# jeya-maria-jose/Medical-Transformer

Hardware: AMD Instinct MI355X
Metric: training images/sec (MedT, 3x128x128) (higher is better)
Workload: dtype f32; 1 GPU; MedT imgsize=128 bs=4/GPU train step (fwd+CE+bwd+Adam), BASELINE.json configs[2] (per GPU: also configs[3]'s shard); global_batch=4, parallelism=dp1

## Files before the change

include/medt_abi.h:

```cpp
#ifndef MEDT_ABI_H
#define MEDT_ABI_H

#include <stddef.h>
#include <stdint.h>

#ifdef __cplusplus
extern "C" {
#endif

#define MEDT_ABI_VERSION 11

#define MEDT_OK            0
#define MEDT_EINVAL       -1
#define MEDT_EUNSUPPORTED -2
#define MEDT_ELAUNCH      -3
#define MEDT_EWORKSPACE   -4

int         medt_abi_version(void);
const char* medt_last_error(void);

void*  medt_queue_create(void);
int    medt_queue_destroy(void* queue);
int    medt_queue_bind(void* queue, void* stream);
size_t medt_queue_pending(const void* queue);
int    medt_queue_flush(void* queue, void* stream);
int    medt_queue_flush2(void* queue, void* stream, void* aux_stream);
int    medt_queue_discard(void* queue);

typedef struct medt_axial_desc {
    int32_t N, C, H, W;
    int32_t G;
    int32_t axis;
    int32_t has_pos;
    int32_t stride;
    int32_t training;
    int32_t bn_groups;
    float   eps;
    float   momentum;
    int32_t out_relu;
    int32_t gate_mode;
    int32_t act_dtype;
} medt_axial_desc;

typedef struct medt_bn_ptrs {
    const float* weight;
    const float* bias;
    float*       running_mean;
    float*       running_var;
    int64_t*     num_batches_tracked;
} medt_bn_ptrs;

typedef struct medt_axial_params {
    const float* w_qkv;
    medt_bn_ptrs bn_qkv;
    medt_bn_ptrs bn_similarity;
    medt_bn_ptrs bn_output;
    const float* relative;
    const float* f_qr;
    const float* f_kr;
    const float* f_sve;
    const float* f_sv;
} medt_axial_params;

typedef struct medt_axial_saved {
    void*  qkv_raw;
    void*  stacked;
    float* lse;
    float* stats;
} medt_axial_saved;

typedef struct medt_axial_grads {
    float* w_qkv;
    float* bn_qkv_weight;  float* bn_qkv_bias;
    float* bn_sim_weight;  float* bn_sim_bias;
    float* bn_out_weight;  float* bn_out_bias;
    float* relative;
    float* gates;
} medt_axial_grads;

size_t medt_axial_stats_floats(const medt_axial_desc*);
size_t medt_axial_workspace_bytes(const medt_axial_desc*);

int medt_axial_layer_fwd(const medt_axial_desc*, const medt_axial_params*, const float* x, float* y,
                         const medt_axial_saved*, void* workspace, size_t workspace_bytes, void* stream);

int medt_axial_layer_bwd(const medt_axial_desc*, const medt_axial_params*, const float* x, const float* y,
                         const float* dy, const medt_axial_saved*, float* dx, const medt_axial_grads*,
                         void* workspace, size_t workspace_bytes, void* stream);

int medt_axial_core_stats(const medt_axial_desc*, const medt_axial_params*, const medt_axial_saved*,
                          void* workspace, size_t workspace_bytes, void* stream);
int medt_axial_core_fwd(const medt_axial_desc*, const medt_axial_params*, const medt_axial_saved*,
                        void* workspace, size_t workspace_bytes, void* stream);
int medt_axial_core_bwd(const medt_axial_desc*, const medt_axial_params*, const medt_axial_saved*, const float* dy,
                        void* workspace, size_t workspace_bytes, void* stream);

typedef struct medt_block_desc {
    int32_t N, C, width, H, W;
    int32_t G;
    int32_t training, bn_groups;
    float   eps, momentum;
} medt_block_desc;

typedef struct medt_block_params {
    const float*      w_down;
    medt_bn_ptrs      bn1;
    medt_axial_params height;
    medt_axial_params width;
    const float*      w_up;
    medt_bn_ptrs      bn2;
} medt_block_params;

typedef struct medt_block_saved {
    float* z1;
    float* y1;
    float* stats1;
    medt_axial_saved height;
    float* y_h;
    medt_axial_saved width;
    float* y_w;
    float* z2;
    float* stats2;
} medt_block_saved;

size_t medt_wopos_block_workspace_bytes(const medt_block_desc*);
int medt_wopos_block_fwd(const medt_block_desc*, const medt_block_params*, const float* x, float* y,
                         const medt_block_saved*, void* workspace, size_t workspace_bytes, void* stream);

typedef struct medt_block_s2_params {
    medt_block_params blk;
    const float*      w_ds;
    medt_bn_ptrs      bn_ds;
} medt_block_s2_params;
typedef struct medt_block_s2_saved {
    medt_block_saved blk;
    float *zd, *yd, *statsd;
} medt_block_s2_saved;
size_t medt_wopos_block_s2_workspace_bytes(const medt_block_desc*);
int medt_wopos_block_s2_fwd(const medt_block_desc*, const medt_block_s2_params*, const float* x, float* y,
                            const medt_block_s2_saved*, void* workspace, size_t workspace_bytes, void* stream);

typedef struct medt_block_grads {
    float *w_down, *bn1_weight, *bn1_bias;
    medt_axial_grads height, width;
    float *w_up, *bn2_weight, *bn2_bias;
} medt_block_grads;
size_t medt_wopos_block_bwd_workspace_bytes(const medt_block_desc*);
int medt_wopos_block_bwd(const medt_block_desc*, const medt_block_params*, const float* x, const float* y, const float* dy,
                         const medt_block_saved*, float* dx, const float* dx_add, const medt_block_grads*,
                         void* workspace, size_t workspace_bytes, void* stream);

typedef struct medt_conv_desc {
    int32_t N, Cin, H, W, Cout;
    int32_t K, stride, pad;
    int32_t has_bias;
    int32_t has_bn;
    int32_t has_res;
    int32_t relu;
    int32_t training, bn_groups;
    float   eps, momentum;
    int32_t lean;
} medt_conv_desc;

size_t medt_conv_stats_floats(const medt_conv_desc*);
size_t medt_conv_workspace_bytes(const medt_conv_desc*);

int medt_conv_block_fwd(const medt_conv_desc*, const float* x, const float* w, const float* bias,
                        const medt_bn_ptrs* bn, const float* res, float* z, float* y, float* stats,
                        void* workspace, size_t workspace_bytes, void* stream);
int medt_conv_block_bwd(const medt_conv_desc*, const float* x, const float* w, const medt_bn_ptrs* bn,
                        const float* z, const float* y, const float* stats, const float* dy,
                        float* dx, float* dw, float* dbias, float* dbn_weight, float* dbn_bias, float* dres,
                        const float* dx_add, void* workspace, size_t workspace_bytes, void* stream);

int medt_gate_mlp_fwd(const float* x, const float* w1, const float* b1, const float* w2, const float* b2, float* xn, float* h,
                      float* o, float* gates, int N, int C, int H, int W, int axis, void* stream);
int medt_gate_mlp_bwd(const float* dgates, const float* gates, const float* o, const float* h, const float* xn,
                      const float* w1, const float* w2, float* scratch, float* dw1, float* db1, float* dw2, float* db2,
                      float* dx, int N, int C, int H, int W, int axis, void* stream);

int medt_up2x_relu_add_fwd(const float* x, const float* skip, float* y, int NC, int H, int W, void* stream);
int medt_up2x_relu_bwd(const float* x, const float* dy, float* dx, int NC, int H, int W, void* stream);

int medt_patch_gather(const float* x, float* xp, int N, int C, int S, int P, int G, void* stream);
int medt_logo_merge_fwd(const float* x, const float* yp, float* y, int N, int C, int S, int P, int G, void* stream);
int medt_logo_merge_bwd(const float* dy, float* dx, float* dyp, int N, int C, int S, int P, int G, void* stream);

size_t medt_ce_partials(int N, int HW);
int medt_ce_fwd(const float* logits, const int64_t* target, float* partials, float* loss_out, int N, int K, int HW,
                int ignore_index, void* stream);
int medt_ce_bwd(const float* logits, const int64_t* target, const float* loss_out, const float* dloss, float* dlogits,
                int N, int K, int HW, int ignore_index, void* stream);

size_t medt_seg_loss_workspace(int N, int K, int HW);
size_t medt_seg_loss_out_floats(int N, int K);
int medt_seg_loss_fwd(const float* logits, const int64_t* target, const float* class_weight, float* partials, float* out,
                      int N, int K, int HW, int ignore_index, float ce_scale, float dice_scale, float eps, void* stream);
int medt_seg_loss_bwd(const float* logits, const int64_t* target, const float* class_weight, const float* out,
                      const float* dloss, float* dlogits, int N, int K, int HW, int ignore_index, float ce_scale,
                      float dice_scale, float eps, void* stream);

int medt_adam_step(float* p, const float* g, float* m, float* v, float* state, size_t n, float lr, float beta1,
                   float beta2, float eps, float weight_decay, float gscale, void* stream);

int medt_relu_mask(const float* a, const float* y, float* out, size_t n, void* stream);

int medt_seg_counts(const float* logits, const int64_t* target, int32_t* counts, int N, int K, int HW, float threshold,
                    void* stream);

int medt_window_gather(const float* image, float* windows, const int32_t* oy, const int32_t* ox, int C, int H, int W, int S,
                       int ny, int nx, void* stream);
int medt_window_blend(const float* win_logits, float* blended, uint8_t* mask, const int32_t* oy, const int32_t* ox, int K,
                      int H, int W, int S, int ny, int nx, float threshold, void* stream);

size_t medt_augment_param_floats(void);
size_t medt_augment_workspace(int N, int th, int tw);
int medt_augment_stats(const uint8_t* image, const float* params, float* workspace, int N, int H, int W, int C, int th,
                       int tw, void* stream);
int medt_augment_apply(const uint8_t* image, const uint8_t* mask, const float* params, float* workspace, float* out_image,
                       int64_t* out_mask, int N, int H, int W, int C, int th, int tw, int use_stats, void* stream);

#define MEDT_EDT_NONE    2147483647
#define MEDT_EDT_MAX_DIM 4096
int medt_edt_cols(const uint8_t* mask, int32_t* g2, int N, int H, int W, int border_mode, void* stream);
int medt_edt_rows(const int32_t* g2, const uint8_t* select, int32_t* d2, int N, int H, int W, void* stream);

#define MEDT_LABEL_TILE_H  16
#define MEDT_LABEL_TILE_W  64
#define MEDT_LABEL_MAX_DIM 4096
size_t medt_label_workspace_bytes(int N, int H, int W);
int medt_label_components(const uint8_t* mask, int32_t* labels, int32_t* count, void* workspace, size_t workspace_bytes, int N,
                          int H, int W, int connectivity, int background, void* stream);
int medt_label_tables(const int32_t* labels, int32_t* area, uint8_t* frame, int N, int H, int W, int stride, int max_count,
                      void* stream);
int medt_label_select(const int32_t* labels, const uint8_t* keep, const uint8_t* mask, uint8_t* out, int N, int H, int W,
                      int stride, void* stream);

#ifdef __cplusplus
}
#endif
#endif
```

medical-transformer_amd/csrc/conv.hip:

```cpp
#include "defer.h"
#include <type_traits>

namespace medt {

template <int K, int OT>
__global__ __launch_bounds__(MEDT_THREADS) void conv2d_fwd_kernel(
    const float* __restrict__ x, const float* __restrict__ w, const float* __restrict__ bias, float* __restrict__ y,
    float* __restrict__ partials, int Cin, int H, int W, int Cout, int Ho, int Wo, int stride, int pad, int relu,
    int npg, int y_bf16) {
    constexpr int KK = K * K;
    MEDT_STATIC_SHARED float red[MEDT_WAVES * OT * 2 * 2];
    const int HoWo = Ho * Wo, per_group = npg * HoWo, ppg = (per_group + MEDT_THREADS - 1) / MEDT_THREADS;
    const int grp = blockIdx.x / ppg, part = blockIdx.x - grp * ppg, o0 = blockIdx.y * OT;
    const int q = part * MEDT_THREADS + threadIdx.x;
    const bool ok = q < per_group;
    const int ni = ok ? q / HoWo : 0, p = ok ? q - ni * HoWo : 0;
    const int n = grp * npg + ni;
    const int ho = p / Wo, wo = p - ho * Wo;
    const int h0 = ho * stride - pad, w0 = wo * stride - pad;
    float acc[OT];
#pragma unroll
    for (int o = 0; o < OT; ++o) acc[o] = bias ? bias[o0 + o] : 0.f;
    const float* xn = x + (size_t)n * Cin * H * W;
    int off[KK];
// ... 304 lines not shown
    for (; o + U <= Cout; o += U) taps(std::integral_constant<int, U>{}, o);
    for (; o < Cout; ++o) taps(std::integral_constant<int, 1>{}, o);
    if (ok) {
        const size_t o0 = ((size_t)n * Cin + c0) * HW + p;
#pragma unroll
        for (int c = 0; c < CT; ++c) dx[o0 + (size_t)c * HW] = add ? acc[c] + add[o0 + (size_t)c * HW] : acc[c];
    }
}

template <int K, int CT, int TM = (1 << (K * K)) - 1>
__global__ __launch_bounds__(MEDT_THREADS) void conv2d_bwd_data_ws_kernel(
    const float* __restrict__ dy, const float* __restrict__ w, float* __restrict__ dx, int N, int Cin, int H, int W,
    int Cout, int Ho, int Wo, int stride, int pad, const float* __restrict__ add, int stage_dy) {
    constexpr int KK = K * K;
    MEDT_STATIC_SHARED float red[3][CT][64];
    extern __shared__ __attribute__((aligned(16))) float wl[];
    const int lane = threadIdx.x & 63, wv = threadIdx.x >> 6;
    const int HW = H * W;
    const long q = (long)blockIdx.x * 64 + lane;
    const int c0 = blockIdx.y * CT;
    if constexpr (TM == (1 << KK) - 1) {
        const int nw = Cout * CT * KK;
        for (int e0 = threadIdx.x; e0 < nw; e0 += 8 * MEDT_THREADS) {
            float v[8];
#pragma unroll
            for (int u = 0; u < 8; ++u) {
                const int e = min(e0 + u * MEDT_THREADS, nw - 1), o = e / (CT * KK), r = e - o * (CT * KK);
                v[u] = w[((size_t)o * Cin + c0) * KK + r];
            }
            MEDT_SCHED_FENCE();
#pragma unroll
            for (int u = 0; u < 8; ++u)
                if (e0 + u * MEDT_THREADS < nw) wl[e0 + u * MEDT_THREADS] = v[u];
        }
    } else {
        constexpr int NL = __builtin_popcount((unsigned)TM);
        const int nw = Cout * CT * NL;
        for (int e0 = threadIdx.x; e0 < nw; e0 += 8 * MEDT_THREADS) {
            float v[8];
            int dst[8];
#pragma unroll
            for (int u = 0; u < 8; ++u) {
                const int e = min(e0 + u * MEDT_THREADS, nw - 1), oc = e / NL, tl = e - oc * NL;
                int t = 0, seen = 0;
#pragma unroll
                for (int b = 0; b < KK; ++b)
                    if ((TM >> b) & 1) { if (seen == tl) t = b; ++seen; }
                const int o = oc / CT, c = oc - o * CT;
                dst[u] = oc * KK + t;
                v[u] = w[((size_t)o * Cin + c0 + c) * KK + t];
            }
            MEDT_SCHED_FENCE();
#pragma unroll
            for (int u = 0; u < 8; ++u)
                if (e0 + u * MEDT_THREADS < nw) wl[dst[u]] = v[u];
        }
    }
    float* dl = wl + Cout * CT * KK;
    const int HoWo_ = Ho * Wo;
    const int nb0 = (int)(((long)blockIdx.x * 64) / HW);
    const int img_stride = Cout * HoWo_ + 1;
    if (stage_dy) {
        const int nb1 = min(N - 1, (int)(((long)blockIdx.x * 64 + 63) / HW));
        const int per = Cout * HoWo_, cnt = (nb1 - nb0 + 1) * per;
        const float* src = dy + (size_t)nb0 * per;
        for (int e0 = threadIdx.x; e0 < cnt; e0 += 8 * MEDT_THREADS) {
            float v[8];
#pragma unroll
            for (int u = 0; u < 8; ++u) v[u] = src[min(e0 + u * MEDT_THREADS, cnt - 1)];
            MEDT_SCHED_FENCE();
#pragma unroll
            for (int u = 0; u < 8; ++u) {
                const int e = e0 + u * MEDT_THREADS;
                if (e < cnt) { const int im = e / per; dl[im * img_stride + (e - im * per)] = v[u]; }
            }
        }
    }
    const bool ok = q < (long)N * HW;
    const int n = ok ? (int)(q / HW) : 0, p = ok ? (int)(q - (long)n * HW) : 0;
    const int h = p / W, ww = p - h * W;
    int off[KK];
#pragma unroll
    for (int kh = 0; kh < K; ++kh)
#pragma unroll
        for (int kw = 0; kw < K; ++kw) {
            const int hh = h + pad - kh, wq = ww + pad - kw;
            int o = -1;
            if (ok && hh >= 0 && wq >= 0 && hh % stride == 0 && wq % stride == 0) {
                const int ho = hh / stride, wo = wq / stride;
                if (ho < Ho && wo < Wo) o = ho * Wo + wo;
            }
            off[kh * K + kw] = o;
        }
    float acc[CT];
#pragma unroll
    for (int c = 0; c < CT; ++c) acc[c] = 0.f;
    const float* dyn = dy + (size_t)n * Cout * Ho * Wo;
    const int ob = (Cout * wv) / 4, oe = (Cout * (wv + 1)) / 4;
    __syncthreads();
    constexpr int U = K == 1 ? 16 : 4;
    const int HoWo = Ho * Wo;
    const float* dln = dl + (n - nb0) * img_stride;
    auto taps = [&](auto u_tag, int o) {
        constexpr int UU = decltype(u_tag)::value;
        float dr[UU][KK];
        if (stage_dy) {
#pragma unroll
            for (int u = 0; u < UU; ++u)
#pragma unroll
                for (int t = 0; t < KK; ++t) dr[u][t] = ((TM >> t) & 1) ? dln[(o + u) * HoWo + max(off[t], 0)] : 0.f;
        } else {
#pragma unroll
            for (int u = 0; u < UU; ++u)
#pragma unroll
                for (int t = 0; t < KK; ++t) dr[u][t] = ((TM >> t) & 1) ? dyn[(size_t)(o + u) * HoWo + max(off[t], 0)] : 0.f;
            MEDT_SCHED_FENCE();
        }
#pragma unroll
        for (int u = 0; u < UU; ++u) {
            float dv[KK];
#pragma unroll
            for (int t = 0; t < KK; ++t) dv[t] = off[t] >= 0 ? dr[u][t] : 0.f;
#pragma unroll
            for (int c = 0; c < CT; ++c) {
                const float* wp = wl + ((o + u) * CT + c) * KK;
#pragma unroll
                for (int t = 0; t < KK; ++t)
                    if ((TM >> t) & 1) acc[c] = fmaf(wp[t], dv[t], acc[c]);
            }
        }
        MEDT_SCHED_FENCE();
    };
    int o = ob;
    for (; o + U <= oe; o += U) taps(std::integral_constant<int, U>{}, o);
    for (; o < oe; ++o) taps(std::integral_constant<int, 1>{}, o);
    if (wv > 0) {
#pragma unroll
        for (int c = 0; c < CT; ++c) red[wv - 1][c][lane] = acc[c];
    }
    __syncthreads();
    if (wv == 0 && ok) {
        const size_t o0 = ((size_t)n * Cin + c0) * HW + p;
#pragma unroll
        for (int c = 0; c < CT; ++c) {
            const float v = acc[c] + (red[0][c][lane] + red[1][c][lane]) + red[2][c][lane];
            dx[o0 + (size_t)c * HW] = add ? v + add[o0 + (size_t)c * HW] : v;
        }
    }
}

static bool conv_bwd_data_ws_enabled() {
    static const bool on = true;
    return on;
}

template <int K>
static int conv2d_bwd_data_k(const float* dy, const float* w, float* dx, int N, int Cin, int H, int W, int Cout, int Ho,
                             int Wo, int stride, int pad, hipStream_t s, const float* add) {
    if constexpr (K != 7) {
        static const long ws_pos3 = 16384L;
        const long npos = (long)N * H * W;
        if ((npos <= 4096 || (K == 3 && Cout * K * K >= 512 && npos <= ws_pos3)) && Cout >= 64 && conv_bwd_data_ws_enabled()) {
            const unsigned g64 = (unsigned)(((long)N * H * W + 63) / 64);
            const int imgs = H * W >= 64 ? 2 : 64 / (H * W) + 1;
            const size_t dy_floats = (size_t)imgs * (Cout * Ho * Wo + 1);
            int tmask = 0;
            if (K == 3)
                for (int h = 0; h < H && h < 8; ++h)
                    for (int ww = 0; ww < W && ww < 8; ++ww)
                        for (int t = 0; t < 9; ++t) {
                            const int hh = h + pad - t / 3, wq = ww + pad - t % 3;
                            if (hh >= 0 && wq >= 0 && hh % stride == 0 && wq % stride == 0 && hh / stride < Ho && wq / stride < Wo) tmask |= 1 << t;
                        }
#ifdef MEDT_AB_DGRAD_ALLTAPS
            tmask = 0x1ff;
#endif
            const bool four = K == 3 && H <= 8 && W <= 8 && tmask == 0x1b0;
#define MEDT_LAUNCH_WS(CT)                                                                                           \
    do {                                                                                                             \
        if constexpr (K == 3) {                                                                                      \
            if (four) {                                                                                              \
                hipLaunchKernelGGL((conv2d_bwd_data_ws_kernel<K, CT, 0x1b0>), dim3(g64, Cin / CT), dim3(MEDT_THREADS), \
                                   ((size_t)Cout * CT * K * K + (stage ? dy_floats : 0)) * sizeof(float), s, dy, w, dx, N, Cin, H, W, \
                                   Cout, Ho, Wo, stride, pad, add, stage);                                          \
                break;                                                                                               \
            }                                                                                                        \
        }                                                                                                            \
        hipLaunchKernelGGL((conv2d_bwd_data_ws_kernel<K, CT>), dim3(g64, Cin / CT), dim3(MEDT_THREADS),               \
                           ((size_t)Cout * CT * K * K + (stage ? dy_floats : 0)) * sizeof(float), s, dy, w, dx, N, Cin, H, W, \
                           Cout, Ho, Wo, stride, pad, add, stage);                                                  \
    } while (0)
            int ct = pick_tile(Cin, K == 1 ? 8 : 4, g64);
            while (ct > 1 && (size_t)Cout * ct * K * K * sizeof(float) > 48 * 1024) ct >>= 1;
            if ((size_t)Cout * ct * K * K * sizeof(float) > 48 * 1024) ct = 0;
            const int stage = (K == 3 && ct && ((size_t)Cout * ct * K * K + dy_floats) * sizeof(float) <= 60 * 1024) ? 1 : 0;
            switch (ct) {
                case 0: break;
                case 8: if constexpr (K == 1) { MEDT_LAUNCH_WS(8); } break;
                case 4: MEDT_LAUNCH_WS(4); break;
                case 2: MEDT_LAUNCH_WS(2); break;
                default: MEDT_LAUNCH_WS(1); break;
            }
#undef MEDT_LAUNCH_WS
            if (ct) return launch_status("conv2d_bwd_data_ws");
        }
    }
    const unsigned gx = (unsigned)(((long)N * H * W + MEDT_THREADS - 1) / MEDT_THREADS);
#define MEDT_LAUNCH_BWD(CT)                                                                                       \
    hipLaunchKernelGGL((conv2d_bwd_data_kernel<K, CT>), dim3(gx, Cin / CT), dim3(MEDT_THREADS), 0, s, dy, w, dx, N, Cin, \
                       H, W, Cout, Ho, Wo, stride, pad, add)
    switch (pick_tile(Cin, K == 7 ? 4 : 16, gx)) {
        case 16: if constexpr (K != 7) { MEDT_LAUNCH_BWD(16); } break;
        case 8: if constexpr (K != 7) { MEDT_LAUNCH_BWD(8); } break;
        case 4: MEDT_LAUNCH_BWD(4); break;
        case 2: MEDT_LAUNCH_BWD(2); break;
        default: MEDT_LAUNCH_BWD(1); break;
    }
#undef MEDT_LAUNCH_BWD
    return launch_status("conv2d_bwd_data");
}

static bool conv2d_bwd_data_thin(int N, int Cin, int H, int W, int Cout, int K, int stride, int pad) {
    return (conv_thin_mode() & 2) && stride == 1 && K == 3 && pad == 1 && !conv_use_mfma(Cout, Cin, K, 1, (long)N * H * W) &&
           conv_thin_ok(N, 1, Cout, H, W, Cin, K, 1, 1);
}
bool conv2d_bwd_data_flips(int N, int Cin, int H, int W, int Cout, int K, int stride, int pad) {
    return stride == 1 && K - 1 - pad >= 0 &&
           (conv_use_mfma(Cout, Cin, K, 1, (long)N * H * W) || conv2d_bwd_data_thin(N, Cin, H, W, Cout, K, stride, pad));
}

int conv2d_bwd_data(const float* dy, const float* w, float* dx, float* wt_scratch, float* ksplit_scratch, int N, int Cin,
                    int H, int W, int Cout, int K, int stride, int pad, hipStream_t s, const float* add, bool wt_ready) {
    const int Ho = (H + 2 * pad - K) / stride + 1, Wo = (W + 2 * pad - K) / stride + 1;
    if (abl_skip(N >= 16 ? (K == 3 ? "conv3_dgrad_l" : "conv1_dgrad_l") : (K == 3 ? "conv3_dgrad_g" : "conv1_dgrad_g"))) return MEDT_OK;
    if (wt_scratch && conv2d_bwd_data_thin(N, Cin, H, W, Cout, K, stride, pad)) {
        if (!wt_ready) {
            int rc = conv_flip_weights(w, wt_scratch, Cout, Cin, K, s);
            if (rc) return rc;
        }
        return conv_thin_fwd(dy, wt_scratch, nullptr, add, dx, nullptr, N, 1, Cout, H, W, Cin, 0, s);
    }
    if (!add && wt_scratch && conv_use_mfma(Cout, Cin, K, 1, (long)N * H * W) && conv2d_bwd_data_flips(N, Cin, H, W, Cout, K, stride, pad) &&
        (ksplit_scratch || conv_mfma_scratch_floats(N, 1, H * W, Cout, Cin, K, conv_rows16_ok(Cout, H, W, K, 1, K - 1 - pad)) == 0))
        return conv_mfma_bwd_data_s1(dy, w, wt_scratch, ksplit_scratch, dx, N, Cin, H, W, Cout, K, pad, s, wt_ready);
    switch (K) {
        case 1: return conv2d_bwd_data_k<1>(dy, w, dx, N, Cin, H, W, Cout, Ho, Wo, stride, pad, s, add);
        case 3: return conv2d_bwd_data_k<3>(dy, w, dx, N, Cin, H, W, Cout, Ho, Wo, stride, pad, s, add);
        case 7: return conv2d_bwd_data_k<7>(dy, w, dx, N, Cin, H, W, Cout, Ho, Wo, stride, pad, s, add);
    }
    set_error("conv2d: kernel size %d unsupported (1, 3, 7)", K);
    return MEDT_EUNSUPPORTED;
}

template <int K, int TO, int TC>
__device__ __forceinline__ void conv_wgrad_body(
    const float* __restrict__ dy, const float* __restrict__ raw, const float* __restrict__ coef,
    const float* __restrict__ x, float* __restrict__ scratch, int N, int Cin, int H, int W, int Cout, int Ho, int Wo,
    int stride, int pad, int QS, int npg, int bx, int by, int bz) {
    constexpr int KK = K * K, RO = TO / 16, RC = TC / 16;
    MEDT_STATIC_SHARED __attribute__((aligned(16))) float A[TO][68];
    MEDT_STATIC_SHARED __attribute__((aligned(16))) float B[TC][68];
    const int Ktot = Cin * KK, HoWo = Ho * Wo;
    const int o0 = bx * TO, k0 = by * TC;
    const long NP = (long)N * HoWo;
    const long q_begin = (long)bz * QS;
    const long q_end = q_begin + QS < NP ? q_begin + QS : NP;
    const int to = threadIdx.x >> 4, tc = threadIdx.x & 15;
    const int j = threadIdx.x & 63, r0 = threadIdx.x >> 6;
    float acc[RO][RC];
#pragma unroll
    for (int a = 0; a < RO; ++a)
#pragma unroll
        for (int b = 0; b < RC; ++b) acc[a][b] = 0.f;
    constexpr int NA = TO / 4, NB = TC / 4;
    float ra[NA], rb[NB];
    auto fetch = [&](long q0) {
        const long q = q0 + j;
        const bool qok = q < q_end;
        const int n = qok ? (int)(q / HoWo) : 0, p = qok ? (int)(q - (long)n * HoWo) : 0;
        const int ho = p / Wo, wo = p - ho * Wo;
        const int hb = ho * stride - pad, wb = wo * stride - pad;
        const float* dyp = dy + (size_t)n * Cout * HoWo + p;
        const float* rawp = raw ? raw + (size_t)n * Cout * HoWo + p : nullptr;
        const float* cf = coef ? coef + (size_t)(n / npg) * Cout * 3 : nullptr;
        const float* xp = x + (size_t)n * Cin * H * W;
#pragma unroll
        for (int i = 0; i < NA; ++i) {
            float a = 0.f;
            const int o = o0 + r0 + 4 * i;
            if (qok && o < Cout) {
                a = dyp[(size_t)o * HoWo];
                if (cf) a = fmaf(cf[o * 3], a, fmaf(cf[o * 3 + 1], rawp[(size_t)o * HoWo], cf[o * 3 + 2]));
            }
            ra[i] = a;
        }
#pragma unroll
        for (int i = 0; i < NB; ++i) {
            float b = 0.f;
            const int k = k0 + r0 + 4 * i;
            if (qok && k < Ktot) {
                const int c = k / KK, t = k - c * KK;
                const int kh = t / K, kw = t - kh * K;
                const int h = hb + kh, w = wb + kw;
                if (h >= 0 && h < H && w >= 0 && w < W) b = xp[((size_t)c * H + h) * W + w];
            }
            rb[i] = b;
// ... 223 lines not shown
```

medical-transformer_amd/csrc/medt_api.hip:

```cpp
#include "defer.h"
#include "fin_inline.h"
#include <string.h>

namespace medt {

static thread_local char g_err[512] = "";

void set_error(const char* fmt, ...) {
    va_list ap;
    va_start(ap, fmt);
    vsnprintf(g_err, sizeof(g_err), fmt, ap);
    va_end(ap);
}

bool abl_skip(const char* family) {
#ifndef MEDT_ABLATE
    (void)family;
    return false;
#else
    static const char* env = [] {
        const char* e = getenv("MEDT_SKIP");
        if (e && *e)
            fprintf(stderr, "libmedt_hip: MEDT_SKIP=%s -- TIMING EXPERIMENT: these kernel families are NOT launched, every result of "
                            "this process is garbage\n", e);
// ... 19 lines not shown
    if (e != hipSuccess) {
        (void)hipGetLastError();
        set_error("%s: opt-in for more than 64 KB of dynamic LDS refused on device %d: %s", what, dev, hipGetErrorString(e));
        return MEDT_ELAUNCH;
    }
    if (dev < 64) done[dev] = 1;
    return MEDT_OK;
}

int launch_status(const char* what) {
    hipError_t e = hipGetLastError();
    if (e != hipSuccess) {
        set_error("%s: %s", what, hipGetErrorString(e));
        return MEDT_ELAUNCH;
    }
    return MEDT_OK;
}

struct LayerStats {
    BnStats qkv, sim, out;
    LayerStats(float* p, const AxialGeom& g) {
        const int nq = g.groups * 2 * g.C, ns = g.groups * g.SC, no = g.groups * g.OC;
        qkv = BnStats(p, nq);
        sim = BnStats(p + 4 * (size_t)nq, ns);
        out = BnStats(p + 4 * (size_t)(nq + ns), no);
    }
};

struct FwdWs {
    float *part_qkv, *part_sim, *part_out, *qkv_ksplit, *tables, *gate_eff;
    unsigned* flag;
    FwdWs(Carver& c, const AxialGeom& g) {
        flag = c.take<unsigned>(4);
        gate_eff = c.take<float>(4);
        const size_t kq = conv2d_fwd_scratch_floats(g.N, g.groups, g.C, g.H, g.W, 2 * g.C, 1, 1, 0);
        qkv_ksplit = c.take<float>(kq);
        if (!kq) qkv_ksplit = nullptr;
        part_qkv = c.take<float>((size_t)g.groups * conv_parts_per_group(g.N, g.groups, g.HW, g.C, 2 * g.C, 1, 1) * 2 * g.C * 2 * 2);
        part_sim = c.take<float>((size_t)g.groups * sim_stats_parts(g) * g.SC * 2 * 2);
        tables = c.take<float>(sim_tables_floats(g));
        part_out = c.take<float>((size_t)g.groups * g.tpg * g.OC * 2 * 2);
    }
};

struct BwdWs {
    float *part_ob, *coef_out, *part_sb, *coef_sim, *dqkv, *part_qb, *coef_qkv, *rel_part, *gate_part, *dw_scratch,
        *dy_masked, *gate_eff, *gate_tmp;
    float *tables, *gram, *pg_part, *gate_raw, *gate_rows;
    float* raw32;
    size_t nblocks;
    bool sweep;
    SweepPlan plan;
    size_t sweep_blocks;
    int qb_rpg;
    BwdWs(Carver& c, const AxialGeom& g, int stride, int out_relu, int gate_mode) {
        gate_eff = c.take<float>(4);
        gate_tmp = c.take<float>(4);
        const int ppg = conv2d_parts_per_group(g.N, g.groups, g.HW), TL = 2 * g.L - 1;
        sweep = axial_bwd_sweep_plan(g, gate_mode == 2 ? 4 : 0, &plan);
        sweep_blocks = sweep ? (size_t)g.groups * plan.nparts * g.G : 0;
        qb_rpg = sweep ? plan.nparts + plan.fparts : g.tpg;
        nblocks = (size_t)g.groups * g.tpg * g.G;
        const size_t rel_rows = sweep ? sweep_blocks + (size_t)g.groups * g.G : nblocks;
        part_ob = c.take<float>((size_t)g.groups * ppg * g.OC * 2);
        coef_out = c.take<float>((size_t)g.groups * g.OC * 3);
        part_sb = c.take<float>((size_t)g.groups * (sweep && plan.nparts > g.tpg ? plan.nparts : g.tpg) * g.G * 4);
        coef_sim = c.take<float>((size_t)g.groups * g.SC * 3);
        dqkv = c.take<float>((size_t)g.N * 2 * g.C * g.HW);
        part_qb = c.take<float>((size_t)g.groups * (qb_rpg > g.tpg ? qb_rpg : g.tpg) * 2 * g.C * 2);
        coef_qkv = c.take<float>((size_t)g.groups * 2 * g.C * 3);
        rel_part = c.take<float>(g.pos ? (rel_rows > nblocks ? rel_rows : nblocks) * 2 * g.gp * TL : 0);
        const size_t nseqh = (size_t)g.groups * g.spg * g.G;
        gate_part = c.take<float>(g.pos ? (nblocks > nseqh ? nblocks : nseqh) * 4 : 0);
        dw_scratch = c.take<float>((size_t)conv2d_bwd_weight_splits(g.N, g.C, 2 * g.C, 1, g.H, g.W) * 2 * g.C * g.C);
        dy_masked = c.take<float>(out_relu ? (size_t)g.N * g.C * (g.H / stride) * (g.W / stride) : 0);
        tables = c.take<float>(sweep ? sim_tables_floats(g) : 0);
        gram = c.take<float>(sweep ? (size_t)g.groups * g.spg * g.G * plan.npg_floats : 0);
        pg_part = c.take<float>(sweep ? sweep_blocks * g.L * plan.npg_floats : 0);
        gate_raw = c.take<float>(sweep ? sweep_blocks * 4 : 0);
        gate_rows = c.take<float>(sweep ? (size_t)g.groups * g.G * 4 : 0);
        static const bool raw32_on = true;
        raw32 = c.take<float>(sweep && g.bf16 && raw32_on ? (size_t)g.N * 2 * g.C * g.HW : 0);
        if (!(sweep && g.bf16 && raw32_on)) raw32 = nullptr;
    }
};

static int attention_core_bwd(const AxialGeom& g, const medt_axial_desc* d, const medt_axial_params* p, const BwdWs& w,
                              const float* qkv_raw, const float* stacked, const float* lse, const float* dy, const LayerStats& st,
                              GatePtrs gates, bool want_gates, float* d_sim_w, float* d_sim_b, hipStream_t s,
                              const BfinSrc* ob = nullptr, bool sim_inline = false, const BfinSrc* qb = nullptr,
                              const float* ymask = nullptr) {
    const int tr = d->training ? 1 : 0;
    int rc;
    if (w.sweep) {
        if ((rc = axial_attn_bwd_sweep(g, w.plan, qkv_raw, st.qkv, st.sim, p->relative, gates, stacked, lse, dy, w.coef_out,
                                       d->stride, w.dqkv, w.part_qb, w.qb_rpg, w.part_sb, w.rel_part, w.pg_part, w.gram,
                                       want_gates ? w.gate_raw : nullptr, s, w.raw32, ob, ymask))) return rc;
        AxialGeom gs = g;
        gs.tpg = w.plan.nparts;
        SimBSrc sb = no_simb_src();
        if (sim_inline) {
            sb.partials = w.part_sb; sb.rows = w.plan.nparts; sb.G = g.G; sb.SC = g.SC; sb.training = tr; sb.on = 1;
            sb.count = g.sim_count; sb.ss = st.sim; sb.weight = p->bn_similarity.weight;
            sb.coef = w.coef_sim; sb.dweight = d_sim_w; sb.dbias = d_sim_b;
        } else {
            const TablesJob tj{p->relative, w.tables, g.hq, g.L, tr ? sim_tables_blocks(g) : 0};
            if ((rc = axial_sim_bwd_finalize(gs, w.part_sb, st.sim, p->bn_similarity.weight, tr, w.coef_sim, d_sim_w, d_sim_b, s, &tj)))
                return rc;
        }
        if ((rc = axial_attn_bwd_fix(g, w.plan, qkv_raw, st.qkv, w.coef_sim, w.tables, w.gram, gates, tr, w.dqkv, w.part_qb,
                                     w.qb_rpg, s, sim_inline ? &sb : nullptr))) return rc;
        return axial_attn_bwd_relfix(g, w.plan, p->relative, w.coef_sim, st.sim, gates, w.pg_part,
                                     want_gates ? w.gate_raw : nullptr, tr, d->eps,
                                     w.rel_part + w.sweep_blocks * 2 * g.gp * (2 * g.L - 1), w.gate_rows, s, qb);
    }
    if ((rc = axial_attn_bwd_stats(g, qkv_raw, st.qkv, st.sim, p->relative, gates, stacked, lse, dy, w.coef_out, d->stride,
                                   w.part_sb, s))) return rc;
    if ((rc = axial_sim_bwd_finalize(g, w.part_sb, st.sim, p->bn_similarity.weight, tr, w.coef_sim, d_sim_w, d_sim_b, s)))
        return rc;
    return axial_attn_bwd(g, qkv_raw, st.qkv, st.sim, w.coef_sim, p->relative, gates, stacked, lse, dy, w.coef_out, d->stride,
                          w.dqkv, w.part_qb, w.rel_part, want_gates ? w.gate_part : nullptr, s);
}

static int effective_gates(const medt_axial_desc* d, const medt_axial_params* p, float* eff, hipStream_t s, GatePtrs* out) {
    *out = GatePtrs{p->f_qr, p->f_kr, p->f_sve, p->f_sv, 0};
    if (d->gate_mode == 0 || !p->f_qr) return MEDT_OK;
    if (d->gate_mode == 2) {
        *out = GatePtrs{p->f_qr, p->f_qr + 1, p->f_qr + 3, p->f_qr + 2, 4};
        return MEDT_OK;
    }
    if (d->gate_mode != 1) { set_error("axial: gate_mode %d unsupported (0: raw, 1: sigmoid, 2: per sequence)", d->gate_mode); return MEDT_EUNSUPPORTED; }
    if (!p->f_kr || !p->f_sve || !p->f_sv) { set_error("axial: gate_mode 1 needs all four gates"); return MEDT_EINVAL; }
    int rc = gate_sigmoid_fwd(p->f_qr, p->f_kr, p->f_sve, p->f_sv, eff, s);
    if (rc) return rc;
    *out = GatePtrs{eff, eff + 1, eff + 2, eff + 3, 0};
    return MEDT_OK;
}

static int check_common(const medt_axial_desc* d, const medt_axial_params* p, const medt_axial_saved* sv, AxialGeom* g) {
    if (!d || !p || !sv) { set_error("null descriptor / params / saved"); return MEDT_EINVAL; }
    int rc = axial_geom(*d, g);
    if (rc) return rc;
    if (!p->w_qkv || !p->bn_qkv.weight || !p->bn_qkv.bias || !p->bn_similarity.weight || !p->bn_similarity.bias ||
        !p->bn_output.weight || !p->bn_output.bias) { set_error("null parameter pointer"); return MEDT_EINVAL; }
    if (!d->training && (!p->bn_qkv.running_mean || !p->bn_qkv.running_var || !p->bn_similarity.running_mean ||
                         !p->bn_similarity.running_var || !p->bn_output.running_mean || !p->bn_output.running_var)) {
        set_error("eval mode needs running statistics"); return MEDT_EINVAL;
    }
    if (g->pos && !p->relative) { set_error("has_pos without relative table"); return MEDT_EINVAL; }
    if (!sv->qkv_raw || !sv->stacked || !sv->stats) { set_error("null saved buffer"); return MEDT_EINVAL; }
    return MEDT_OK;
}

}

using namespace medt;

extern "C" {

int medt_abi_version(void) { return MEDT_ABI_VERSION; }
const char* medt_last_error(void) { return g_err; }

size_t medt_axial_stats_floats(const medt_axial_desc* d) {
    AxialGeom g;
    if (!d || axial_geom(*d, &g)) return 0;
    return (size_t)4 * g.groups * (2 * g.C + g.SC + g.OC);
}

size_t medt_axial_workspace_bytes(const medt_axial_desc* d) {
    AxialGeom g;
    if (!d || axial_geom(*d, &g)) return 0;
    Carver cf(nullptr, 0), cb(nullptr, 0);
    FwdWs f(cf, g);
    BwdWs b(cb, g, d->stride, d->out_relu, d->gate_mode);
    return align_up(cf.off > cb.off ? cf.off : cb.off, 256) + 256;
}

int medt_axial_core_stats(const medt_axial_desc* d, const medt_axial_params* p, const medt_axial_saved* sv, void* ws,
                          size_t ws_bytes, void* stream) {
    AxialGeom g;
    int rc = check_common(d, p, sv, &g);
    if (rc) return rc;
    float* qkv_raw = (float*)sv->qkv_raw;
    float* stacked = (float*)sv->stacked;
    Carver c(ws, ws_bytes);
    FwdWs w(c, g);
    if (!ws || !c.ok()) { set_error("workspace too small: need %zu", c.off); return MEDT_EWORKSPACE; }
    LayerStats st(sv->stats, g);
    GatePtrs gates;
    if ((rc = effective_gates(d, p, w.gate_eff, (hipStream_t)stream, &gates))) return rc;
    return axial_logit_stats(g, qkv_raw, st.qkv, p->relative, gates, w.tables, w.part_sim, (hipStream_t)stream);
}

int medt_axial_core_fwd(const medt_axial_desc* d, const medt_axial_params* p, const medt_axial_saved* sv, void* ws,
                        size_t ws_bytes, void* stream) {
    AxialGeom g;
    int rc = check_common(d, p, sv, &g);
    if (rc) return rc;
    float* qkv_raw = (float*)sv->qkv_raw;
    float* stacked = (float*)sv->stacked;
    Carver c(ws, ws_bytes);
    FwdWs w(c, g);
    if (!ws || !c.ok()) { set_error("workspace too small: need %zu", c.off); return MEDT_EWORKSPACE; }
    LayerStats st(sv->stats, g);
    GatePtrs gates;
    if ((rc = effective_gates(d, p, w.gate_eff, (hipStream_t)stream, &gates))) return rc;
    return axial_attn_fwd(g, qkv_raw, st.qkv, st.sim, p->relative, gates, stacked, sv->lse,
                          d->training ? w.part_out : nullptr, w.flag, (hipStream_t)stream);
}

int medt_axial_core_bwd(const medt_axial_desc* d, const medt_axial_params* p, const medt_axial_saved* sv, const float* dy,
                        void* ws, size_t ws_bytes, void* stream) {
    AxialGeom g;
    int rc = check_common(d, p, sv, &g);
    if (rc) return rc;
    float* qkv_raw = (float*)sv->qkv_raw;
    float* stacked = (float*)sv->stacked;
    if (!dy || !sv->lse) { set_error("core_bwd: null dy / lse"); return MEDT_EINVAL; }
    if (d->out_relu) { set_error("core_bwd: out_relu layers are not supported by the benchmark entry"); return MEDT_EUNSUPPORTED; }
    Carver c(ws, ws_bytes);
    BwdWs w(c, g, d->stride, d->out_relu, d->gate_mode);
    if (!ws || !c.ok()) { set_error("workspace too small: need %zu", c.off); return MEDT_EWORKSPACE; }
    hipStream_t s = (hipStream_t)stream;
    LayerStats st(sv->stats, g);
    GatePtrs gates;
    if ((rc = effective_gates(d, p, w.gate_eff, s, &gates))) return rc;
    return attention_core_bwd(g, d, p, w, qkv_raw, stacked, sv->lse, dy, st, gates, p->f_qr != nullptr, w.part_ob,
                              w.part_ob + g.SC, s);
}

int medt_axial_layer_fwd(const medt_axial_desc* d, const medt_axial_params* p, const float* x, float* y,
                         const medt_axial_saved* sv, void* ws, size_t ws_bytes, void* stream) {
    AxialGeom g;
    int rc = check_common(d, p, sv, &g);
    if (rc) return rc;
    float* qkv_raw = (float*)sv->qkv_raw;
    float* stacked = (float*)sv->stacked;
    if (!x || !y) { set_error("null x / y"); return MEDT_EINVAL; }
    if (d->training && g.row_count <= 1.0) {
        set_error("axial: training-mode BatchNorm needs more than 1 value per channel (got %g)", g.row_count);
        return MEDT_EINVAL;
    }
    Carver c(ws, ws_bytes);
    FwdWs w(c, g);
    if (!ws || !c.ok()) { set_error("workspace too small: need %zu", c.off); return MEDT_EWORKSPACE; }
    hipStream_t s = (hipStream_t)stream;
    LayerStats st(sv->stats, g);
    GatePtrs gates;
    if ((rc = effective_gates(d, p, w.gate_eff, s, &gates))) return rc;
    const int tr = d->training ? 1 : 0, ppg = conv_parts_per_group(g.N, g.groups, g.HW, g.C, 2 * g.C, 1, 1);
    if (wopos_small_ok(g, *d)) {
        if ((rc = wopos_small_fwd(g, *d, *p, x, y, qkv_raw, stacked, sv->lse, w.part_qkv, w.part_sim, w.part_out,
                                  s))) return rc;
        if (Queue* q = queue_for(s)) {
            q->fin.push_back(FinJob{make_fin(w.part_qkv, 1, 2 * g.C, g.row_count, p->bn_qkv, st.qkv), g.groups, tr, d->momentum, d->eps});
            q->fin.push_back(FinJob{make_fin(w.part_sim, 1, g.SC, g.sim_count, p->bn_similarity, st.sim), g.groups, tr, d->momentum, d->eps});
            q->fin.push_back(FinJob{make_fin(w.part_out, 1, g.OC, g.row_count, p->bn_output, st.out), g.groups, tr, d->momentum, d->eps});
            return MEDT_OK;
        }
        return bn_finalize3(w.part_qkv, 2 * g.C, g.row_count, p->bn_qkv, st.qkv, w.part_sim, g.SC, g.sim_count,
                            p->bn_similarity, st.sim, w.part_out, g.OC, g.row_count, p->bn_output, st.out, 1, g.groups,
                            d->momentum, d->eps, tr, s);
    }
    if ((rc = conv2d_fwd(x, p->w_qkv, nullptr, qkv_raw, tr ? w.part_qkv : nullptr, w.qkv_ksplit, g.N, g.C, g.H, g.W,
                         2 * g.C, 1, 1, 0, 0, g.groups, s, g.bf16))) return rc;
    const TablesJob tj{p->relative, w.tables, g.hq, g.L, tr ? sim_tables_blocks(g) : 0};
    if ((rc = bn_finalize(w.part_qkv, ppg, g.groups, 2 * g.C, g.row_count, p->bn_qkv, d->momentum, d->eps, tr,
                          st.qkv, s, &tj))) return rc;
    if (tr && (rc = axial_logit_stats(g, qkv_raw, st.qkv, p->relative, gates, w.tables, w.part_sim, s))) return rc;
    auto fin_src_of = [&](const float* partials, int parts, int CH, double count, const medt_bn_ptrs& bn, BnStats out) {
        FinSrc fs = no_fin_src();
        fs.f = make_fin(partials, parts, CH, count, bn, out);
        fs.momentum = d->momentum; fs.eps = d->eps; fs.on = 1;
        return fs;
    };
    const bool sim_inl = inline_fin_ok(tr, g.groups, sim_stats_parts(g)) && axial_attn_fwd_inlines(g, gates, w.flag);
    const FinSrc sim_src = fin_src_of(w.part_sim, sim_stats_parts(g), g.SC, g.sim_count, p->bn_similarity, st.sim);
    if (!sim_inl && (rc = bn_finalize(w.part_sim, sim_stats_parts(g), g.groups, g.SC, g.sim_count, p->bn_similarity, d->momentum,
                                      d->eps, tr, st.sim, s))) return rc;
    if ((rc = axial_attn_fwd(g, qkv_raw, st.qkv, st.sim, p->relative, gates, stacked, sv->lse,
                             tr ? w.part_out : nullptr, w.flag, s, sim_inl ? &sim_src : nullptr))) return rc;
    const bool out_inl = inline_fin_ok(tr, g.groups, g.oparts) && axial_out_fwd_inlines(*d);
    const FinSrc out_src = fin_src_of(w.part_out, g.oparts, g.OC, g.row_count, p->bn_output, st.out);
    if (!out_inl && (rc = bn_finalize(w.part_out, g.oparts, g.groups, g.OC, g.row_count, p->bn_output, d->momentum, d->eps, tr,
                                      st.out, s))) return rc;
    return axial_out_fwd(*d, stacked, st.out, y, s, out_inl ? &out_src : nullptr);
}

int medt_axial_layer_bwd(const medt_axial_desc* d, const medt_axial_params* p, const float* x, const float* y,
                         const float* dy, const medt_axial_saved* sv, float* dx, const medt_axial_grads* gr, void* ws,
                         size_t ws_bytes, void* stream) {
    AxialGeom g;
    int rc = check_common(d, p, sv, &g);
    if (rc) return rc;
    float* qkv_raw = (float*)sv->qkv_raw;
    float* stacked = (float*)sv->stacked;
    if (!x || !dy || !dx || !gr || !sv->lse) { set_error("null x / dy / dx / grads / lse"); return MEDT_EINVAL; }
    if (!gr->w_qkv || !gr->bn_qkv_weight || !gr->bn_qkv_bias || !gr->bn_sim_weight || !gr->bn_sim_bias ||
        !gr->bn_out_weight || !gr->bn_out_bias || (g.pos && !gr->relative)) {
        set_error("null gradient pointer"); return MEDT_EINVAL;
    }
    if (d->out_relu && !y) { set_error("out_relu backward needs the forward output y"); return MEDT_EINVAL; }
    Carver c(ws, ws_bytes);
    BwdWs w(c, g, d->stride, d->out_relu, d->gate_mode);
    if (!ws || !c.ok()) { set_error("workspace too small: need %zu", c.off); return MEDT_EWORKSPACE; }
    hipStream_t s = (hipStream_t)stream;
    LayerStats st(sv->stats, g);
    GatePtrs gates;
    if ((rc = effective_gates(d, p, w.gate_eff, s, &gates))) return rc;
    const int tr = d->training ? 1 : 0, ppg = conv2d_parts_per_group(g.N, g.groups, g.HW), TL = 2 * g.L - 1;
    if (wopos_small_bwd_ok(g, *d)) {
        if ((rc = wopos_small_bwd(g, *d, *p, y, dy, qkv_raw, stacked, sv->lse, st.qkv, st.sim, st.out, w.dqkv,
                                  w.part_ob, w.part_sb, w.part_qb, w.coef_qkv, s))) return rc;
        if ((rc = wopos_small_bwd_finalize(g, *d, *p, w.part_ob, w.part_sb, w.part_qb, st.qkv, st.sim, st.out, *gr, s,
                                           queue_for(s)))) return rc;
        if ((rc = conv1x1_bwd_data(w.dqkv, qkv_raw, w.coef_qkv, p->w_qkv, dx, g.N, g.C, 2 * g.C, g.HW, g.groups, s)))
            return rc;
        return conv2d_bwd_weight(w.dqkv, qkv_raw, w.coef_qkv, x, gr->w_qkv, w.dw_scratch, g.N, g.C, g.H, g.W, 2 * g.C,
                                 1, 1, 0, g.groups, s, queue_for(s));
    }
    const float* ymask = nullptr;
    if (d->out_relu) {
#ifndef MEDT_AB_NO_MASK_FUSE
        if (w.sweep) ymask = y;
#endif
        if (!ymask) {
            if ((rc = relu_mask(dy, y, w.dy_masked, (size_t)g.N * g.C * (g.H / d->stride) * (g.W / d->stride), s))) return rc;
            dy = w.dy_masked;
        }
    }
    const float out_dscale = 1.f / (float)(d->stride * d->stride);
    const bool sim_inl = w.sweep && g.pos && inline_fin_ok(tr, g.groups, w.plan.nparts) &&
                         axial_out_bwd_stats_tables_ok(*d, sim_tables_blocks(g), g.L);
    const TablesJob btj{p->relative, w.tables, g.hq, g.L, sim_tables_blocks(g)};
    if ((rc = axial_out_bwd_stats(*d, stacked, dy, st.out, w.part_ob, s, sim_inl ? &btj : nullptr, ymask))) return rc;
    BfinSrc ob = no_bfin_src();
    if (w.sweep && inline_fin_ok(tr, g.groups, ppg)) {
        ob.j = BfinJob{w.part_ob, ppg, g.groups, g.OC, tr, g.row_count, out_dscale, st.out, p->bn_output.weight, w.coef_out,
                       gr->bn_out_weight, gr->bn_out_bias};
        ob.on = 1;
    } else if ((rc = bn_bwd_finalize(w.part_ob, ppg, g.groups, g.OC, g.row_count, out_dscale, st.out, p->bn_output.weight, tr,
                                     w.coef_out, gr->bn_out_weight, gr->bn_out_bias, s))) return rc;
    BfinSrc qb = no_bfin_src();
    if (w.sweep && (!g.bf16 || w.raw32) && inline_fin_ok(tr, g.groups, w.qb_rpg)) {
        qb.j = BfinJob{w.part_qb, w.qb_rpg, g.groups, 2 * g.C, tr, g.row_count, 1.f, st.qkv, p->bn_qkv.weight, w.coef_qkv,
                       gr->bn_qkv_weight, gr->bn_qkv_bias};
        qb.on = 1;
    }
    if ((rc = attention_core_bwd(g, d, p, w, qkv_raw, stacked, sv->lse, dy, st, gates, gr->gates != nullptr,
                                 gr->bn_sim_weight, gr->bn_sim_bias, s, ob.on ? &ob : nullptr, sim_inl, qb.on ? &qb : nullptr, ymask))) return rc;
    const float *bq_raw = qkv_raw, *bq_coef = w.coef_qkv;
    static const bool bf16_fused = true;
    if (g.bf16 && w.raw32) {
        if (!qb.on && (rc = bn_bwd_finalize(w.part_qb, w.qb_rpg, g.groups, 2 * g.C, g.row_count, 1.f, st.qkv, p->bn_qkv.weight, tr,
                                         w.coef_qkv, gr->bn_qkv_weight, gr->bn_qkv_bias, s))) return rc;
        bq_raw = w.raw32;
    } else if (g.bf16 && bf16_fused && (long)g.N * 2 * g.C <= 65535) {
        if ((rc = bn_bwd_fin_apply_bf16(w.part_qb, w.qb_rpg, g.groups, 2 * g.C, g.row_count, 1.f, st.qkv, p->bn_qkv.weight, tr,
                                        w.coef_qkv, gr->bn_qkv_weight, gr->bn_qkv_bias, w.dqkv, qkv_raw, g.N, g.HW, s))) return rc;
        bq_raw = nullptr;
        bq_coef = nullptr;
    } else {
        if (!qb.on && (rc = bn_bwd_finalize(w.part_qb, w.qb_rpg, g.groups, 2 * g.C, g.row_count, 1.f, st.qkv, p->bn_qkv.weight, tr,
                                            w.coef_qkv, gr->bn_qkv_weight, gr->bn_qkv_bias, s))) return rc;
        if (g.bf16) {
            if ((rc = bn_bwd_apply_raw_bf16(w.dqkv, qkv_raw, w.coef_qkv, g.N, 2 * g.C, g.HW, g.groups, s))) return rc;
            bq_raw = nullptr;
            bq_coef = nullptr;
        }
    }
    if ((rc = conv1x1_bwd_data(w.dqkv, bq_raw, bq_coef, p->w_qkv, dx, g.N, g.C, 2 * g.C, g.HW, g.groups, s)))
        return rc;
    Queue* q = queue_for(s);
    if ((rc = conv2d_bwd_weight(w.dqkv, bq_raw, bq_coef, x, gr->w_qkv, w.dw_scratch, g.N, g.C, g.H, g.W, 2 * g.C, 1,
                                1, 0, g.groups, s, q))) return rc;
    if (g.pos) {
        const int rel_rows = w.sweep ? (int)w.sweep_blocks + g.groups * g.G : (int)w.nblocks;
        const float* gate_src = w.sweep ? w.gate_rows : w.gate_part;
        const int gate_rows = w.sweep ? g.groups * g.G : (int)w.nblocks;
        if (q) q->reduce.push_back(RJob{w.rel_part, gr->relative, rel_rows, 2 * g.gp * TL});
        else if ((rc = reduce_rows(w.rel_part, rel_rows, 2 * g.gp * TL, gr->relative, s))) return rc;
        if (gr->gates && d->gate_mode == 2) {
            if ((rc = gate_seq_reduce(w.gate_part, gr->gates, g.groups * g.spg, g.G, s))) return rc;
        } else if (gr->gates) {
            const bool sig = d->gate_mode == 1 && p->f_qr;
            if (q && !sig) q->reduce.push_back(RJob{gate_src, gr->gates, gate_rows, 4});
            else {
                if ((rc = reduce_rows(gate_src, gate_rows, 4, sig ? w.gate_tmp : gr->gates, s))) return rc;
                if (sig && (rc = gate_sigmoid_bwd(w.gate_tmp, w.gate_eff, gr->gates, s))) return rc;
            }
        }
    }
    return MEDT_OK;
}


}

namespace medt {
struct ConvGeom { int Ho, Wo, HoWo, ppg, ppg_bwd, splits; size_t out_elems; };
static int conv_geom(const medt_conv_desc* d, ConvGeom* g) {
    if (!d || d->N <= 0 || d->Cin <= 0 || d->Cout <= 0 || d->H <= 0 || d->W <= 0 || d->stride < 1 || d->pad < 0) {
        set_error("conv: bad descriptor"); return MEDT_EINVAL;
    }
    if (d->K != 1 && d->K != 3 && d->K != 7) { set_error("conv: kernel size %d unsupported (1, 3, 7)", d->K); return MEDT_EUNSUPPORTED; }
    if (d->has_bn && (d->bn_groups < 1 || d->N % d->bn_groups)) { set_error("conv: bad bn_groups"); return MEDT_EINVAL; }
    if (d->has_bn && d->has_bias) { set_error("conv: bias followed by BatchNorm is not on the reference's path"); return MEDT_EUNSUPPORTED; }
    if (!d->has_bn && d->has_res) { set_error("conv: residual without BatchNorm is not on the reference's path"); return MEDT_EUNSUPPORTED; }
    g->Ho = (d->H + 2 * d->pad - d->K) / d->stride + 1;
    g->Wo = (d->W + 2 * d->pad - d->K) / d->stride + 1;
    if (g->Ho <= 0 || g->Wo <= 0) { set_error("conv: empty output"); return MEDT_EINVAL; }
    if ((double)d->N * d->Cin * d->H * d->W >= 2147483648.0 || (double)d->N * d->Cout * g->Ho * g->Wo >= 2147483648.0 ||
        (double)d->Cout * d->Cin * d->K * d->K >= 2147483648.0) {
        set_error("conv: tensors of 2^31 elements and more are unsupported"); return MEDT_EUNSUPPORTED;
    }
    g->HoWo = g->Ho * g->Wo;
    g->ppg = conv_stem7_ok(d->Cin, d->H, d->W, d->Cout, d->K, d->stride, d->pad)
                 ? conv_stem7_parts_per_group(d->N, d->has_bn ? d->bn_groups : 1, g->HoWo)
                 : conv_parts_per_group(d->N, d->has_bn ? d->bn_groups : 1, g->HoWo, d->Cin, d->Cout, d->K, d->stride, d->H, d->W, d->pad);
    g->ppg_bwd = conv2d_parts_per_group(d->N, d->has_bn ? d->bn_groups : 1, g->HoWo);
    g->splits = conv2d_bwd_weight_splits(d->N, d->Cin, d->Cout, d->K, g->Ho, g->Wo);
    g->out_elems = (size_t)d->N * d->Cout * g->HoWo;
    return MEDT_OK;
}
struct ConvWs {
    float *partials, *coef, *bias_scratch, *gbuf, *dz, *dw_scratch, *wt, *ksplit, *ksplit_fwd, *ksplit_bwd;
    ConvWs(Carver& c, const medt_conv_desc* d, const ConvGeom& g) {
        wt = c.take<float>((size_t)d->Cout * d->Cin * d->K * d->K);
        const size_t kf = conv2d_fwd_scratch_floats(d->N, d->has_bn ? d->bn_groups : 1, d->Cin, d->H, d->W, d->Cout, d->K,
                                                    d->stride, d->pad);
        const size_t kb = conv2d_bwd_data_scratch_floats(d->N, d->Cin, d->H, d->W, d->Cout, d->K, d->stride, d->pad);
        ksplit = c.take<float>(kf > kb ? kf : kb);
        if (!(kf > 0 || kb > 0)) ksplit = nullptr;
        ksplit_fwd = kf > 0 ? ksplit : nullptr;
        ksplit_bwd = kb > 0 ? ksplit : nullptr;
        partials = c.take<float>(d->has_bn ? (size_t)d->bn_groups * (2 * g.ppg > g.ppg_bwd ? 2 * g.ppg : g.ppg_bwd) * d->Cout * 2 : 0);
        coef = c.take<float>(d->has_bn ? (size_t)d->bn_groups * d->Cout * 3 : 0);
        bias_scratch = c.take<float>((size_t)16 * d->Cout);
        gbuf = c.take<float>(g.out_elems);
        dz = c.take<float>(d->has_bn ? g.out_elems : 0);
        dw_scratch = c.take<float>((size_t)g.splits * d->Cout * d->Cin * d->K * d->K);
    }
};
}

extern "C" {

static bool conv_preflip(const medt_conv_desc* d) {
    static const bool on = true;
    return on && d->training && d->K == 3 && conv2d_bwd_data_flips(d->N, d->Cin, d->H, d->W, d->Cout, d->K, d->stride, d->pad);
}
static size_t conv_bn_stats_floats(const medt_conv_desc* d) { return d->has_bn ? (size_t)4 * d->bn_groups * d->Cout : 0; }
static float* conv_preflip_ptr(const medt_conv_desc* d, float* stats) { return stats + align_up(conv_bn_stats_floats(d), 64); }

size_t medt_conv_stats_floats(const medt_conv_desc* d) {
    if (!d) return 0;
    const size_t bn = (d->has_bn && d->bn_groups > 0 && d->Cout > 0) ? (size_t)4 * d->bn_groups * d->Cout : 0;
    ConvGeom g;
    if (conv_geom(d, &g)) return bn;
    return conv_preflip(d) ? align_up(bn, 64) + (size_t)d->Cout * d->Cin * d->K * d->K : bn;
}

size_t medt_conv_workspace_bytes(const medt_conv_desc* d) {
    ConvGeom g;
    if (conv_geom(d, &g)) return 0;
    Carver c(nullptr, 0);
    ConvWs w(c, d, g);
    return align_up(c.off, 256) + 256;
}

int medt_conv_block_fwd(const medt_conv_desc* d, const float* x, const float* w, const float* bias,
                        const medt_bn_ptrs* bn, const float* res, float* z, float* y, float* stats, void* ws,
                        size_t ws_bytes, void* stream) {
    ConvGeom g;
    int rc = conv_geom(d, &g);
    if (rc) return rc;
    if (!x || !w || !y || (d->has_bias && !bias) || (d->has_bn && (!bn || !z || !stats)) || (d->has_res && !res)) {
        set_error("conv fwd: null pointer"); return MEDT_EINVAL;
    }
    hipStream_t s = (hipStream_t)stream;
    Carver c(ws, ws_bytes);
    ConvWs cw(c, d, g);
    if (!ws || !c.ok()) { set_error("conv workspace too small: need %zu", c.off); return MEDT_EWORKSPACE; }
    if (stats && conv_preflip(d)) {
        float* wt = conv_preflip_ptr(d, stats);
        if (Queue* q = queue_for(s)) q->flip.push_back(FlipJob{w, wt, d->Cout, d->Cin, d->K});
        else if ((rc = conv_flip_weights(w, wt, d->Cout, d->Cin, d->K, s))) return rc;
    }
    if (!d->has_bn)
        return conv2d_fwd(x, w, d->has_bias ? bias : nullptr, y, nullptr, cw.ksplit_fwd, d->N, d->Cin, d->H, d->W, d->Cout,
                          d->K, d->stride, d->pad, d->relu, 1, s);
    const int tr = d->training ? 1 : 0;
    if (!tr && (!bn->running_mean || !bn->running_var)) { set_error("conv fwd: eval mode needs running statistics"); return MEDT_EINVAL; }
    if (tr && (double)(d->N / d->bn_groups) * g.HoWo <= 1.0) {
        set_error("conv fwd: training-mode BatchNorm needs more than 1 value per channel"); return MEDT_EINVAL;
    }
    BnStats st(stats, d->bn_groups * d->Cout);
    if (conv_small_ok(*d)) {
        if ((rc = conv_small_fwd(*d, x, w, *bn, res, z, y, cw.partials, s))) return rc;
        if (Queue* q = queue_for(s)) {
            q->fin.push_back(FinJob{make_fin(cw.partials, 1, d->Cout, (double)(d->N / d->bn_groups) * g.HoWo, *bn, st),
                                    d->bn_groups, tr, d->momentum, d->eps});
            return MEDT_OK;
        }
        return bn_finalize(cw.partials, 1, d->bn_groups, d->Cout, (double)(d->N / d->bn_groups) * g.HoWo, *bn, d->momentum,
                           d->eps, tr, st, s);
    }
    if ((rc = conv2d_fwd(x, w, nullptr, z, tr ? cw.partials : nullptr, cw.ksplit_fwd, d->N, d->Cin, d->H, d->W, d->Cout, d->K,
                         d->stride, d->pad, 0, d->bn_groups, s))) return rc;
    static const bool fused_fin = true;
    const double count = (double)(d->N / d->bn_groups) * g.HoWo;
    if (!fused_fin) {
        if ((rc = bn_finalize(cw.partials, g.ppg, d->bn_groups, d->Cout, count, *bn, d->momentum, d->eps, tr, st, s))) return rc;
        return bn_apply_act(z, st, d->has_res ? res : nullptr, y, d->N, d->Cout, g.HoWo, d->bn_groups, d->relu, s);
    }
    if ((rc = bn_fin_apply(z, cw.partials, g.ppg, count, *bn, d->eps, tr, st, d->has_res ? res : nullptr, y, d->N, d->Cout,
                           g.HoWo, d->bn_groups, d->relu, s))) return rc;
    if (!tr) return MEDT_OK;
    if (Queue* q = queue_for(s)) {
        q->fin.push_back(FinJob{make_fin(cw.partials, g.ppg, d->Cout, count, *bn, st), d->bn_groups, 2, d->momentum, d->eps});
        return MEDT_OK;
    }
    return bn_finalize(cw.partials, g.ppg, d->bn_groups, d->Cout, count, *bn, d->momentum, d->eps, 2, st, s);
}

int medt_conv_block_bwd(const medt_conv_desc* d, const float* x, const float* w, const medt_bn_ptrs* bn, const float* z,
                        const float* y, const float* stats, const float* dy, float* dx, float* dw, float* dbias,
                        float* dbn_weight, float* dbn_bias, float* dres, const float* dx_add, void* ws, size_t ws_bytes,
                        void* stream) {
    ConvGeom g;
    int rc = conv_geom(d, &g);
    if (rc) return rc;
    if (!x || !w || !dy || !dw || (d->relu && !y) || (d->has_bn && (!bn || !z || !stats || !dbn_weight || !dbn_bias)) ||
        (d->has_bias && !dbias)) { set_error("conv bwd: null pointer"); return MEDT_EINVAL; }
    Carver c(ws, ws_bytes);
    ConvWs cw(c, d, g);
    if (!ws || !c.ok()) { set_error("conv workspace too small: need %zu", c.off); return MEDT_EWORKSPACE; }
    hipStream_t s = (hipStream_t)stream;
    const float* grad_out;
    bool dx_done = false;
    if (d->has_bn) {
        BnStats st(const_cast<float*>(stats), d->bn_groups * d->Cout);
        float* gb = (d->has_res && dres) ? dres : cw.gbuf;
        const bool small = conv_small_ok(*d);
        const bool aligned = ((((uintptr_t)dy | (uintptr_t)y | (uintptr_t)z | (uintptr_t)dres | (uintptr_t)cw.dz) & 15) == 0);
        if (small || (aligned && bn_chan_threads(*d, g.HoWo))) {
            if (small && dx && aligned && !d->lean && bn_dgrad1x1_small_ok(*d)) {
                rc = bn_dgrad1x1_small(*d, dy, y, z, st, bn->weight, w, dx_add, (d->has_res && dres) ? dres : nullptr,
                                       cw.dz, cw.partials, dx, s);
                dx_done = true;
            } else if (small)
                rc = bn_act_bwd_small(*d, dy, y, z, st, bn->weight, (d->has_res && dres) ? dres : nullptr, cw.dz,
                                      cw.partials, g.HoWo, s);
            else
                rc = bn_act_bwd_chan(*d, dy, y, z, st, bn->weight, (d->has_res && dres) ? dres : nullptr, cw.dz,
                                     cw.partials, g.HoWo, s);
            if (rc) return rc;
            if (Queue* q = queue_for(s))
                q->bfin.push_back(BfinJob{cw.partials, 1, d->bn_groups, d->Cout, d->training ? 1 : 0,
                                          (double)(d->N / d->bn_groups) * g.HoWo, 1.f, st, bn->weight, cw.coef, dbn_weight,
                                          dbn_bias});
            else if ((rc = bn_bwd_finalize(cw.partials, 1, d->bn_groups, d->Cout, (double)(d->N / d->bn_groups) * g.HoWo, 1.f,
                                           st, bn->weight, d->training ? 1 : 0, cw.coef, dbn_weight, dbn_bias, s))) return rc;
        } else {
        if ((rc = bn_act_bwd_stats(dy, y, z, st, gb, cw.partials, d->N, d->Cout, g.HoWo, d->bn_groups, d->relu, s))) return rc;
        if ((rc = bn_bwd_finalize(cw.partials, g.ppg_bwd, d->bn_groups, d->Cout,
                                  (double)(d->N / d->bn_groups) * g.HoWo, 1.f, st, bn->weight, d->training ? 1 : 0, cw.coef,
                                  dbn_weight, dbn_bias, s))) return rc;
        if ((rc = bn_bwd_apply(gb, z, cw.coef, cw.dz, d->N, d->Cout, g.HoWo, d->bn_groups, s))) return rc;
        }
        grad_out = cw.dz;
    } else if (d->relu) {
        if ((rc = relu_mask(dy, y, cw.gbuf, g.out_elems, s))) return rc;
        grad_out = cw.gbuf;
    } else {
        grad_out = dy;
    }
    const bool preflipped = stats && conv_preflip(d);
    if (dx && !dx_done && (rc = conv2d_bwd_data(grad_out, w, dx, preflipped ? conv_preflip_ptr(d, const_cast<float*>(stats)) : cw.wt, cw.ksplit_bwd,
                                                d->N, d->Cin, d->H, d->W, d->Cout, d->K, d->stride, d->pad, s, dx_add, preflipped))) return rc;
    Queue* q = queue_for(s);
    if (d->has_bias) {
        if (q) {
            const int splits = channel_sum_splits_for(d->N, g.HoWo);
            q->csum.push_back(CJob{grad_out, splits == 1 ? dbias : cw.bias_scratch, d->N, d->Cout, g.HoWo, splits});
            if (splits > 1) q->reduce.push_back(RJob{cw.bias_scratch, dbias, splits, d->Cout});
        } else if ((rc = channel_sum(grad_out, dbias, cw.bias_scratch, d->N, d->Cout, g.HoWo, s))) return rc;
    }
    return conv2d_bwd_weight(grad_out, nullptr, nullptr, x, dw, cw.dw_scratch, d->N, d->Cin, d->H, d->W, d->Cout, d->K, d->stride,
                             d->pad, 1, s, q);
}

size_t medt_wopos_block_workspace_bytes(const medt_block_desc* d) {
    if (!d || !wopos_block_ok(*d)) return 0;
    return align_up(wopos_block_part_doubles(*d) * sizeof(double), 256) + 256;
}

int medt_wopos_block_fwd(const medt_block_desc* d, const medt_block_params* p, const float* x, float* y,
                         const medt_block_saved* sv, void* ws, size_t ws_bytes, void* stream) {
    if (!d || !p || !x || !y || !sv) { set_error("block fwd: null argument"); return MEDT_EINVAL; }
    if (!wopos_block_ok(*d)) { set_error("block fwd: shape not supported by the fused kernel"); return MEDT_EUNSUPPORTED; }
    if (!p->w_down || !p->w_up || !p->height.w_qkv || !p->width.w_qkv || !sv->z1 || !sv->y1 || !sv->stats1 || !sv->y_h ||
        !sv->y_w || !sv->z2 || !sv->stats2 || !sv->height.qkv_raw || !sv->height.stacked || !sv->height.lse ||
        !sv->height.stats || !sv->width.qkv_raw || !sv->width.stacked || !sv->width.lse || !sv->width.stats) {
        set_error("block fwd: null pointer"); return MEDT_EINVAL;
    }
    const medt_bn_ptrs* bns[8] = {&p->bn1, &p->height.bn_qkv, &p->height.bn_similarity, &p->height.bn_output,
                                  &p->width.bn_qkv, &p->width.bn_similarity, &p->width.bn_output, &p->bn2};
    for (int b = 0; b < 8; ++b) {
        if (!bns[b]->weight || !bns[b]->bias) { set_error("block fwd: null BatchNorm parameter"); return MEDT_EINVAL; }
        if (!d->training && (!bns[b]->running_mean || !bns[b]->running_var)) {
            set_error("block fwd: eval mode needs running statistics"); return MEDT_EINVAL;
        }
    }
    Carver c(ws, ws_bytes);
    double* parts = c.take<double>(wopos_block_part_doubles(*d));
    if (!ws || !c.ok()) { set_error("block workspace too small: need %zu", c.off); return MEDT_EWORKSPACE; }
    hipStream_t s = (hipStream_t)stream;
    int rc = wopos_block_fwd(*d, *p, x, y, *sv, parts, s);
    if (rc) return rc;
    const int tr = d->training ? 1 : 0, gs = d->bn_groups, W = d->width, G = d->G;
    const double rows = (double)(d->N / gs) * d->H * d->W, sims = rows * d->H;
    AxialGeom gh;
    {
        medt_axial_desc ad{d->N, W, d->H, d->W, G, 0, 0, 1, d->training, gs, d->eps, d->momentum, 0, 0, 0};
        if ((rc = axial_geom(ad, &gh))) return rc;
    }
    LayerStats sh(sv->height.stats, gh), sw(sv->width.stats, gh);
    const int chs[8] = {W, 2 * W, G, W, 2 * W, G, W, d->C};
    const double cnt[8] = {rows, rows, sims, rows, rows, sims, rows, rows};
    BnStats outs[8] = {BnStats(sv->stats1, gs * W), sh.qkv, sh.sim, sh.out, sw.qkv, sw.sim, sw.out, BnStats(sv->stats2, gs * d->C)};
    const float* pp = reinterpret_cast<const float*>(parts);
    Queue* q = queue_for(s);
    for (int b = 0; b < 8; ++b) {
        if (q) q->fin.push_back(FinJob{make_fin(pp, 1, chs[b], cnt[b], *bns[b], outs[b]), gs, tr, d->momentum, d->eps});
        else if ((rc = bn_finalize(pp, 1, gs, chs[b], cnt[b], *bns[b], d->momentum, d->eps, tr, outs[b], s))) return rc;
        pp += (size_t)gs * chs[b] * 2 * 2;
    }
    return MEDT_OK;
}

size_t medt_wopos_block_s2_workspace_bytes(const medt_block_desc* d) {
    if (!d || !wopos_block_s2_ok(*d)) return 0;
    return align_up(wopos_block_s2_part_doubles(*d) * sizeof(double), 256) + 256;
}

int medt_wopos_block_s2_fwd(const medt_block_desc* d, const medt_block_s2_params* p, const float* x, float* y,
                            const medt_block_s2_saved* sv, void* ws, size_t ws_bytes, void* stream) {
    if (!d || !p || !x || !y || !sv) { set_error("block s2 fwd: null argument"); return MEDT_EINVAL; }
    if (!wopos_block_s2_ok(*d)) { set_error("block s2 fwd: shape not supported by the fused kernel"); return MEDT_EUNSUPPORTED; }
    const medt_block_params& bp = p->blk;
    const medt_block_saved& b0 = sv->blk;
    if (!bp.w_down || !bp.w_up || !bp.height.w_qkv || !bp.width.w_qkv || !p->w_ds || !b0.z1 || !b0.y1 || !b0.stats1 || !b0.y_h ||
        !b0.y_w || !b0.z2 || !b0.stats2 || !b0.height.qkv_raw || !b0.height.stacked || !b0.height.lse || !b0.height.stats ||
        !b0.width.qkv_raw || !b0.width.stacked || !b0.width.lse || !b0.width.stats || !sv->zd || !sv->yd || !sv->statsd) {
        set_error("block s2 fwd: null pointer"); return MEDT_EINVAL;
    }
    const medt_bn_ptrs* bns[9] = {&bp.bn1, &bp.height.bn_qkv, &bp.height.bn_similarity, &bp.height.bn_output,
                                  &bp.width.bn_qkv, &bp.width.bn_similarity, &bp.width.bn_output, &bp.bn2, &p->bn_ds};
    for (int b = 0; b < 9; ++b) {
        if (!bns[b]->weight || !bns[b]->bias) { set_error("block s2 fwd: null BatchNorm parameter"); return MEDT_EINVAL; }
        if (!d->training && (!bns[b]->running_mean || !bns[b]->running_var)) {
            set_error("block s2 fwd: eval mode needs running statistics"); return MEDT_EINVAL;
        }
    }
    Carver c(ws, ws_bytes);
    double* parts = c.take<double>(wopos_block_s2_part_doubles(*d));
    if (!ws || !c.ok()) { set_error("block s2 workspace too small: need %zu", c.off); return MEDT_EWORKSPACE; }
    hipStream_t s = (hipStream_t)stream;
    int rc = wopos_block_s2_fwd(*d, *p, x, y, *sv, parts, s);
    if (rc) return rc;
    const int tr = d->training ? 1 : 0, gs = d->bn_groups, W = d->width, G = d->G, CO = 2 * d->width;
    const double rows = (double)(d->N / gs) * d->H * d->W, sims = rows * d->H, rows2 = rows / 4;
    AxialGeom gh;
    {
        medt_axial_desc ad{d->N, W, d->H, d->W, G, 0, 0, 1, d->training, gs, d->eps, d->momentum, 0, 0, 0};
        if ((rc = axial_geom(ad, &gh))) return rc;
    }
    LayerStats sh(b0.height.stats, gh), sw(b0.width.stats, gh);
    const int chs[9] = {W, 2 * W, G, W, 2 * W, G, W, CO, CO};
    const double cnt[9] = {rows, rows, sims, rows, rows, sims, rows, rows2, rows2};
    BnStats outs[9] = {BnStats(b0.stats1, gs * W), sh.qkv, sh.sim, sh.out, sw.qkv, sw.sim, sw.out, BnStats(b0.stats2, gs * CO),
                       BnStats(sv->statsd, gs * CO)};
    const float* pp = reinterpret_cast<const float*>(parts);
    Queue* q = queue_for(s);
    for (int b = 0; b < 9; ++b) {
        if (q) q->fin.push_back(FinJob{make_fin(pp, 1, chs[b], cnt[b], *bns[b], outs[b]), gs, tr, d->momentum, d->eps});
        else if ((rc = bn_finalize(pp, 1, gs, chs[b], cnt[b], *bns[b], d->momentum, d->eps, tr, outs[b], s))) return rc;
        pp += (size_t)gs * chs[b] * 2 * 2;
    }
    return MEDT_OK;
}

size_t medt_wopos_block_bwd_workspace_bytes(const medt_block_desc* d) {
    if (!d || !wopos_block_bwd_ok(*d)) return 0;
    return wopos_block_bwd_ws_bytes(*d);
}

int medt_wopos_block_bwd(const medt_block_desc* d, const medt_block_params* p, const float* x, const float* y, const float* dy,
                         const medt_block_saved* sv, float* dx, const float* dx_add, const medt_block_grads* gr, void* ws,
                         size_t ws_bytes, void* stream) {
    if (!d || !p || !x || !y || !dy || !sv || !dx || !gr) { set_error("block bwd: null argument"); return MEDT_EINVAL; }
    if (!wopos_block_bwd_ok(*d)) { set_error("block bwd: shape not supported by the fused kernel, or MEDT_BLOCK_BWD != 1"); return MEDT_EUNSUPPORTED; }
    if (!p->w_down || !p->w_up || !p->height.w_qkv || !p->width.w_qkv || !sv->z1 || !sv->y1 || !sv->stats1 || !sv->y_h ||
        !sv->y_w || !sv->z2 || !sv->stats2 || !sv->height.qkv_raw || !sv->height.stacked || !sv->height.lse ||
        !sv->height.stats || !sv->width.qkv_raw || !sv->width.stacked || !sv->width.lse || !sv->width.stats) {
        set_error("block bwd: null pointer"); return MEDT_EINVAL;
    }
    const medt_bn_ptrs* bns[8] = {&p->bn1, &p->height.bn_qkv, &p->height.bn_similarity, &p->height.bn_output,
                                  &p->width.bn_qkv, &p->width.bn_similarity, &p->width.bn_output, &p->bn2};
    for (int b = 0; b < 8; ++b)
        if (!bns[b]->weight) { set_error("block bwd: null BatchNorm weight"); return MEDT_EINVAL; }
    const medt_axial_grads* ag[2] = {&gr->height, &gr->width};
    for (int l = 0; l < 2; ++l)
        if (!ag[l]->w_qkv || !ag[l]->bn_qkv_weight || !ag[l]->bn_qkv_bias || !ag[l]->bn_sim_weight || !ag[l]->bn_sim_bias ||
            !ag[l]->bn_out_weight || !ag[l]->bn_out_bias) { set_error("block bwd: null gradient pointer"); return MEDT_EINVAL; }
    if (!gr->w_down || !gr->bn1_weight || !gr->bn1_bias || !gr->w_up || !gr->bn2_weight || !gr->bn2_bias) {
        set_error("block bwd: null gradient pointer"); return MEDT_EINVAL;
    }
    return wopos_block_bwd(*d, *p, x, y, dy, dx_add, *sv, dx, *gr, ws, ws_bytes, (hipStream_t)stream);
}

int medt_gate_mlp_fwd(const float* x, const float* w1, const float* b1, const float* w2, const float* b2, float* xn, float* h,
                      float* o, float* gates, int N, int C, int H, int W, int axis, void* stream) {
    if (!x || !w1 || !b1 || !w2 || !b2 || !xn || !h || !o || !gates || N < 1 || C < 1 || C > 4096 || H < 1 || W < 1) {
        set_error("gate_mlp fwd: bad arguments"); return MEDT_EINVAL;
    }
    return gate_mlp_fwd(x, w1, b1, w2, b2, xn, h, o, gates, N, C, H, W, axis ? 1 : 0, (hipStream_t)stream);
}
int medt_gate_mlp_bwd(const float* dgates, const float* gates, const float* o, const float* h, const float* xn,
                      const float* w1, const float* w2, float* scratch, float* dw1, float* db1, float* dw2, float* db2,
                      float* dx, int N, int C, int H, int W, int axis, void* stream) {
    if (!dgates || !gates || !o || !h || !xn || !w1 || !w2 || !scratch || !dw1 || !db1 || !dw2 || !db2 || !dx) {
        set_error("gate_mlp bwd: null pointer"); return MEDT_EINVAL;
    }
    const size_t nseq = (size_t)N * (axis ? H : W);
    float *d_o = scratch, *dh = d_o + nseq * 4, *dxn = dh + nseq * C;
    return gate_mlp_bwd(dgates, gates, o, h, xn, w1, w2, d_o, dh, dxn, dw1, db1, dw2, db2, dx, N, C, H, W, axis ? 1 : 0,
                        (hipStream_t)stream);
}

int medt_up2x_relu_add_fwd(const float* x, const float* skip, float* y, int NC, int H, int W, void* stream) {
    if (!x || !y || NC <= 0 || H <= 0 || W <= 0) { set_error("up2x fwd: bad arguments"); return MEDT_EINVAL; }
// ... 228 lines not shown
```

medical-transformer_amd/csrc/medt_kernels.h:

```cpp
#pragma once
#include "medt_common.h"

namespace medt {

struct Queue;

int conv1x1_ptiles(int HW);
int conv1x1_fwd(const float* x, const float* w, float* y, float* partials,
                int N, int Cin, int Cout, int HW, hipStream_t s);
int conv1x1_bwd_data(const float* dy, const float* raw, const float* coef, const float* w, float* dx,
                     int N, int Cin, int Cout, int HW, int groups, hipStream_t s);
struct TablesJob { const float* relative; float* tables; int HQ, L, blocks; };
int bn_finalize(const float* partials, int parts_per_group, int groups, int CH, double count,
                const medt_bn_ptrs& bn, float momentum, float eps, int training, BnStats out, hipStream_t s,
                const TablesJob* tables = nullptr);
int bn_finalize3(const float* p0, int CH0, double n0, const medt_bn_ptrs& bn0, BnStats o0,
                 const float* p1, int CH1, double n1, const medt_bn_ptrs& bn1, BnStats o1,
                 const float* p2, int CH2, double n2, const medt_bn_ptrs& bn2, BnStats o2,
                 int ppg, int groups, float momentum, float eps, int training, hipStream_t s);
int bn_bwd_finalize(const float* partials, int parts_per_group, int groups, int CH, double count, float dscale,
                    BnStats st, const float* weight, int training, float* coef, float* dweight, float* dbias,
                    hipStream_t s);

struct FinSrc;
bool axial_out_fwd_inlines(const medt_axial_desc& d);
int axial_out_fwd(const medt_axial_desc& d, const float* stacked, BnStats st, float* y, hipStream_t s, const FinSrc* src = nullptr);
int bn_bwd_apply_raw_bf16(float* d, const float* raw_bf16, const float* coef, int N, int CH, int HW, int groups, hipStream_t s);
int bn_bwd_fin_apply_bf16(const float* partials, int ppg, int groups, int CH, double count, float dscale, BnStats st,
                          const float* weight, int training, float* coef, float* dweight, float* dbias, float* d,
                          const float* raw_bf16, int N, int HW, hipStream_t s);
bool axial_out_bwd_stats_tables_ok(const medt_axial_desc& d, int blocks, int L);
int axial_out_bwd_stats(const medt_axial_desc& d, const float* stacked, const float* dy, BnStats st,
                        float* partials, hipStream_t s, const TablesJob* tj = nullptr, const float* ymask = nullptr);

int reduce_rows(const float* in, int P, int K, float* out, hipStream_t s);

int conv2d_parts_per_group(int N, int groups, int HoWo);
int conv_parts_per_group(int N, int groups, int HoWo, int Cin, int Cout, int K, int stride, int H = 0, int W = 0, int pad = 0);
bool conv_thin_ok(int N, int groups, int Cin, int H, int W, int Cout, int K, int stride, int pad);
int conv_thin_parts_per_group(int N, int groups, int Cin, int H, int W, int Cout, int K, int stride, int pad);
int conv_thin_fwd(const float* x, const float* w, const float* bias, const float* add, float* y, float* partials, int N, int groups,
                  int Cin, int H, int W, int Cout, int relu, hipStream_t s);
bool conv_stem7_ok(int Cin, int H, int W, int Cout, int K, int stride, int pad);
int conv_stem7_parts_per_group(int N, int groups, int HoWo);
int conv_stem7_fwd(const float* x, const float* w, const float* bias, float* y, float* partials, int N, int H, int W, int Cout,
                   int relu, hipStream_t s);
int conv2d_fwd(const float* x, const float* w, const float* bias, float* y, float* partials, float* scratch, int N,
               int Cin, int H, int W, int Cout, int K, int stride, int pad, int relu, int groups, hipStream_t s,
               int y_bf16 = 0);
size_t conv2d_fwd_scratch_floats(int N, int groups, int Cin, int H, int W, int Cout, int K, int stride, int pad);
int conv2d_bwd_data(const float* dy, const float* w, float* dx, float* wt_scratch, float* ksplit_scratch, int N, int Cin,
                    int H, int W, int Cout, int K, int stride, int pad, hipStream_t s, const float* add = nullptr, bool wt_ready = false);
bool conv2d_bwd_data_flips(int N, int Cin, int H, int W, int Cout, int K, int stride, int pad);
int conv_flip_weights(const float* w, float* wt, int Cout, int Cin, int K, hipStream_t s);
size_t conv2d_bwd_data_scratch_floats(int N, int Cin, int H, int W, int Cout, int K, int stride, int pad);
int conv2d_bwd_weight_splits(int N, int Cin, int Cout, int K, int Ho, int Wo);
int conv2d_bwd_weight(const float* dy, const float* raw, const float* coef, const float* x, float* dw, float* scratch,
                      int N, int Cin, int H, int W, int Cout, int K, int stride, int pad, int groups, hipStream_t s,
                      Queue* q = nullptr);
int channel_sum_splits_for(int N, int HW);
int channel_sum(const float* x, float* out, float* scratch , int N, int C, int HW, hipStream_t s);

bool conv_use_mfma(int Cin, int Cout, int K, int stride, long positions);
int conv_mfma_parts_per_group(int N, int groups, int HoWo);
bool conv_rows16_ok(int Cin, int H, int W, int K, int stride, int pad);
size_t conv_mfma_scratch_floats(int N, int groups, int HoWo, int Cin, int Cout, int K, bool rows16 = false);
int conv_mfma_fwd(const float* x, const float* w, const float* bias, float* y, float* partials, float* scratch, int N,
                  int Cin, int H, int W, int Cout, int K, int stride, int pad, int relu, int groups, hipStream_t s);
int conv_mfma_bwd_data_s1(const float* dy, const float* w, float* wt_scratch, float* ksplit_scratch, float* dx, int N,
                          int Cin, int H, int W, int Cout, int K, int pad, hipStream_t s, bool wt_ready = false);
int conv_wgrad_mfma(const float* dy, const float* raw, const float* coef, const float* x, float* scratch, int N, int Cin,
                    int H, int W, int Cout, int Ho, int Wo, int K, int stride, int pad, int QS, int splits, int npg,
                    hipStream_t s);

int bn_apply_act(const float* z, BnStats st, const float* res, float* y, int N, int C, int HW, int groups, int relu,
                 hipStream_t s);
int bn_act_bwd_stats(const float* dy, const float* y, const float* z, BnStats st, float* g, float* partials, int N, int C,
                     int HW, int groups, int relu, hipStream_t s);
int bn_bwd_apply(const float* g, const float* z, const float* coef, float* dz, int N, int C, int HW, int groups,
                 hipStream_t s);
int relu_mask(const float* a, const float* y, float* out, size_t total, hipStream_t s);
int seg_counts(const float* logits, const int64_t* target, int* counts, int N, int K, int HW, float threshold, hipStream_t s);
int relu_fwd(const float* x, float* y, size_t total, hipStream_t s);
int up2x_relu_add_fwd(const float* x, const float* skip, float* y, int NC, int H, int W, hipStream_t s);
int up2x_relu_bwd(const float* x, const float* dy, float* dx, int NC, int H, int W, hipStream_t s);
int patch_gather(const float* x, float* xp, int N, int C, int S, int P, int G, hipStream_t s);
int window_gather(const float* image, float* windows, const int32_t* oy, const int32_t* ox, int C, int H, int W, int S,
                  int ny, int nx, hipStream_t s);
int window_blend(const float* win, float* blended, uint8_t* mask, const int32_t* oy, const int32_t* ox, int K, int H, int W,
                 int S, int ny, int nx, float threshold, hipStream_t s);
size_t augment_param_floats();
int augment_parts(int th, int tw);
int augment_stats(const uint8_t* image, const float* params, float* workspace, int N, int H, int W, int C, int th, int tw,
                  hipStream_t s);
int augment_apply(const uint8_t* image, const uint8_t* mask, const float* params, float* workspace, float* out_image,
                  int64_t* out_mask, int N, int H, int W, int C, int th, int tw, int use_stats, hipStream_t s);
int edt_cols(const uint8_t* mask, int32_t* g2, int N, int H, int W, int border_mode, hipStream_t s);
int edt_rows(const int32_t* g2, const uint8_t* select, int32_t* d2, int N, int H, int W, hipStream_t s);
size_t label_workspace_bytes(int N, int H, int W);
int label_components(const uint8_t* mask, int32_t* labels, int32_t* count, void* workspace, int N, int H, int W, int connectivity,
                     int background, hipStream_t s);
int label_tables(const int32_t* labels, int32_t* area, uint8_t* frame, int N, int H, int W, int stride, hipStream_t s);
int label_select(const int32_t* labels, const uint8_t* keep, const uint8_t* mask, uint8_t* out, int N, int H, int W, int stride,
                 hipStream_t s);
int logo_merge_fwd(const float* x, const float* yp, float* y, int N, int C, int S, int P, int G, hipStream_t s);
int logo_merge_bwd(const float* dy, float* dx, float* dyp, int N, int C, int S, int P, int G, hipStream_t s);
int ce_parts(size_t npix);
int ce_fwd(const float* logits, const int64_t* target, float* partials, float* loss_out, int N, int K, int HW, int ignore,
           hipStream_t s);
int ce_bwd(const float* logits, const int64_t* target, const float* loss_out, const float* dloss, float* dlogits, int N,
           int K, int HW, int ignore, hipStream_t s);
int seg_loss_bpi(int HW);
size_t seg_loss_partials(int N, int K, int HW);
size_t seg_loss_out_floats(int N, int K);
int seg_loss_fwd(const float* logits, const int64_t* target, const float* weight, float* partials, float* out, int N, int K,
                 int HW, int ignore, float ce_scale, float dice_scale, float eps, hipStream_t s);
int seg_loss_bwd(const float* logits, const int64_t* target, const float* weight, const float* out, const float* dloss,
                 float* dlogits, int N, int K, int HW, int ignore, float ce_scale, float dice_scale, hipStream_t s);
int gate_sigmoid_fwd(const float* f_qr, const float* f_kr, const float* f_sve, const float* f_sv, float* eff, hipStream_t s);
int gate_sigmoid_bwd(const float* d_eff, const float* eff, float* dgate, hipStream_t s);
int gate_seq_reduce(const float* partials, float* dgates, int nseq, int G, hipStream_t s);
int gate_mlp_fwd(const float* x, const float* w1, const float* b1, const float* w2, const float* b2, float* xn, float* h,
                 float* o, float* gates, int N, int C, int H, int W, int axis, hipStream_t s);
int gate_mlp_bwd(const float* dgates, const float* gates, const float* o, const float* h, const float* xn, const float* w1,
                 const float* w2, float* d_o, float* dh, float* dxn, float* dw1, float* db1, float* dw2, float* db2,
                 float* dx, int N, int C, int H, int W, int axis, hipStream_t s);
int adam_step(float* p, const float* g, float* m, float* v, float* state, size_t n, float lr, float b1, float b2,
              float eps, float wd, float gscale, hipStream_t s);

struct AxialGeom {
    int N, C, H, W, G, gp, hq, L, Bo, axis, pos, OC, OCg, SC;
    int bf16;
    int groups, npg;
    int spg;
    int S_T;
    int tpg;
    int HW;
    int fast3;
    int fparts;
    int nt;
    int rows4, nt4, oparts;
    int bound_path;
    float bound_shift;
    double sim_count;
    double row_count;
};
int  axial_geom(const medt_axial_desc& d, AxialGeom* g);
size_t axial_core_lds_bytes(const AxialGeom& g, bool backward);

struct GatePtrs { const float *f_qr, *f_kr, *f_sve, *f_sv; int stride; };

struct FinSrc;
struct BfinSrc;
int axial_attn_fwd_fast(const AxialGeom& g, const float* qkv_raw, BnStats qkv, BnStats sim, const float* relative,
                        GatePtrs gates, float* stacked, float* lse, float* out_partials, unsigned* flag, hipStream_t s,
                        const FinSrc* simsrc = nullptr);
int axial_attn_fwd_fast_bf16(const AxialGeom& g, const float* qkv_raw, BnStats qkv, BnStats sim, const float* relative,
                             GatePtrs gates, float* stacked, float* lse, float* out_partials, unsigned* flag,
                             hipStream_t s, const FinSrc* simsrc = nullptr);
int fast3_max_subtiles(int gp, int L, int axis);
int fast4_subtile_sequences(int L);
int fast4_max_subtiles(int axis);
bool wopos_block_ok(const medt_block_desc& d);
size_t wopos_block_part_doubles(const medt_block_desc& d);
int wopos_block_fwd(const medt_block_desc& d, const medt_block_params& p, const float* x, float* y,
                    const medt_block_saved& sv, double* parts, hipStream_t s);
bool wopos_block_s2_ok(const medt_block_desc& d);
size_t wopos_block_s2_part_doubles(const medt_block_desc& d);
int wopos_block_s2_fwd(const medt_block_desc& d, const medt_block_s2_params& p, const float* x, float* y,
                       const medt_block_s2_saved& sv, double* parts, hipStream_t s);
bool wopos_block_bwd_ok(const medt_block_desc& d);
size_t wopos_block_bwd_ws_bytes(const medt_block_desc& d);
int wopos_block_bwd(const medt_block_desc& d, const medt_block_params& p, const float* x, const float* y, const float* dy,
                    const float* dx_add, const medt_block_saved& sv, float* dx, const medt_block_grads& gr, void* ws,
                    size_t ws_bytes, hipStream_t s);

bool conv_small_ok(const medt_conv_desc& d);
int conv_small_fwd(const medt_conv_desc& d, const float* x, const float* w, const medt_bn_ptrs& bn, const float* res,
                   float* z, float* y, float* partials, hipStream_t s);
bool bn_dgrad1x1_small_ok(const medt_conv_desc& d);
int bn_dgrad1x1_small(const medt_conv_desc& d, const float* dy, const float* y, const float* z, BnStats st,
                      const float* gamma, const float* w, const float* dx_add, float* g, float* dz, float* partials,
                      float* dx, hipStream_t s);
int bn_act_bwd_small(const medt_conv_desc& d, const float* dy, const float* y, const float* z, BnStats st,
                     const float* weight, float* g, float* dz, float* partials, int HoWo, hipStream_t s);
int bn_fin_apply(const float* z, const float* partials, int ppg, double count, const medt_bn_ptrs& bn, float eps, int training,
                 BnStats st, const float* res, float* y, int N, int C, int HW, int groups, int relu, hipStream_t s);
bool conv_fwd_ws_ok(int Cin, int Cout, int K, int stride, long positions);
int bn_chan_threads(const medt_conv_desc& d, int HoWo);
int bn_act_bwd_chan(const medt_conv_desc& d, const float* dy, const float* y, const float* z, BnStats st,
                    const float* weight, float* g, float* dz, float* partials, int HoWo, hipStream_t s);
bool wopos_small_ok(const AxialGeom& g, const medt_axial_desc& d);
int wopos_small_fwd(const AxialGeom& g, const medt_axial_desc& d, const medt_axial_params& p, const float* x, float* y,
                    float* qkv_raw, float* stacked, float* lse, float* part_q, float* part_s, float* part_o,
                    hipStream_t s);
bool wopos_small_bwd_ok(const AxialGeom& g, const medt_axial_desc& d);
int wopos_small_bwd(const AxialGeom& g, const medt_axial_desc& d, const medt_axial_params& p, const float* y,
                    const float* dy, const float* qkv_raw, const float* stacked, const float* lse, BnStats sq, BnStats ss,
                    BnStats so, float* dqkv, float* part_ob, float* part_sb, float* part_qb, float* coef_qkv,
                    hipStream_t s);
int wopos_small_bwd_finalize(const AxialGeom& g, const medt_axial_desc& d, const medt_axial_params& p,
                             const float* part_ob, const float* part_sb, const float* part_qb, BnStats sq, BnStats ss,
                             BnStats so, const medt_axial_grads& gr, hipStream_t s, Queue* q);
bool fast_path_enabled();

// ... 45 lines not shown
```

medical-transformer_amd/csrc/pointwise.hip:

```cpp
#include "defer.h"
#include "fin_inline.h"
#include "sim_tables.h"
#include <type_traits>

namespace medt {

template <int OT>
__global__ __launch_bounds__(MEDT_THREADS) void conv1x1_fwd_kernel(
    const float* __restrict__ x, const float* __restrict__ w, float* __restrict__ y, float* __restrict__ partials,
    int Cin, int Cout, int HW) {
    MEDT_STATIC_SHARED float red[MEDT_WAVES * OT * 2 * 2];
    const int  p  = blockIdx.x * MEDT_THREADS + threadIdx.x;
    const int  n  = blockIdx.y;
    const int  o0 = blockIdx.z * OT;
    const bool ok = p < HW;
    const float* xp = x + (size_t)n * Cin * HW + (ok ? p : 0);
    float acc[OT];
#pragma unroll
    for (int o = 0; o < OT; ++o) acc[o] = 0.f;
    {
        int c = 0;
        for (; c + 8 <= Cin; c += 8) {
            float xr[8];
#pragma unroll
            for (int u = 0; u < 8; ++u) xr[u] = xp[(size_t)(c + u) * HW];
            MEDT_SCHED_FENCE();
#pragma unroll
            for (int u = 0; u < 8; ++u)
#pragma unroll
                for (int o = 0; o < OT; ++o) acc[o] = fmaf(w[(o0 + o) * Cin + c + u], xr[u], acc[o]);
            MEDT_SCHED_FENCE();
        }
        for (; c < Cin; ++c) {
            const float xv = xp[(size_t)c * HW];
#pragma unroll
            for (int o = 0; o < OT; ++o) acc[o] = fmaf(w[(o0 + o) * Cin + c], xv, acc[o]);
        }
    }
    if (ok) {
        float* yp = y + ((size_t)n * Cout + o0) * HW + p;
#pragma unroll
        for (int o = 0; o < OT; ++o) yp[(size_t)o * HW] = acc[o];
    }
    if (partials) {
        float v[2 * OT];
#pragma unroll
        for (int o = 0; o < OT; ++o) { v[2 * o] = acc[o]; v[2 * o + 1] = acc[o] * acc[o]; }
        block_sum_d<2 * OT>(v, red, reinterpret_cast<double*>(partials) + ((size_t)(n * gridDim.x + blockIdx.x) * Cout + o0) * 2);
    }
}

int conv1x1_ptiles(int HW) { return cdiv(HW, MEDT_THREADS); }

int conv1x1_fwd(const float* x, const float* w, float* y, float* partials, int N, int Cin, int Cout, int HW,
                hipStream_t s) {
    const int pt = conv1x1_ptiles(HW);
    if (Cout % 16 == 0) {
        hipLaunchKernelGGL(conv1x1_fwd_kernel<16>, dim3(pt, N, Cout / 16), dim3(MEDT_THREADS), 0, s, x, w, y, partials,
                           Cin, Cout, HW);
    } else if (Cout % 8 == 0) {
        hipLaunchKernelGGL(conv1x1_fwd_kernel<8>, dim3(pt, N, Cout / 8), dim3(MEDT_THREADS), 0, s, x, w, y, partials,
                           Cin, Cout, HW);
    } else if (Cout % 2 == 0) {
        hipLaunchKernelGGL(conv1x1_fwd_kernel<2>, dim3(pt, N, Cout / 2), dim3(MEDT_THREADS), 0, s, x, w, y, partials,
                           Cin, Cout, HW);
    } else {
        hipLaunchKernelGGL(conv1x1_fwd_kernel<1>, dim3(pt, N, Cout), dim3(MEDT_THREADS), 0, s, x, w, y, partials, Cin,
                           Cout, HW);
    }
    return launch_status("conv1x1_fwd");
}

template <int CT>
__global__ __launch_bounds__(MEDT_THREADS) void conv1x1_bwd_data_kernel(
    const float* __restrict__ dy, const float* __restrict__ raw, const float* __restrict__ coef,
    const float* __restrict__ w, float* __restrict__ dx, int N, int Cin, int Cout, int HW, int npg) {
    const long q = (long)blockIdx.x * MEDT_THREADS + threadIdx.x;
    const int  c0 = blockIdx.y * CT;
    const bool ok = q < (long)N * HW;
    const int  n = ok ? (int)(q / HW) : 0, p = ok ? (int)(q - (long)n * HW) : 0;
    const size_t base = (size_t)n * Cout * HW + p;
    const float* cf = coef ? coef + (size_t)(n / npg) * Cout * 3 : nullptr;
    float acc[CT];
#pragma unroll
    for (int c = 0; c < CT; ++c) acc[c] = 0.f;
    auto batch = [&](auto u_tag, auto cf_tag, int o) {
        constexpr int UU = decltype(u_tag)::value;
        constexpr bool CF = decltype(cf_tag)::value;
        float dv[UU], rv[UU], k0[UU], k1[UU], k2[UU];
#pragma unroll
        for (int u = 0; u < UU; ++u) {
            dv[u] = dy[base + (size_t)(o + u) * HW];
            if constexpr (CF) {
                rv[u] = raw[base + (size_t)(o + u) * HW];
                k0[u] = cf[(o + u) * 3 + 0];
                k1[u] = cf[(o + u) * 3 + 1];
                k2[u] = cf[(o + u) * 3 + 2];
            }
        }
        MEDT_SCHED_FENCE();
#pragma unroll
        for (int u = 0; u < UU; ++u) {
            float v = dv[u];
            if constexpr (CF) v = fmaf(k0[u], v, fmaf(k1[u], rv[u], k2[u]));
#pragma unroll
            for (int c = 0; c < CT; ++c) acc[c] = fmaf(w[(o + u) * Cin + c0 + c], v, acc[c]);
        }
        MEDT_SCHED_FENCE();
    };
    {
        int o = 0;
        if (cf) {
            for (; o + 8 <= Cout; o += 8) batch(std::integral_constant<int, 8>{}, std::true_type{}, o);
            for (; o < Cout; ++o) batch(std::integral_constant<int, 1>{}, std::true_type{}, o);
        } else {
            for (; o + 8 <= Cout; o += 8) batch(std::integral_constant<int, 8>{}, std::false_type{}, o);
            for (; o < Cout; ++o) batch(std::integral_constant<int, 1>{}, std::false_type{}, o);
        }
    }
    if (ok) {
        float* dp = dx + ((size_t)n * Cin + c0) * HW + p;
#pragma unroll
        for (int c = 0; c < CT; ++c) dp[(size_t)c * HW] = acc[c];
    }
}

template <int CT>
__global__ __launch_bounds__(MEDT_THREADS) void conv1x1_bwd_data_ws_kernel(
    const float* __restrict__ dy, const float* __restrict__ raw, const float* __restrict__ coef,
    const float* __restrict__ w, float* __restrict__ dx, int N, int Cin, int Cout, int HW, int npg) {
    MEDT_STATIC_SHARED float red[3][CT][64];
    extern __shared__ __attribute__((aligned(16))) float wl[];
    const int lane = threadIdx.x & 63, wv = threadIdx.x >> 6;
    const long q = (long)blockIdx.x * 64 + lane;
    const int  c0 = blockIdx.y * CT;
    for (int e0 = threadIdx.x; e0 < Cout * CT; e0 += 8 * MEDT_THREADS) {
        float v[8];
#pragma unroll
        for (int u = 0; u < 8; ++u) {
            const int e = min(e0 + u * MEDT_THREADS, Cout * CT - 1);
            v[u] = w[(e / CT) * Cin + c0 + (e % CT)];
        }
        MEDT_SCHED_FENCE();
#pragma unroll
        for (int u = 0; u < 8; ++u)
            if (e0 + u * MEDT_THREADS < Cout * CT) wl[e0 + u * MEDT_THREADS] = v[u];
    }
    const bool ok = q < (long)N * HW;
    const int  n = ok ? (int)(q / HW) : 0, p = ok ? (int)(q - (long)n * HW) : 0;
    const size_t base = (size_t)n * Cout * HW + p;
    const float* cf = coef ? coef + (size_t)(n / npg) * Cout * 3 : nullptr;
    const int ob = (Cout * wv) / 4, oe = (Cout * (wv + 1)) / 4;
    float acc[CT];
#pragma unroll
    for (int c = 0; c < CT; ++c) acc[c] = 0.f;
    __syncthreads();
    auto batch = [&](auto u_tag, auto cf_tag, int o) {
        constexpr int UU = decltype(u_tag)::value;
        constexpr bool CF = decltype(cf_tag)::value;
        float dv[UU], rv[UU], k0[UU], k1[UU], k2[UU];
#pragma unroll
        for (int u = 0; u < UU; ++u) {
            dv[u] = dy[base + (size_t)(o + u) * HW];
            if constexpr (CF) {
                rv[u] = raw[base + (size_t)(o + u) * HW];
                k0[u] = cf[(o + u) * 3 + 0];
                k1[u] = cf[(o + u) * 3 + 1];
                k2[u] = cf[(o + u) * 3 + 2];
            }
        }
        MEDT_SCHED_FENCE();
#pragma unroll
        for (int u = 0; u < UU; ++u) {
            float v = dv[u];
            if constexpr (CF) v = fmaf(k0[u], v, fmaf(k1[u], rv[u], k2[u]));
#pragma unroll
            for (int c = 0; c < CT; ++c) acc[c] = fmaf(wl[(o + u) * CT + c], v, acc[c]);
        }
        MEDT_SCHED_FENCE();
    };
    {
        int o = ob;
        if (cf) {
            for (; o + 16 <= oe; o += 16) batch(std::integral_constant<int, 16>{}, std::true_type{}, o);
            for (; o < oe; ++o) batch(std::integral_constant<int, 1>{}, std::true_type{}, o);
        } else {
            for (; o + 16 <= oe; o += 16) batch(std::integral_constant<int, 16>{}, std::false_type{}, o);
            for (; o < oe; ++o) batch(std::integral_constant<int, 1>{}, std::false_type{}, o);
        }
    }
    if (wv > 0) {
#pragma unroll
        for (int c = 0; c < CT; ++c) red[wv - 1][c][lane] = acc[c];
    }
    __syncthreads();
    if (wv == 0 && ok) {
        float* dp = dx + ((size_t)n * Cin + c0) * HW + p;
#pragma unroll
        for (int c = 0; c < CT; ++c) dp[(size_t)c * HW] = acc[c] + (red[0][c][lane] + red[1][c][lane]) + red[2][c][lane];
    }
}

int conv1x1_bwd_data_impl(const float* dy, const float* raw, const float* coef, const float* w, float* dx, int N, int Cin,
                          int Cout, int HW, int groups, hipStream_t s);
int conv1x1_bwd_data(const float* dy, const float* raw, const float* coef, const float* w, float* dx, int N, int Cin,
                     int Cout, int HW, int groups, hipStream_t s) {
    if (abl_skip(groups > 1 ? "qkv_dgrad_l" : "qkv_dgrad_g")) return MEDT_OK;
    return conv1x1_bwd_data_impl(dy, raw, coef, w, dx, N, Cin, Cout, HW, groups, s);
}
int conv1x1_bwd_data_impl(const float* dy, const float* raw, const float* coef, const float* w, float* dx, int N, int Cin,
                     int Cout, int HW, int groups, hipStream_t s) {
    const int npg = N / groups;
    const unsigned gx = (unsigned)(((long)N * HW + MEDT_THREADS - 1) / MEDT_THREADS);
    if ((long)N * HW <= 4096 && Cout >= 64 && Cout <= 768 && Cin % 8 == 0) {
        const unsigned g64 = (unsigned)(((long)N * HW + 63) / 64);
        if (Cin % 16 == 0 && g64 * (Cin / 16) >= 64)
            hipLaunchKernelGGL(conv1x1_bwd_data_ws_kernel<16>, dim3(g64, Cin / 16), dim3(MEDT_THREADS),
                               (size_t)Cout * 16 * sizeof(float), s, dy, raw, coef, w, dx, N, Cin, Cout, HW, npg);
        else
            hipLaunchKernelGGL(conv1x1_bwd_data_ws_kernel<8>, dim3(g64, Cin / 8), dim3(MEDT_THREADS),
                               (size_t)Cout * 8 * sizeof(float), s, dy, raw, coef, w, dx, N, Cin, Cout, HW, npg);
        return launch_status("conv1x1_bwd_data_ws");
    }
    int CT = 16;
    while (CT > 1 && (Cin % CT != 0 || (long)gx * (Cin / CT) < 512)) CT >>= 1;
    while (Cin % CT != 0) CT >>= 1;
#define MEDT_LAUNCH_1X1(T)                                                                                       \
    hipLaunchKernelGGL(conv1x1_bwd_data_kernel<T>, dim3(gx, Cin / T), dim3(MEDT_THREADS), 0, s, dy, raw, coef, w, dx, N, \
                       Cin, Cout, HW, npg)
    switch (CT) {
        case 16: MEDT_LAUNCH_1X1(16); break;
        case 8: MEDT_LAUNCH_1X1(8); break;
        case 4: MEDT_LAUNCH_1X1(4); break;
        case 2: MEDT_LAUNCH_1X1(2); break;
        default: MEDT_LAUNCH_1X1(1); break;
    }
#undef MEDT_LAUNCH_1X1
    return launch_status("conv1x1_bwd_data");
}

__device__ __forceinline__ void reduce_rows_body(const float* __restrict__ in, int P, int K, float* __restrict__ out,
                                                 int block) {
    MEDT_STATIC_SHARED float red[4][64];
    const int k = block * 64 + (threadIdx.x & 63);
    const int slice = threadIdx.x >> 6;
    float s = 0.f;
    if (k < K) {
        float c[16];
#pragma unroll
        for (int u = 0; u < 16; ++u) c[u] = 0.f;
        int p = slice;
        for (; p + 60 < P; p += 64) {
            float t[16];
#pragma unroll
            for (int u = 0; u < 16; ++u) t[u] = in[(size_t)(p + 4 * u) * K + k];
#pragma unroll
            for (int u = 0; u < 16; ++u) c[u] += t[u];
        }
        if (p < P) {
            float t[16];
#pragma unroll
            for (int u = 0; u < 16; ++u) t[u] = in[(size_t)min(p + 4 * u, P - 1) * K + k];
#pragma unroll
            for (int u = 0; u < 16; ++u) c[u] += p + 4 * u < P ? t[u] : 0.f;
        }
#pragma unroll
        for (int w = 8; w > 0; w >>= 1)
#pragma unroll
            for (int u = 0; u < w; ++u) c[u] += c[u + w];
        s = c[0];
    }
    red[slice][threadIdx.x & 63] = s;
    __syncthreads();
    if (slice == 0 && k < K) out[k] = (red[0][threadIdx.x] + red[1][threadIdx.x]) + (red[2][threadIdx.x] + red[3][threadIdx.x]);
}

__global__ __launch_bounds__(MEDT_THREADS) void reduce_rows_kernel(const float* __restrict__ in, int P, int K,
                                                                   float* __restrict__ out) {
    reduce_rows_body(in, P, K, out, blockIdx.x);
}

using RBatch = JobBatch<RJob, 144>;
__global__ __launch_bounds__(MEDT_THREADS) void reduce_rows_grouped_kernel(RBatch b) {
    const int j = find_job(b, blockIdx.x);
    reduce_rows_body(b.job[j].src, b.job[j].P, b.job[j].K, b.job[j].dst, blockIdx.x - b.start[j]);
}

int reduce_rows_grouped(const RJob* jobs, int n, hipStream_t s) {
    for (int i0 = 0; i0 < n; i0 += 144) {
        RBatch b;
        b.n = n - i0 < 144 ? n - i0 : 144;
        int blocks = 0;
        for (int i = 0; i < b.n; ++i) {
            b.job[i] = jobs[i0 + i];
            b.start[i] = blocks;
            blocks += cdiv(jobs[i0 + i].K, 64);
        }
        b.start[b.n] = blocks;
        hipLaunchKernelGGL(reduce_rows_grouped_kernel, dim3(blocks), dim3(MEDT_THREADS), 0, s, b);
        int rc = launch_status("reduce_rows_grouped");
        if (rc) return rc;
    }
    return MEDT_OK;
}

int reduce_rows(const float* in, int P, int K, float* out, hipStream_t s) {
    hipLaunchKernelGGL(reduce_rows_kernel, dim3(cdiv(K, 64)), dim3(MEDT_THREADS), 0, s, in, P, K, out);
    return launch_status("reduce_rows");
}


template <int NV, class T = float>
__device__ __forceinline__ bool group_sums(const T* __restrict__ partials, int ppg, int groups, int CH, int ch,
                                           int stride, const int (&which)[NV], double (&out)[NV]) {
    const int lane = threadIdx.x;
    if (groups > 64 || (groups & (groups - 1))) return false;
    const int slots = 64 / groups, g = lane % groups, slot = lane / groups;
#pragma unroll
    for (int k = 0; k < NV; ++k) out[k] = 0.0;
    for (int p = slot; p < ppg; p += slots) {
        const T* q = partials + ((size_t)(g * ppg + p) * CH + ch) * stride;
#pragma unroll
        for (int k = 0; k < NV; ++k) out[k] += (double)q[which[k]];
    }
    for (int o = groups; o < 64; o <<= 1)
#pragma unroll
        for (int k = 0; k < NV; ++k) out[k] += __shfl_xor(out[k], o, 64);
    return true;
}

__device__ __forceinline__ void bn_finalize_body(int ch, const float* __restrict__ partials_f, int ppg, int groups, int CH,
                                                 double count, const float* __restrict__ weight,
                                                 const float* __restrict__ bias, float* running_mean,
                                                 float* running_var, int64_t* nbt, float momentum, float eps,
                                                 int training, BnStats out) {
    const int lane = threadIdx.x;
    const double* partials = reinterpret_cast<const double*>(partials_f);
    const float g = weight[ch], b = bias[ch];
    if (!training) {
        const float  mean = running_mean[ch];
        const float  rstd = (float)(1.0 / sqrt((double)running_var[ch] + (double)eps));
        for (int grp = lane; grp < groups; grp += 64) {
            out.mean[grp * CH + ch]  = mean;
            out.rstd[grp * CH + ch]  = rstd;
            out.scale[grp * CH + ch] = g * rstd;
            out.shift[grp * CH + ch] = b - mean * g * rstd;
        }
        return;
    }
    const bool save = training != 2;
    double rm = running_mean ? (double)running_mean[ch] : 0.0, rv = running_var ? (double)running_var[ch] : 0.0;
    double sums[2];
    const int which[2] = {0, 1};
    if (group_sums<2, double>(partials, ppg, groups, CH, ch, 2, which, sums)) {
        const double mean = sums[0] / count;
        double var = sums[1] / count - mean * mean;
        if (var < 0.0) var = 0.0;
        const double rstd = 1.0 / sqrt(var + (double)eps);
        if (lane < groups && save) {
            out.mean[lane * CH + ch]  = (float)mean;
            out.rstd[lane * CH + ch]  = (float)rstd;
            out.scale[lane * CH + ch] = (float)(g * rstd);
            out.shift[lane * CH + ch] = (float)(b - mean * g * rstd);
        }
        for (int grp = 0; grp < groups; ++grp) {
            const double m = __shfl(mean, grp, 64), v = __shfl(var, grp, 64);
            rm = (1.0 - momentum) * rm + momentum * m;
            rv = (1.0 - momentum) * rv + momentum * v * (count / (count - 1.0));
        }
    } else {
        for (int grp = 0; grp < groups; ++grp) {
            double s = 0.0, ss = 0.0;
            for (int p = lane; p < ppg; p += 64) {
                const double* q = partials + ((size_t)(grp * ppg + p) * CH + ch) * 2;
                s += q[0];
                ss += q[1];
            }
            s = wave_sum_d(s);
            ss = wave_sum_d(ss);
            const double mean = s / count;
            double var = ss / count - mean * mean;
            if (var < 0.0) var = 0.0;
            const double rstd = 1.0 / sqrt(var + (double)eps);
            if (lane == 0 && save) {
                out.mean[grp * CH + ch]  = (float)mean;
                out.rstd[grp * CH + ch]  = (float)rstd;
                out.scale[grp * CH + ch] = (float)(g * rstd);
                out.shift[grp * CH + ch] = (float)(b - mean * g * rstd);
            }
            rm = (1.0 - momentum) * rm + momentum * mean;
// ... 356 lines not shown
```

medical-transformer_amd/lib/models/axialnet.py:

```python
import math

import torch
import torch.nn as nn
import torch.nn.functional as F

from .utils import qkv_transform

import medt_amd
from medt_amd import net as _net

__all__ = ["AxialAttention", "AxialAttention_dynamic", "AxialAttention_wopos", "AxialBlock", "AxialBlock_dynamic",
           "AxialBlock_wopos", "ResAxialAttentionUNet", "medt_net", "axialunet", "gated", "MedT", "logo", "conv1x1",
           "qkv_transform"]


def conv1x1(in_planes, out_planes, stride=1):
    return nn.Conv2d(in_planes, out_planes, kernel_size=1, stride=stride, bias=False)


class _AxialAttentionBase(nn.Module):
    _has_pos = True
    _gated = False
    _gate_init = (0.1, 0.1, 0.1, 1.0)
    _gate_mode = 0

    def __init__(self, in_planes, out_planes, groups=8, kernel_size=56, stride=1, bias=False, width=False):
        assert (in_planes % groups == 0) and (out_planes % groups == 0)
        super().__init__()
        self.in_planes, self.out_planes, self.groups = in_planes, out_planes, groups
        self.group_planes = out_planes // groups
        self.kernel_size, self.stride, self.bias, self.width = kernel_size, stride, bias, width
        self.bn_groups = 1

        pos = self._has_pos
        self.qkv_transform = qkv_transform(in_planes, out_planes * 2, kernel_size=1, stride=1, padding=0, bias=False)
        self.bn_qkv = nn.BatchNorm1d(out_planes * 2)
        self.bn_similarity = nn.BatchNorm2d(groups * 3 if pos else groups)
        self.bn_output = nn.BatchNorm1d(out_planes * 2 if pos else out_planes)
        if self._gated:
            for name, val in zip(("f_qr", "f_kr", "f_sve", "f_sv"), self._gate_init):
                setattr(self, name, nn.Parameter(torch.tensor(val), requires_grad=False))
        self._gate_modules(in_planes)
        if pos:
            self.relative = nn.Parameter(torch.randn(self.group_planes * 2, kernel_size * 2 - 1), requires_grad=True)
            rows = torch.arange(kernel_size).unsqueeze(1)
            cols = torch.arange(kernel_size).unsqueeze(0)
            self.register_buffer("flatten_index", (rows - cols + kernel_size - 1).view(-1))
        if stride > 1:
            self.pooling = nn.AvgPool2d(stride, stride=stride)
        self.reset_parameters()

    def _gate_modules(self, in_planes):
        pass

    def _gates(self, x):
        return (self.f_qr, self.f_kr, self.f_sve, self.f_sv) if self._gated else None

    def reset_parameters(self):
        self.qkv_transform.weight.data.normal_(0, math.sqrt(1. / self.in_planes))
        if self._has_pos:
            nn.init.normal_(self.relative, 0., math.sqrt(1. / self.group_planes))

    def forward(self, x):
        return self.run(x, self.bn_groups, False)

    def run(self, x, bn_groups=1, out_relu=False, pre=None):
        L = x.shape[3] if self.width else x.shape[2]
        if self._has_pos and L != self.kernel_size:
            raise RuntimeError(f"axial attention built for sequence length {self.kernel_size}, got {L}")
        gates = self._gates(x)
        return medt_amd.axial_attention(
            x, self.qkv_transform.weight, self.bn_qkv, self.bn_similarity, self.bn_output,
            self.relative if self._has_pos else None, gates, self.groups, self.width, self.stride,
            self.training, bn_groups, out_relu, self._gate_mode, pre)


class AxialAttention(_AxialAttentionBase):
    pass


class AxialAttention_dynamic(_AxialAttentionBase):
    _gated = True


class AxialAttention_wopos(_AxialAttentionBase):
    _has_pos = False


class _AxialBlockBase(nn.Module):
    expansion = 2
    _attention = AxialAttention
    _extra_conv1 = False

    def __init__(self, inplanes, planes, stride=1, downsample=None, groups=1, base_width=64, dilation=1,
                 norm_layer=None, kernel_size=56):
        super().__init__()
        if norm_layer is None:
            norm_layer = nn.BatchNorm2d
        width = int(planes * (base_width / 64.))
        self.conv_down = conv1x1(inplanes, width)
        if self._extra_conv1:
            self.conv1 = nn.Conv2d(width, width, kernel_size=1)
        self.bn1 = norm_layer(width)
        self.hight_block = self._attention(width, width, groups=groups, kernel_size=kernel_size)
        self.width_block = self._attention(width, width, groups=groups, kernel_size=kernel_size, stride=stride,
                                           width=True)
        self.conv_up = conv1x1(width, planes * self.expansion)
        self.bn2 = norm_layer(planes * self.expansion)
        self.relu = nn.ReLU(inplace=True)
        self.downsample = downsample
        self.stride = stride

    def forward(self, x):
        return _net.axial_block_forward(self, x)


class AxialBlock(_AxialBlockBase):
    pass


class AxialBlock_dynamic(_AxialBlockBase):
    _attention = AxialAttention_dynamic


class AxialBlock_wopos(_AxialBlockBase):
    _attention = AxialAttention_wopos
    _extra_conv1 = True


class _AxialNetBase(nn.Module):
    def _make_layer(self, block, planes, blocks, kernel_size=56, stride=1, dilate=False):
        norm_layer = self._norm_layer
        downsample = None
        previous_dilation = self.dilation
        if dilate:
            self.dilation *= stride
            stride = 1
        if stride != 1 or self.inplanes != planes * block.expansion:
            downsample = nn.Sequential(conv1x1(self.inplanes, planes * block.expansion, stride),
                                       norm_layer(planes * block.expansion))
        stages = [block(self.inplanes, planes, stride, downsample, groups=self.groups, base_width=self.base_width,
                        dilation=previous_dilation, norm_layer=norm_layer, kernel_size=kernel_size)]
        self.inplanes = planes * block.expansion
        if stride != 1:
            kernel_size = kernel_size // 2
        for _ in range(1, blocks):
            stages.append(block(self.inplanes, planes, groups=self.groups, base_width=self.base_width,
                                dilation=self.dilation, norm_layer=norm_layer, kernel_size=kernel_size))
        return nn.Sequential(*stages)

    def _common_init(self, groups, width_per_group, replace_stride_with_dilation, norm_layer, s):
        if norm_layer is None:
            norm_layer = nn.BatchNorm2d
        self._norm_layer = norm_layer
        self.inplanes = int(64 * s)
        self.dilation = 1
        if replace_stride_with_dilation is None:
            replace_stride_with_dilation = [False, False, False]
        if len(replace_stride_with_dilation) != 3:
            raise ValueError("replace_stride_with_dilation should be None "
                             "or a 3-element tuple, got {}".format(replace_stride_with_dilation))
        self.groups = groups
        self.base_width = width_per_group
        return norm_layer, replace_stride_with_dilation

    def forward(self, x):
        return self._forward_impl(x)


class ResAxialAttentionUNet(_AxialNetBase):
    def __init__(self, block, layers, num_classes=2, zero_init_residual=True, groups=8, width_per_group=64,
                 replace_stride_with_dilation=None, norm_layer=None, s=0.125, img_size=128, imgchan=3):
        super().__init__()
        norm_layer, rswd = self._common_init(groups, width_per_group, replace_stride_with_dilation, norm_layer, s)
        self.conv1 = nn.Conv2d(imgchan, self.inplanes, kernel_size=7, stride=2, padding=3, bias=False)
        self.conv2 = nn.Conv2d(self.inplanes, 128, kernel_size=3, stride=1, padding=1, bias=False)
        self.conv3 = nn.Conv2d(128, self.inplanes, kernel_size=3, stride=1, padding=1, bias=False)
        self.bn1 = norm_layer(self.inplanes)
        self.bn2 = norm_layer(128)
        self.bn3 = norm_layer(self.inplanes)
        self.relu = nn.ReLU(inplace=True)
        self.layer1 = self._make_layer(block, int(128 * s), layers[0], kernel_size=(img_size // 2))
        self.layer2 = self._make_layer(block, int(256 * s), layers[1], stride=2, kernel_size=(img_size // 2),
                                       dilate=rswd[0])
        self.layer3 = self._make_layer(block, int(512 * s), layers[2], stride=2, kernel_size=(img_size // 4),
                                       dilate=rswd[1])
        self.layer4 = self._make_layer(block, int(1024 * s), layers[3], stride=2, kernel_size=(img_size // 8),
                                       dilate=rswd[2])
        self.decoder1 = nn.Conv2d(int(1024 * 2 * s), int(1024 * 2 * s), kernel_size=3, stride=2, padding=1)
        self.decoder2 = nn.Conv2d(int(1024 * 2 * s), int(1024 * s), kernel_size=3, stride=1, padding=1)
        self.decoder3 = nn.Conv2d(int(1024 * s), int(512 * s), kernel_size=3, stride=1, padding=1)
        self.decoder4 = nn.Conv2d(int(512 * s), int(256 * s), kernel_size=3, stride=1, padding=1)
        self.decoder5 = nn.Conv2d(int(256 * s), int(128 * s), kernel_size=3, stride=1, padding=1)
        self.adjust = nn.Conv2d(int(128 * s), num_classes, kernel_size=1, stride=1, padding=0)
        self.soft = nn.Softmax(dim=1)

    def _forward_impl(self, x):
        return _net.unet_forward(self, x)


class medt_net(_AxialNetBase):
    def __init__(self, block, block_2, layers, num_classes=2, zero_init_residual=True, groups=8, width_per_group=64,
                 replace_stride_with_dilation=None, norm_layer=None, s=0.125, img_size=128, imgchan=3):
        super().__init__()
        norm_layer, rswd = self._common_init(groups, width_per_group, replace_stride_with_dilation, norm_layer, s)
        self.conv1 = nn.Conv2d(imgchan, self.inplanes, kernel_size=7, stride=2, padding=3, bias=False)
        self.conv2 = nn.Conv2d(self.inplanes, 128, kernel_size=3, stride=1, padding=1, bias=False)
        self.conv3 = nn.Conv2d(128, self.inplanes, kernel_size=3, stride=1, padding=1, bias=False)
        self.bn1 = norm_layer(self.inplanes)
        self.bn2 = norm_layer(128)
        self.bn3 = norm_layer(self.inplanes)
        self.bn1 = norm_layer(self.inplanes)
        self.relu = nn.ReLU(inplace=True)
        self.layer1 = self._make_layer(block, int(128 * s), layers[0], kernel_size=(img_size // 2))
        self.layer2 = self._make_layer(block, int(256 * s), layers[1], stride=2, kernel_size=(img_size // 2),
                                       dilate=rswd[0])
        self.decoder4 = nn.Conv2d(int(512 * s), int(256 * s), kernel_size=3, stride=1, padding=1)
        self.decoder5 = nn.Conv2d(int(256 * s), int(128 * s), kernel_size=3, stride=1, padding=1)
        self.adjust = nn.Conv2d(int(128 * s), num_classes, kernel_size=1, stride=1, padding=0)
        self.soft = nn.Softmax(dim=1)
        self.conv1_p = nn.Conv2d(imgchan, self.inplanes, kernel_size=7, stride=2, padding=3, bias=False)
        self.conv2_p = nn.Conv2d(self.inplanes, 128, kernel_size=3, stride=1, padding=1, bias=False)
        self.conv3_p = nn.Conv2d(128, self.inplanes, kernel_size=3, stride=1, padding=1, bias=False)
        self.bn1_p = norm_layer(self.inplanes)
        self.bn2_p = norm_layer(128)
        self.bn3_p = norm_layer(self.inplanes)
        self.relu_p = nn.ReLU(inplace=True)
# ... 36 lines not shown
```

medical-transformer_amd/medt_amd/_lib.py:

```python
from __future__ import annotations

import ctypes as C
import os

import torch

from .build import LIB_PATH

_lib = None
ABI_VERSION = 11


class MedtError(RuntimeError):
    pass


class AxialDesc(C.Structure):
    _fields_ = [("N", C.c_int32), ("C", C.c_int32), ("H", C.c_int32), ("W", C.c_int32), ("G", C.c_int32),
                ("axis", C.c_int32), ("has_pos", C.c_int32), ("stride", C.c_int32), ("training", C.c_int32),
                ("bn_groups", C.c_int32), ("eps", C.c_float), ("momentum", C.c_float), ("out_relu", C.c_int32),
                ("gate_mode", C.c_int32), ("act_dtype", C.c_int32)]


class ConvDesc(C.Structure):
    _fields_ = [("N", C.c_int32), ("Cin", C.c_int32), ("H", C.c_int32), ("W", C.c_int32), ("Cout", C.c_int32),
                ("K", C.c_int32), ("stride", C.c_int32), ("pad", C.c_int32), ("has_bias", C.c_int32),
                ("has_bn", C.c_int32), ("has_res", C.c_int32), ("relu", C.c_int32), ("training", C.c_int32),
                ("bn_groups", C.c_int32), ("eps", C.c_float), ("momentum", C.c_float), ("lean", C.c_int32)]


class BnPtrs(C.Structure):
    _fields_ = [("weight", C.c_void_p), ("bias", C.c_void_p), ("running_mean", C.c_void_p),
                ("running_var", C.c_void_p), ("num_batches_tracked", C.c_void_p)]


class AxialParams(C.Structure):
    _fields_ = [("w_qkv", C.c_void_p), ("bn_qkv", BnPtrs), ("bn_similarity", BnPtrs), ("bn_output", BnPtrs),
                ("relative", C.c_void_p), ("f_qr", C.c_void_p), ("f_kr", C.c_void_p), ("f_sve", C.c_void_p),
                ("f_sv", C.c_void_p)]


class AxialSaved(C.Structure):
    _fields_ = [("qkv_raw", C.c_void_p), ("stacked", C.c_void_p), ("lse", C.c_void_p), ("stats", C.c_void_p)]


class AxialGrads(C.Structure):
    _fields_ = [("w_qkv", C.c_void_p), ("bn_qkv_weight", C.c_void_p), ("bn_qkv_bias", C.c_void_p),
                ("bn_sim_weight", C.c_void_p), ("bn_sim_bias", C.c_void_p), ("bn_out_weight", C.c_void_p),
                ("bn_out_bias", C.c_void_p), ("relative", C.c_void_p), ("gates", C.c_void_p)]


class BlockDesc(C.Structure):
    _fields_ = [("N", C.c_int32), ("C", C.c_int32), ("width", C.c_int32), ("H", C.c_int32), ("W", C.c_int32),
                ("G", C.c_int32), ("training", C.c_int32), ("bn_groups", C.c_int32), ("eps", C.c_float),
                ("momentum", C.c_float)]


class BlockParams(C.Structure):
    _fields_ = [("w_down", C.c_void_p), ("bn1", BnPtrs), ("height", AxialParams), ("width", AxialParams),
                ("w_up", C.c_void_p), ("bn2", BnPtrs)]


class BlockSaved(C.Structure):
    _fields_ = [("z1", C.c_void_p), ("y1", C.c_void_p), ("stats1", C.c_void_p), ("height", AxialSaved),
                ("y_h", C.c_void_p), ("width", AxialSaved), ("y_w", C.c_void_p), ("z2", C.c_void_p),
                ("stats2", C.c_void_p)]


class BlockS2Params(C.Structure):
    _fields_ = [("blk", BlockParams), ("w_ds", C.c_void_p), ("bn_ds", BnPtrs)]


class BlockS2Saved(C.Structure):
    _fields_ = [("blk", BlockSaved), ("zd", C.c_void_p), ("yd", C.c_void_p), ("statsd", C.c_void_p)]


class BlockGrads(C.Structure):
    _fields_ = [("w_down", C.c_void_p), ("bn1_weight", C.c_void_p), ("bn1_bias", C.c_void_p), ("height", AxialGrads),
                ("width", AxialGrads), ("w_up", C.c_void_p), ("bn2_weight", C.c_void_p), ("bn2_bias", C.c_void_p)]


SIGNATURES = {
    "medt_abi_version": (C.c_int, []),
    "medt_last_error": (C.c_char_p, []),
    "medt_queue_create": (C.c_void_p, []),
    "medt_queue_destroy": (C.c_int, [C.c_void_p]),
    "medt_queue_bind": (C.c_int, [C.c_void_p, C.c_void_p]),
    "medt_queue_pending": (C.c_size_t, [C.c_void_p]),
    "medt_queue_flush": (C.c_int, [C.c_void_p, C.c_void_p]),
    "medt_queue_flush2": (C.c_int, [C.c_void_p, C.c_void_p, C.c_void_p]),
    "medt_queue_discard": (C.c_int, [C.c_void_p]),
    "medt_axial_stats_floats": (C.c_size_t, [C.POINTER(AxialDesc)]),
    "medt_axial_workspace_bytes": (C.c_size_t, [C.POINTER(AxialDesc)]),
    "medt_axial_layer_fwd": (C.c_int, [C.POINTER(AxialDesc), C.POINTER(AxialParams), C.c_void_p, C.c_void_p,
                                       C.POINTER(AxialSaved), C.c_void_p, C.c_size_t, C.c_void_p]),
    "medt_axial_layer_bwd": (C.c_int, [C.POINTER(AxialDesc), C.POINTER(AxialParams), C.c_void_p, C.c_void_p, C.c_void_p,
                                       C.POINTER(AxialSaved), C.c_void_p, C.POINTER(AxialGrads), C.c_void_p,
                                       C.c_size_t, C.c_void_p]),
    "medt_axial_core_stats": (C.c_int, [C.POINTER(AxialDesc), C.POINTER(AxialParams), C.POINTER(AxialSaved),
                                        C.c_void_p, C.c_size_t, C.c_void_p]),
    "medt_axial_core_fwd": (C.c_int, [C.POINTER(AxialDesc), C.POINTER(AxialParams), C.POINTER(AxialSaved),
                                      C.c_void_p, C.c_size_t, C.c_void_p]),
    "medt_axial_core_bwd": (C.c_int, [C.POINTER(AxialDesc), C.POINTER(AxialParams), C.POINTER(AxialSaved), C.c_void_p,
                                      C.c_void_p, C.c_size_t, C.c_void_p]),
    "medt_wopos_block_workspace_bytes": (C.c_size_t, [C.POINTER(BlockDesc)]),
    "medt_wopos_block_fwd": (C.c_int, [C.POINTER(BlockDesc), C.POINTER(BlockParams), C.c_void_p, C.c_void_p,
                                       C.POINTER(BlockSaved), C.c_void_p, C.c_size_t, C.c_void_p]),
    "medt_wopos_block_s2_workspace_bytes": (C.c_size_t, [C.POINTER(BlockDesc)]),
    "medt_wopos_block_s2_fwd": (C.c_int, [C.POINTER(BlockDesc), C.POINTER(BlockS2Params), C.c_void_p, C.c_void_p,
                                          C.POINTER(BlockS2Saved), C.c_void_p, C.c_size_t, C.c_void_p]),
    "medt_wopos_block_bwd_workspace_bytes": (C.c_size_t, [C.POINTER(BlockDesc)]),
    "medt_wopos_block_bwd": (C.c_int, [C.POINTER(BlockDesc), C.POINTER(BlockParams), C.c_void_p, C.c_void_p, C.c_void_p,
                                       C.POINTER(BlockSaved), C.c_void_p, C.c_void_p, C.POINTER(BlockGrads), C.c_void_p,
                                       C.c_size_t, C.c_void_p]),
    "medt_conv_stats_floats": (C.c_size_t, [C.POINTER(ConvDesc)]),
    "medt_conv_workspace_bytes": (C.c_size_t, [C.POINTER(ConvDesc)]),
    "medt_conv_block_fwd": (C.c_int, [C.POINTER(ConvDesc), C.c_void_p, C.c_void_p, C.c_void_p, C.POINTER(BnPtrs),
                                      C.c_void_p, C.c_void_p, C.c_void_p, C.c_void_p, C.c_void_p, C.c_size_t, C.c_void_p]),
    "medt_conv_block_bwd": (C.c_int, [C.POINTER(ConvDesc), C.c_void_p, C.c_void_p, C.POINTER(BnPtrs), C.c_void_p,
                                      C.c_void_p, C.c_void_p, C.c_void_p, C.c_void_p, C.c_void_p, C.c_void_p, C.c_void_p,
                                      C.c_void_p, C.c_void_p, C.c_void_p, C.c_void_p, C.c_size_t, C.c_void_p]),
    "medt_gate_mlp_fwd": (C.c_int, [C.c_void_p] * 9 + [C.c_int] * 5 + [C.c_void_p]),
    "medt_gate_mlp_bwd": (C.c_int, [C.c_void_p] * 13 + [C.c_int] * 5 + [C.c_void_p]),
    "medt_up2x_relu_add_fwd": (C.c_int, [C.c_void_p, C.c_void_p, C.c_void_p, C.c_int, C.c_int, C.c_int, C.c_void_p]),
    "medt_up2x_relu_bwd": (C.c_int, [C.c_void_p, C.c_void_p, C.c_void_p, C.c_int, C.c_int, C.c_int, C.c_void_p]),
    "medt_patch_gather": (C.c_int, [C.c_void_p, C.c_void_p, C.c_int, C.c_int, C.c_int, C.c_int, C.c_int, C.c_void_p]),
    "medt_logo_merge_fwd": (C.c_int, [C.c_void_p, C.c_void_p, C.c_void_p, C.c_int, C.c_int, C.c_int, C.c_int, C.c_int,
                                      C.c_void_p]),
    "medt_logo_merge_bwd": (C.c_int, [C.c_void_p, C.c_void_p, C.c_void_p, C.c_int, C.c_int, C.c_int, C.c_int, C.c_int,
                                      C.c_void_p]),
    "medt_ce_partials": (C.c_size_t, [C.c_int, C.c_int]),
    "medt_ce_fwd": (C.c_int, [C.c_void_p, C.c_void_p, C.c_void_p, C.c_void_p, C.c_int, C.c_int, C.c_int, C.c_int,
                              C.c_void_p]),
    "medt_ce_bwd": (C.c_int, [C.c_void_p, C.c_void_p, C.c_void_p, C.c_void_p, C.c_void_p, C.c_int, C.c_int, C.c_int,
                              C.c_int, C.c_void_p]),
    "medt_seg_loss_workspace": (C.c_size_t, [C.c_int, C.c_int, C.c_int]),
    "medt_seg_loss_out_floats": (C.c_size_t, [C.c_int, C.c_int]),
    "medt_seg_loss_fwd": (C.c_int, [C.c_void_p] * 5 + [C.c_int] * 4 + [C.c_float] * 3 + [C.c_void_p]),
    "medt_seg_loss_bwd": (C.c_int, [C.c_void_p] * 6 + [C.c_int] * 4 + [C.c_float] * 3 + [C.c_void_p]),
    "medt_adam_step": (C.c_int, [C.c_void_p, C.c_void_p, C.c_void_p, C.c_void_p, C.c_void_p, C.c_size_t, C.c_float,
                                 C.c_float, C.c_float, C.c_float, C.c_float, C.c_float, C.c_void_p]),
    "medt_relu_mask": (C.c_int, [C.c_void_p, C.c_void_p, C.c_void_p, C.c_size_t, C.c_void_p]),
    "medt_seg_counts": (C.c_int, [C.c_void_p, C.c_void_p, C.c_void_p, C.c_int, C.c_int, C.c_int, C.c_float, C.c_void_p]),
    "medt_window_gather": (C.c_int, [C.c_void_p] * 4 + [C.c_int] * 6 + [C.c_void_p]),
    "medt_window_blend": (C.c_int, [C.c_void_p] * 5 + [C.c_int] * 6 + [C.c_float, C.c_void_p]),
    "medt_augment_param_floats": (C.c_size_t, []),
    "medt_augment_workspace": (C.c_size_t, [C.c_int, C.c_int, C.c_int]),
    "medt_augment_stats": (C.c_int, [C.c_void_p] * 3 + [C.c_int] * 6 + [C.c_void_p]),
    "medt_augment_apply": (C.c_int, [C.c_void_p] * 6 + [C.c_int] * 7 + [C.c_void_p]),
    "medt_edt_cols": (C.c_int, [C.c_void_p] * 2 + [C.c_int] * 4 + [C.c_void_p]),
    "medt_edt_rows": (C.c_int, [C.c_void_p] * 3 + [C.c_int] * 3 + [C.c_void_p]),
    "medt_label_workspace_bytes": (C.c_size_t, [C.c_int] * 3),
    "medt_label_components": (C.c_int, [C.c_void_p] * 4 + [C.c_size_t] + [C.c_int] * 5 + [C.c_void_p]),
    "medt_label_tables": (C.c_int, [C.c_void_p] * 3 + [C.c_int] * 5 + [C.c_void_p]),
    "medt_label_select": (C.c_int, [C.c_void_p] * 4 + [C.c_int] * 4 + [C.c_void_p]),
}


def lib():
    global _lib
    if _lib is None:
        if not os.path.exists(LIB_PATH):
            raise MedtError(f"{LIB_PATH} not found: build it with `python __graft_entry__.py` "
                            "(hipcc --offload-arch=gfx950); there is no CPU / eager fallback")
        l = C.CDLL(os.environ.get("MEDT_LIB_OVERRIDE", LIB_PATH))
        for name, (res, args) in SIGNATURES.items():
            fn = getattr(l, name)
            fn.restype = res
            fn.argtypes = args
        if l.medt_abi_version() != ABI_VERSION:
            raise MedtError("libmedt_hip.so ABI version mismatch")
        _lib = l
    return _lib


def check(rc: int, what: str):
    if rc != 0:
        raise MedtError(f"{what} failed ({rc}): {lib().medt_last_error().decode()}")


def ptr(t):
    return None if t is None else t.data_ptr()
```

medical-transformer_amd/medt_amd/axial.py:

```python
from __future__ import annotations

import ctypes as C
from typing import Optional

import torch

from . import _lib as L
from . import optim as OPT
from . import defer as DEFER


ACT_BF16 = False


def set_activation_dtype(dtype) -> None:
    global ACT_BF16
    if dtype in (torch.bfloat16, "bf16", "bfloat16"):
        ACT_BF16 = True
    elif dtype in (torch.float32, "f32", "fp32", "float32"):
        ACT_BF16 = False
    else:
        raise L.MedtError(f"activation storage dtype {dtype!r} unsupported (float32 or bfloat16)")


class AxialConfig:
    __slots__ = ("groups", "axis", "has_pos", "stride", "bn_groups", "eps", "momentum",
                 "bn_qkv", "bn_similarity", "bn_output", "out_relu", "gate_mode", "act_dtype", "pre")

    def __init__(self, groups, axis, has_pos, stride, bn_qkv, bn_similarity, bn_output, bn_groups=1,
                 eps=1e-5, momentum=0.1, out_relu=False, gate_mode=0):
        self.groups, self.axis, self.has_pos, self.stride = groups, axis, has_pos, stride
        self.gate_mode = gate_mode
        self.act_dtype = 1 if (ACT_BF16 and has_pos) else 0
        self.bn_groups, self.eps, self.momentum, self.out_relu = bn_groups, eps, momentum, out_relu
        self.bn_qkv, self.bn_similarity, self.bn_output = bn_qkv, bn_similarity, bn_output
        self.pre = None


def _require_device(x: torch.Tensor):
    if not x.is_cuda:
        raise L.MedtError("medt_amd runs on MI355X only: got a CPU tensor and there is no CPU fallback "
                          "(the CPU restatement under oracle/ is test infrastructure)")
    if x.dtype != torch.float32:
        raise L.MedtError(f"medt_amd: float32 activations expected, got {x.dtype}")


def _momentum(bn) -> float:
    if bn.momentum is None:
        raise L.MedtError("BatchNorm momentum=None (cumulative moving average) is not implemented by the HIP kernels; "
                          "the reference uses the default 0.1 everywhere")
    return float(bn.momentum)


def _bn_ptrs(bn, training: bool) -> L.BnPtrs:
    track = bn.running_mean is not None
    return L.BnPtrs(L.ptr(bn.weight), L.ptr(bn.bias),
                    L.ptr(bn.running_mean) if track else None, L.ptr(bn.running_var) if track else None,
                    L.ptr(bn.num_batches_tracked) if (track and training) else None)


def _desc(x, cfg: AxialConfig, training: bool) -> L.AxialDesc:
    N, Cc, H, W = x.shape
    return L.AxialDesc(N, Cc, H, W, cfg.groups, cfg.axis, int(cfg.has_pos), cfg.stride, int(training),
                       cfg.bn_groups, cfg.eps, cfg.momentum, int(cfg.out_relu), int(cfg.gate_mode), int(cfg.act_dtype))


def _params(cfg, w_qkv, relative, gates, training) -> L.AxialParams:
    g = [L.ptr(t) for t in gates] if gates is not None else [None] * 4
    return L.AxialParams(L.ptr(w_qkv), _bn_ptrs(cfg.bn_qkv, training), _bn_ptrs(cfg.bn_similarity, training),
                         _bn_ptrs(cfg.bn_output, training), L.ptr(relative), g[0], g[1], g[2], g[3])


class AxialAttentionFn(torch.autograd.Function):

    @staticmethod
    def forward(ctx, x, w_qkv, bnq_w, bnq_b, bns_w, bns_b, bno_w, bno_b, relative, f_qr, f_kr, f_sve, f_sv,
                cfg: AxialConfig, training: bool):
        _require_device(x)
        lib = L.lib()
        x = x.contiguous()
        N, Cc, H, W = x.shape
        desc = _desc(x, cfg, training)
        gates = None if f_qr is None else (f_qr, f_kr, f_sve, f_sv)
        params = _params(cfg, w_qkv, relative, gates, training)
        OC = 2 * Cc if cfg.has_pos else Cc
        dev = x.device
        sdt = torch.bfloat16 if cfg.act_dtype == 1 else torch.float32
        if cfg.pre is not None:
            qkv_raw, stacked, lse, stats, y = cfg.pre
            cfg.pre = None
        else:
            qkv_raw = torch.empty((N, 2 * Cc, H, W), device=dev, dtype=sdt)
            stacked = torch.empty((N, OC, H, W), device=dev, dtype=sdt)
            lse = torch.empty((N, cfg.groups, H, W), device=dev, dtype=torch.float32)
            nstats = lib.medt_axial_stats_floats(C.byref(desc))
            if nstats == 0:
                raise L.MedtError("axial attention: " + lib.medt_last_error().decode())
            stats = torch.empty((nstats,), device=dev, dtype=torch.float32)
            ws_bytes = lib.medt_axial_workspace_bytes(C.byref(desc))
            ws = torch.empty((ws_bytes,), device=dev, dtype=torch.uint8)
            y = torch.empty((N, Cc, H // cfg.stride, W // cfg.stride), device=dev, dtype=torch.float32)
            saved = L.AxialSaved(qkv_raw.data_ptr(), stacked.data_ptr(), lse.data_ptr(), stats.data_ptr())
            stream = torch.cuda.current_stream().cuda_stream
            q = DEFER.recording()
            L.check(lib.medt_axial_layer_fwd(C.byref(desc), C.byref(params), x.data_ptr(), y.data_ptr(), C.byref(saved),
                                             ws.data_ptr(), ws_bytes, stream), "medt_axial_layer_fwd")
            if q is not None:
                q.hold(ws, stats)
        ctx.cfg, ctx.training, ctx.has_gates = cfg, training, gates is not None
        ctx.slots = tuple(OPT.grad_slot(t) if t is not None else None
                          for t in (w_qkv, bnq_w, bnq_b, bns_w, bns_b, bno_w, bno_b, relative))
        ctx.gate_slots = tuple(OPT.grad_slot(t) for t in gates) if gates is not None else None
        ctx.save_for_backward(x, w_qkv, relative, f_qr, f_kr, f_sve, f_sv, qkv_raw, stacked, lse, stats,
                              y if cfg.out_relu else None)
        return y

    @staticmethod
    def backward(ctx, dy):
        lib = L.lib()
        x, w_qkv, relative, f_qr, f_kr, f_sve, f_sv, qkv_raw, stacked, lse, stats, y = ctx.saved_tensors
        cfg, training = ctx.cfg, ctx.training
        dy = dy.contiguous()
        desc = _desc(x, cfg, training)
        gates = (f_qr, f_kr, f_sve, f_sv) if ctx.has_gates else None
        params = _params(cfg, w_qkv, relative, gates, False)
        dev = x.device
        Cc = x.shape[1]
        SC = (3 if cfg.has_pos else 1) * cfg.groups
        OC = (2 if cfg.has_pos else 1) * Cc
        sizes = [2 * Cc * Cc, 2 * Cc, 2 * Cc, SC, SC, OC, OC, relative.numel() if relative is not None else 0]
        shapes = [w_qkv.shape, None, None, None, None, None, None, relative.shape if relative is not None else None]
        dst, ret, pend, need_tmp = [None] * 8, [None] * 8, [], []
        for k in range(8):
            if sizes[k] == 0:
                continue
            slot = OPT.live(ctx.slots[k])
            if slot is not None and ctx.needs_input_grad[k + 1]:
                dst[k], direct = OPT.claim(slot)
                if not direct:
                    pend.append((slot, dst[k]))
            else:
                need_tmp.append(k)
        want_gates = ctx.has_gates and any(ctx.needs_input_grad[9:13])
        gate_direct = False
        n_gate = f_qr.numel() if (ctx.has_gates and cfg.gate_mode == 2) else 4
        if want_gates and cfg.gate_mode != 2:
            gs = tuple(OPT.live(g_) for g_ in ctx.gate_slots)
            if all(g_ is not None for g_ in gs) and all(ctx.needs_input_grad[9:13]) and \
                    all(gs[i + 1].view.data_ptr() == gs[i].view.data_ptr() + 4 for i in range(3)) and \
                    all(g_.stamp != g_.owner.stamp for g_ in gs):
                for g_ in gs:
                    OPT.claim(g_)
                gate_direct = True
        tmp_sizes = [sizes[k] for k in need_tmp] + ([n_gate] if (want_gates and not gate_direct) else [])
        if tmp_sizes:
            parts = list(torch.split(torch.empty((sum(tmp_sizes),), device=dev, dtype=torch.float32), tmp_sizes))
            for k, part in zip(need_tmp, parts):
                dst[k] = part
                if ctx.needs_input_grad[k + 1]:
                    ret[k] = part.view(shapes[k]) if shapes[k] is not None else part
        if want_gates:
            gate_ptr = gs[0].view.data_ptr() if gate_direct else parts[-1].data_ptr()
        else:
            gate_ptr = None
        dx = torch.empty_like(x)
        grads = L.AxialGrads(*[L.ptr(t) for t in dst], gate_ptr)
        saved = L.AxialSaved(qkv_raw.data_ptr(), stacked.data_ptr(), lse.data_ptr(), stats.data_ptr())
        ws_bytes = lib.medt_axial_workspace_bytes(C.byref(desc))
        ws = torch.empty((ws_bytes,), device=dev, dtype=torch.uint8)
        stream = torch.cuda.current_stream().cuda_stream
        q = DEFER.recording(allow=not pend and all(r is None for r in ret) and (not want_gates or gate_direct))
        L.check(lib.medt_axial_layer_bwd(C.byref(desc), C.byref(params), x.data_ptr(), L.ptr(y), dy.data_ptr(), C.byref(saved),
                                         dx.data_ptr(), C.byref(grads), ws.data_ptr(), ws_bytes, stream),
                "medt_axial_layer_bwd")
        if q is not None:
            q.hold(ws, x, qkv_raw, stats, *dst)
            if tmp_sizes:
                q.hold(*parts)
        for slot, tmp in pend:
            OPT.accumulate(slot, tmp)
        if want_gates and cfg.gate_mode == 2:
            dg = [parts[-1].view_as(f_qr), None, None, None]
        elif want_gates and not gate_direct:
            gg = parts[-1]
            dg = [gg[i].reshape(()) if ctx.needs_input_grad[9 + i] else None for i in range(4)]
        else:
            dg = [None] * 4
        return (dx, ret[0], ret[1], ret[2], ret[3], ret[4], ret[5], ret[6], ret[7], dg[0], dg[1], dg[2], dg[3],
                None, None)


def axial_attention(x, qkv_weight, bn_qkv, bn_similarity, bn_output, relative: Optional[torch.Tensor],
                    gates, groups: int, width: bool, stride: int, training: bool, bn_groups: int = 1,
                    out_relu: bool = False, gate_mode: int = 0, pre=None):
    cfg = AxialConfig(groups, 1 if width else 0, relative is not None, stride, bn_qkv, bn_similarity, bn_output,
                      bn_groups, bn_qkv.eps, _momentum(bn_qkv), out_relu, gate_mode)
    cfg.pre = pre
    g = gates if gates is not None else (None, None, None, None)
    return AxialAttentionFn.apply(x, qkv_weight, bn_qkv.weight, bn_qkv.bias, bn_similarity.weight,
                                  bn_similarity.bias, bn_output.weight, bn_output.bias, relative,
                                  g[0], g[1], g[2], g[3], cfg, training)
```

medical-transformer_amd/medt_amd/net.py:

```python
from __future__ import annotations

import torch

from ._lib import MedtError
from . import ops
from . import defer as DEFER
from . import block as BLOCK

import os

PATCH = 32
GRID = 4
TWO_STREAMS = os.environ.get("MEDT_TWO_STREAMS", "1") != "0"
SINKS = os.environ.get("MEDT_GRAD_SINKS", "1") != "0"
EARLY_FIN = os.environ.get("MEDT_EARLY_FIN", "1") != "0"
_side = {}


def _side_stream(device):
    key = (device.type, device.index)
    if key not in _side:
        _side[key] = torch.cuda.Stream(device=device)
    return _side[key]


def join_side_stream(device):
    side = _side.get((device.type, device.index))
    if side is not None:
        torch.cuda.current_stream().wait_stream(side)


def _require_device(x):
    if not x.is_cuda:
        raise MedtError("medt_amd runs on MI355X only: got a CPU tensor and there is no CPU fallback "
                        "(the CPU restatement under oracle/ is test infrastructure)")


def axial_block_forward(blk, x, bn_groups: int = 1):
    _require_device(x)
    sink = ops.sink_of(x) if (SINKS and x.requires_grad) else None
    if BLOCK.BWD_ENABLED:
        y = BLOCK.block_forward(blk, x, bn_groups, sink)
        if y is not None:
            return y
    pre = BLOCK.fused_forward(blk, x, bn_groups)
    if pre is None:
        pre = {"down": None, "h": None, "w": None, "up": None}
    pre.setdefault("ds", None)
    out = ops.conv_block(x, blk.conv_down, blk.bn1, relu=True, training=blk.bn1.training, bn_groups=bn_groups,
                         x_sink=sink, x_role="final", pre=pre["down"])
    out = blk.hight_block.run(out, bn_groups, False, pre["h"])
    out = blk.width_block.run(out, bn_groups, True, pre["w"])
    if blk.downsample is not None:
        identity = ops.conv_block(x, blk.downsample[0], blk.downsample[1], relu=False,
                                  training=blk.downsample[1].training, bn_groups=bn_groups, x_sink=sink, x_role="deposit",
                                  pre=pre["ds"])
        return ops.conv_block(out, blk.conv_up, blk.bn2, res=identity, relu=True, training=blk.bn2.training,
                              bn_groups=bn_groups, pre=pre["up"])
    return ops.conv_block(out, blk.conv_up, blk.bn2, res=x, relu=True, training=blk.bn2.training,
                          bn_groups=bn_groups, res_sink=sink, pre=pre["up"])


def _layer(seq, x, bn_groups=1):
    for blk in seq:
        x = axial_block_forward(blk, x, bn_groups)
    return x


def _stem(net, x, sfx="", bn_groups=1, first_of_branch=False):
    g = lambda n: getattr(net, n + sfx)
    for i in ("1", "2", "3"):
        bn = g("bn" + i)
        x = ops.conv_block(x, g("conv" + i), bn, relu=True, training=bn.training, bn_groups=bn_groups,
                           last_of_branch=first_of_branch and i == "1")
    return x


def _unet_body(net, x, sfx="", bn_groups=1):
    g = lambda n: getattr(net, n + sfx)
    x1 = _layer(g("layer1"), x, bn_groups)
    x2 = _layer(g("layer2"), x1, bn_groups)
    x3 = _layer(g("layer3"), x2, bn_groups)
    x4 = _layer(g("layer4"), x3, bn_groups)
    sk = (lambda t: ops.sink_of(t)) if SINKS else (lambda t: None)
    y = ops.up2x_relu_add(ops.conv_block(x4, g("decoder1")), x4)
    y = ops.up2x_relu_add(ops.conv_block(y, g("decoder2")), x3, sk(x3))
    y = ops.up2x_relu_add(ops.conv_block(y, g("decoder3")), x2, sk(x2))
    y = ops.up2x_relu_add(ops.conv_block(y, g("decoder4")), x1, sk(x1))
    y = ops.up2x_relu_add(ops.conv_block(y, g("decoder5")), None)
    return y


def unet_forward(net, x):
    _require_device(x)
    y = _unet_body(net, _stem(net, x.contiguous()))
    return ops.conv_block(y, net.adjust)


def medt_forward(net, x):
    _require_device(x)
    xin = x.contiguous()
    if xin.shape[2] < PATCH * GRID or xin.shape[3] < PATCH * GRID or xin.shape[2] != xin.shape[3]:
        raise RuntimeError(f"medt_net needs square images of at least {PATCH * GRID} px (4x4 grid of 32-px patches)")
    main = torch.cuda.current_stream()
    side = _side_stream(xin.device) if TWO_STREAMS else None
    if side is not None:
        side.wait_stream(main)
    DEFER.set_aux_stream(side)
    g = _stem(net, xin, first_of_branch=side is not None)
    x1 = _layer(net.layer1, g)
    x2 = _layer(net.layer2, x1)
    y = ops.up2x_relu_add(ops.conv_block(x2, net.decoder4), x1, ops.sink_of(x1) if SINKS else None)
    y = ops.up2x_relu_add(ops.conv_block(y, net.decoder5), None)
    if side is not None and EARLY_FIN:
        DEFER.flush_current_stream()
    groups = GRID * GRID
    ops.set_lean(side is not None and xin.shape[2] * xin.shape[3] > 128 * 128)
    try:
        if side is not None:
            with torch.cuda.stream(side):
                xp = ops.patch_gather(xin, PATCH, GRID)
                yp = _unet_body(net, _stem(net, xp, "_p", groups), "_p", groups)
                if EARLY_FIN:
                    joined = torch.cuda.Event()
                    joined.record(side)
                    DEFER.flush_current_stream()
            if EARLY_FIN:
                main.wait_event(joined)
            else:
                main.wait_stream(side)
            yp.record_stream(main)
        else:
            xp = ops.patch_gather(xin, PATCH, GRID)
            yp = _unet_body(net, _stem(net, xp, "_p", groups), "_p", groups)
    finally:
        ops.set_lean(False)
    y = ops.logo_merge(y, yp, PATCH, GRID)
    y = ops.conv_block(y, net.decoderf, relu=True)
    return ops.conv_block(y, net.adjust)
```

medical-transformer_amd/medt_amd/ops.py:

```python
from __future__ import annotations

import ctypes as C
import os

import torch

from . import _lib as L
from . import optim as OPT
from . import defer as DEFER
from .axial import _bn_ptrs, _momentum, _require_device


def _stream():
    return torch.cuda.current_stream().cuda_stream


class GradSink:
    __slots__ = ("pending", "closed")

    def __init__(self):
        self.pending, self.closed = None, False

    def deposit(self, t) -> bool:
        if self.closed or self.pending is not None:
            return False
        self.pending = t
        return True

    def take(self):
        t, self.pending = self.pending, None
        return t


def sink_of(x):
    s = getattr(x, "_medt_sink", None)
    if s is None:
        s = x._medt_sink = GradSink()
    return s


import threading
_hint = threading.local()


def set_lean(v: bool):
    _hint.lean = bool(v)


def lean() -> bool:
    return getattr(_hint, "lean", False)



class ConvBlockCfg:
    __slots__ = ("stride", "pad", "bn", "relu", "bn_groups", "x_sink", "x_role", "res_sink", "last_of_branch", "pre", "lean")

    def __init__(self, stride, pad, bn, relu, bn_groups=1, x_sink=None, x_role=None, res_sink=None, last_of_branch=False,
                 pre=None):
        self.stride, self.pad, self.bn, self.relu, self.bn_groups = stride, pad, bn, relu, bn_groups
        self.x_sink, self.x_role, self.res_sink = x_sink, x_role, res_sink
        self.last_of_branch = last_of_branch
        self.pre = pre
        self.lean = lean()


def _conv_desc(x, w, cfg: ConvBlockCfg, has_bias, has_res, training) -> L.ConvDesc:
    N, Cin, H, W = x.shape
    bn = cfg.bn
    return L.ConvDesc(N, Cin, H, W, w.shape[0], w.shape[2], cfg.stride, cfg.pad, int(has_bias), int(bn is not None),
                      int(has_res), int(cfg.relu), int(training), cfg.bn_groups,
                      bn.eps if bn is not None else 1e-5,
                      _momentum(bn) if bn is not None else 0.1, int(cfg.lean))


class ConvBlockFn(torch.autograd.Function):
    @staticmethod
    def forward(ctx, x, w, bias, bn_w, bn_b, res, cfg: ConvBlockCfg, training: bool):
        _require_device(x)
        lib = L.lib()
        x = x.contiguous()
        if res is not None:
            res = res.contiguous()
        desc = _conv_desc(x, w, cfg, bias is not None, res is not None, training)
        K, s, p = w.shape[2], cfg.stride, cfg.pad
        N, _, H, W = x.shape
        Ho, Wo = (H + 2 * p - K) // s + 1, (W + 2 * p - K) // s + 1
        has_bn = cfg.bn is not None
        if cfg.pre is not None:
            z, y, stats = cfg.pre
            cfg.pre = None
        else:
            y = torch.empty((N, w.shape[0], Ho, Wo), device=x.device, dtype=torch.float32)
            z = torch.empty_like(y) if has_bn else y
            stats = torch.empty((max(lib.medt_conv_stats_floats(C.byref(desc)), 1),), device=x.device, dtype=torch.float32)
            ws_bytes = lib.medt_conv_workspace_bytes(C.byref(desc))
            if ws_bytes == 0:
                raise L.MedtError("conv block: " + lib.medt_last_error().decode())
            ws = torch.empty((ws_bytes,), device=x.device, dtype=torch.uint8)
            bnp = _bn_ptrs(cfg.bn, training) if has_bn else None
            q = DEFER.recording() if (has_bn or stats.numel() > 1) else None
            L.check(lib.medt_conv_block_fwd(C.byref(desc), x.data_ptr(), w.data_ptr(), L.ptr(bias),
                                            C.byref(bnp) if has_bn else None, L.ptr(res), z.data_ptr(), y.data_ptr(),
                                            stats.data_ptr(), ws.data_ptr(), ws_bytes, _stream()), "medt_conv_block_fwd")
            if q is not None:
                q.hold(ws, stats)
        ctx.cfg, ctx.training, ctx.has_bias, ctx.has_res = cfg, training, bias is not None, res is not None
        ctx.slots = tuple(OPT.grad_slot(t) if t is not None else None for t in (w, bias, bn_w, bn_b))
        ctx.save_for_backward(x, w, z if has_bn else None, y if (cfg.relu or has_bn) else None,
                              stats if (has_bn or stats.numel() > 1) else None)
        return y

    @staticmethod
    def backward(ctx, dy):
        lib = L.lib()
        x, w, z, y, stats = ctx.saved_tensors
        cfg, training = ctx.cfg, ctx.training
        dy = dy.contiguous()
        desc = _conv_desc(x, w, cfg, ctx.has_bias, ctx.has_res, training)
        has_bn = cfg.bn is not None
        dev = x.device
        Cout = w.shape[0]
        need_dx = ctx.needs_input_grad[0]
        dx = torch.empty_like(x) if need_dx else None
        xs = cfg.x_sink if need_dx else None
        dep = xs.take() if xs is not None else None
        dx_add = dep if (dep is not None and w.shape[2] == 1) else None
        present = (True, ctx.has_bias, has_bn, has_bn)
        shapes = (w.shape, (Cout,), (Cout,), (Cout,))
        dst, ret, pend = [None] * 4, [None] * 4, []
        for k in range(4):
            if not present[k]:
                continue
            slot = OPT.live(ctx.slots[k])
            if slot is not None and ctx.needs_input_grad[k + 1]:
                dst[k], direct = OPT.claim(slot)
                if not direct:
                    pend.append((slot, dst[k]))
            else:
                dst[k] = torch.empty(shapes[k], device=dev, dtype=torch.float32)
                if ctx.needs_input_grad[k + 1]:
                    ret[k] = dst[k]
        dres = torch.empty_like(dy) if ctx.has_res else None
        ws_bytes = lib.medt_conv_workspace_bytes(C.byref(desc))
        ws = torch.empty((ws_bytes,), device=dev, dtype=torch.uint8)
        bnp = _bn_ptrs(cfg.bn, False) if has_bn else None
        q = DEFER.recording(allow=not pend and all(r is None for r in ret))
        L.check(lib.medt_conv_block_bwd(C.byref(desc), x.data_ptr(), w.data_ptr(), C.byref(bnp) if has_bn else None,
                                        L.ptr(z), L.ptr(y), L.ptr(stats), dy.data_ptr(), L.ptr(dx), dst[0].data_ptr(),
                                        L.ptr(dst[1]), L.ptr(dst[2]), L.ptr(dst[3]), L.ptr(dres), L.ptr(dx_add), ws.data_ptr(),
                                        ws_bytes, _stream()), "medt_conv_block_bwd")
        if q is not None:
            q.hold(ws, x, dy, stats, dres, *dst)
        for slot, tmp in pend:
            OPT.accumulate(slot, tmp)
        if dep is not None and dx_add is None:
            dx.add_(dep)
        if xs is not None:
            if cfg.x_role == "final":
                xs.closed = True
            elif xs.deposit(dx):
                dx = None
        if dres is not None and cfg.res_sink is not None and cfg.res_sink.deposit(dres):
            dres = None
        if cfg.last_of_branch:
            if DEFER.flush_current_stream():
                OPT.branch_done(0)
        return (dx, ret[0], ret[1], ret[2], ret[3], dres, None, None)


def conv_block(x, conv, bn=None, res=None, relu=False, training=False, bn_groups=1, x_sink=None, x_role=None,
               res_sink=None, last_of_branch=False, pre=None):
    cfg = ConvBlockCfg(conv.stride[0], conv.padding[0], bn, relu, bn_groups if bn is not None else 1, x_sink, x_role,
                       res_sink, last_of_branch, pre)
    if bn is None:
        training = torch.is_grad_enabled() and (x.requires_grad or conv.weight.requires_grad)
    return ConvBlockFn.apply(x, conv.weight, conv.bias, bn.weight if bn is not None else None,
                             bn.bias if bn is not None else None, res, cfg, training)


class UpReluAddFn(torch.autograd.Function):
    @staticmethod
    def forward(ctx, x, skip, skip_sink=None):
        ctx.skip_sink = skip_sink
        _require_device(x)
        lib = L.lib()
        x = x.contiguous()
        N, Cc, H, W = x.shape
        y = torch.empty((N, Cc, 2 * H, 2 * W), device=x.device, dtype=torch.float32)
        if skip is not None:
            skip = skip.contiguous()
        L.check(lib.medt_up2x_relu_add_fwd(x.data_ptr(), L.ptr(skip), y.data_ptr(), N * Cc, H, W, _stream()),
                "medt_up2x_relu_add_fwd")
        ctx.save_for_backward(x)
        ctx.has_skip = skip is not None
        return y

    @staticmethod
    def backward(ctx, dy):
        lib = L.lib()
        (x,) = ctx.saved_tensors
        dy = dy.contiguous()
        N, Cc, H, W = x.shape
        dx = torch.empty_like(x)
        L.check(lib.medt_up2x_relu_bwd(x.data_ptr(), dy.data_ptr(), dx.data_ptr(), N * Cc, H, W, _stream()),
                "medt_up2x_relu_bwd")
        dskip = dy if ctx.has_skip else None
        if dskip is not None and ctx.skip_sink is not None and ctx.skip_sink.deposit(dskip):
            dskip = None
        return dx, dskip, None


def up2x_relu_add(x, skip=None, skip_sink=None):
    return UpReluAddFn.apply(x, skip, skip_sink)


class GateMlpFn(torch.autograd.Function):

    @staticmethod
    def forward(ctx, x, w1, b1, w2, b2, axis):
        _require_device(x)
        lib = L.lib()
        x = x.contiguous()
        N, Cc, H, W = x.shape
        nseq = N * (H if axis else W)
        dev = x.device
        xn = torch.empty((nseq, Cc), device=dev, dtype=torch.float32)
        h = torch.empty_like(xn)
        o = torch.empty((nseq, 4), device=dev, dtype=torch.float32)
        gates = torch.empty_like(o)
        L.check(lib.medt_gate_mlp_fwd(x.data_ptr(), w1.data_ptr(), b1.data_ptr(), w2.data_ptr(), b2.data_ptr(),
                                      xn.data_ptr(), h.data_ptr(), o.data_ptr(), gates.data_ptr(), N, Cc, H, W, axis,
                                      _stream()), "medt_gate_mlp_fwd")
        ctx.save_for_backward(w1, w2, xn, h, o, gates)
        ctx.geom = (N, Cc, H, W, axis)
        return gates

    @staticmethod
    def backward(ctx, dgates):
        lib = L.lib()
        w1, w2, xn, h, o, gates = ctx.saved_tensors
        N, Cc, H, W, axis = ctx.geom
        dev = dgates.device
        nseq = gates.shape[0]
        dgates = dgates.contiguous()
        scratch = torch.empty((nseq * (4 + 2 * Cc),), device=dev, dtype=torch.float32)
        dw1, db1 = torch.empty_like(w1), torch.empty((Cc,), device=dev, dtype=torch.float32)
        dw2, db2 = torch.empty_like(w2), torch.empty((4,), device=dev, dtype=torch.float32)
        dx = torch.empty((N, Cc, H, W), device=dev, dtype=torch.float32)
        L.check(lib.medt_gate_mlp_bwd(dgates.data_ptr(), gates.data_ptr(), o.data_ptr(), h.data_ptr(), xn.data_ptr(),
                                      w1.data_ptr(), w2.data_ptr(), scratch.data_ptr(), dw1.data_ptr(), db1.data_ptr(),
                                      dw2.data_ptr(), db2.data_ptr(), dx.data_ptr(), N, Cc, H, W, axis, _stream()),
                "medt_gate_mlp_bwd")
        return dx, dw1, db1, dw2, db2, None


def gate_mlp(x, fcn1, fcn2, width: bool):
    return GateMlpFn.apply(x, fcn1.weight, fcn1.bias, fcn2.weight, fcn2.bias, 1 if width else 0)


def patch_gather(x, P=32, G=4):
    _require_device(x)
    x = x.contiguous()
    N, Cc, S, _ = x.shape
    xp = torch.empty((G * G * N, Cc, P, P), device=x.device, dtype=torch.float32)
    L.check(L.lib().medt_patch_gather(x.data_ptr(), xp.data_ptr(), N, Cc, S, P, G, _stream()), "medt_patch_gather")
    return xp


class LogoMergeFn(torch.autograd.Function):
    @staticmethod
    def forward(ctx, x, yp, P, G):
        _require_device(x)
        x, yp = x.contiguous(), yp.contiguous()
        N, Cc, S, _ = x.shape
        y = torch.empty_like(x)
        L.check(L.lib().medt_logo_merge_fwd(x.data_ptr(), yp.data_ptr(), y.data_ptr(), N, Cc, S, P, G, _stream()),
                "medt_logo_merge_fwd")
        ctx.geom = (N, Cc, S, P, G)
        return y

    @staticmethod
    def backward(ctx, dy):
        N, Cc, S, P, G = ctx.geom
        dy = dy.contiguous()
        dx = torch.empty_like(dy)
        dyp = torch.empty((G * G * N, Cc, P, P), device=dy.device, dtype=torch.float32)
        L.check(L.lib().medt_logo_merge_bwd(dy.data_ptr(), dx.data_ptr(), dyp.data_ptr(), N, Cc, S, P, G, _stream()),
                "medt_logo_merge_bwd")
        return dx, dyp, None, None


def logo_merge(x, yp, P=32, G=4):
    return LogoMergeFn.apply(x, yp, P, G)


class CrossEntropyFn(torch.autograd.Function):
    @staticmethod
    def forward(ctx, logits, target, ignore_index):
        _require_device(logits)
        lib = L.lib()
        logits, target = logits.contiguous(), target.contiguous()
        if target.dtype != torch.int64:
            raise L.MedtError("cross_entropy: int64 class-index targets expected")
        N, K = logits.shape[0], logits.shape[1]
        HW = logits[0, 0].numel()
        partials = torch.empty((lib.medt_ce_partials(N, HW),), device=logits.device, dtype=torch.float32)
        out = torch.empty((3,), device=logits.device, dtype=torch.float32)
        L.check(lib.medt_ce_fwd(logits.data_ptr(), target.data_ptr(), partials.data_ptr(), out.data_ptr(), N, K, HW,
                                ignore_index, _stream()), "medt_ce_fwd")
        ctx.save_for_backward(logits, target, out)
        ctx.ignore_index = ignore_index
        loss = out[0]
        ctx.mark_non_differentiable(out)
        ctx.set_materialize_grads(False)
        return loss, out

    @staticmethod
    def backward(ctx, dloss, _dout):
        if dloss is None:
            return None, None, None
        lib = L.lib()
        logits, target, out = ctx.saved_tensors
        N, K = logits.shape[0], logits.shape[1]
        HW = logits[0, 0].numel()
        dloss = dloss.contiguous().float()
        dlogits = torch.empty_like(logits)
# ... 321 lines not shown
```

Baseline: 2148 images/s.

## Hand off output-BN backward stats from producer 1x1 bwd-data to next axial layer

Adds a backward handoff so the 1x1 conv backward-data kernel of the layer downstream (conv_up or width axial) computes, in its epilogue, the output-BN gradient statistics and relative-position tables that the next axial layer's backward would otherwise compute in a separate pass. The receiving axial layer skips its axial_out_bwd_stats launch and finalizes from the handed-over partials. This removes one kernel and a re-read of dy and the stacked activations per axial layer in the local/global branch blocks, at the cost of more complex cross-layer plumbing and tighter eligibility conditions. It is disabled for the global stem and the first two layers, and can be turned off with MEDT_BWD_HANDOFF=0.

```diff
diff --git a/include/medt_abi.h b/include/medt_abi.h
--- a/include/medt_abi.h
+++ b/include/medt_abi.h
@@ -88,6 +88,23 @@
                          const float* dy, const medt_axial_saved*, float* dx, const medt_axial_grads*,
                          void* workspace, size_t workspace_bytes, void* stream);
 
+typedef struct medt_bwd_handoff {
+    medt_axial_desc consumer;
+    const void*  stacked;
+    const float* stats;
+    const float* relative;
+    const float* ymask;
+    void*        buf;
+    size_t       buf_bytes;
+    int32_t      rows;
+    int32_t      tables;
+} medt_bwd_handoff;
+size_t medt_bwd_handoff_bytes(const medt_axial_desc* consumer);
+int medt_axial_layer_bwd_handoff(const medt_axial_desc*, const medt_axial_params*, const float* x, const float* y,
+                                 const float* dy, const medt_axial_saved*, float* dx, const medt_axial_grads*,
+                                 const medt_bwd_handoff* take, medt_bwd_handoff* give,
+                                 void* workspace, size_t workspace_bytes, void* stream);
+
 int medt_axial_core_stats(const medt_axial_desc*, const medt_axial_params*, const medt_axial_saved*,
                           void* workspace, size_t workspace_bytes, void* stream);
 int medt_axial_core_fwd(const medt_axial_desc*, const medt_axial_params*, const medt_axial_saved*,
@@ -172,6 +189,11 @@
                         const float* z, const float* y, const float* stats, const float* dy,
                         float* dx, float* dw, float* dbias, float* dbn_weight, float* dbn_bias, float* dres,
                         const float* dx_add, void* workspace, size_t workspace_bytes, void* stream);
+int medt_conv_block_bwd_handoff(const medt_conv_desc*, const float* x, const float* w, const medt_bn_ptrs* bn,
+                                const float* z, const float* y, const float* stats, const float* dy,
+                                float* dx, float* dw, float* dbias, float* dbn_weight, float* dbn_bias, float* dres,
+                                const float* dx_add, medt_bwd_handoff* give,
+                                void* workspace, size_t workspace_bytes, void* stream);
 
 int medt_gate_mlp_fwd(const float* x, const float* w1, const float* b1, const float* w2, const float* b2, float* xn, float* h,
                       float* o, float* gates, int N, int C, int H, int W, int axis, void* stream);
diff --git a/medical-transformer_amd/csrc/conv.hip b/medical-transformer_amd/csrc/conv.hip
--- a/medical-transformer_amd/csrc/conv.hip
+++ b/medical-transformer_amd/csrc/conv.hip
@@ -480,6 +480,10 @@
 static bool conv_bwd_data_ws_enabled() {
     static const bool on = true;
     return on;
+}
+
+bool conv2d_bwd_data_1x1_ws(int N, int H, int W, int Cout) {
+    return (long)N * H * W <= 4096 && Cout >= 64 && conv_bwd_data_ws_enabled() && (size_t)Cout * sizeof(float) <= 48 * 1024;
 }
 
 template <int K>
diff --git a/medical-transformer_amd/csrc/medt_api.hip b/medical-transformer_amd/csrc/medt_api.hip
--- a/medical-transformer_amd/csrc/medt_api.hip
+++ b/medical-transformer_amd/csrc/medt_api.hip
@@ -195,6 +195,55 @@
     return MEDT_OK;
 }
 
+static bool handoff_enabled() {
+    static const bool on = [] { const char* e = getenv("MEDT_BWD_HANDOFF"); return !(e && e[0] == '0'); }();
+    return on;
+}
+static size_t handoff_rows_bytes(const AxialGeom& g) {
+    return align_up((size_t)conv2d_parts_per_group(g.N, g.groups, g.HW) * g.OC * 2 * sizeof(float), 256);
+}
+static size_t handoff_bytes(const AxialGeom& g) { return handoff_rows_bytes(g) + align_up(sim_tables_floats(g) * sizeof(float), 256) + 256; }
+static float* handoff_tables(const AxialGeom& g, void* buf) { return (float*)((char*)buf + handoff_rows_bytes(g)); }
+
+static bool handoff_consumer_ok(const medt_axial_desc& cd, const AxialGeom& g) {
+    if (!handoff_enabled() || cd.stride != 1 || wopos_small_bwd_ok(g, cd) || g.OC / g.C > 2) return false;
+    Carver c(nullptr, 0);
+    const BwdWs w(c, g, cd.stride, cd.out_relu, cd.gate_mode);
+    return w.sweep && ((long)(g.N / g.groups) * g.HW) % MEDT_THREADS == 0 &&
+           inline_fin_ok(cd.training ? 1 : 0, g.groups, conv2d_parts_per_group(g.N, g.groups, g.HW));
+}
+
+static bool handoff_fill(medt_bwd_handoff* h, int N, int Cin, int H, int W, int Cout, StatsEpi* e) {
+    h->rows = 0;
+    h->tables = 0;
+    if (!h->stacked || !h->stats || !h->buf) return false;
+    const medt_axial_desc& cd = h->consumer;
+    AxialGeom g;
+    if (cd.N != N || cd.C != Cin || cd.H != H || cd.W != W || axial_geom(cd, &g) || !handoff_consumer_ok(cd, g)) return false;
+    Carver c(nullptr, 0);
+    const BwdWs w(c, g, cd.stride, cd.out_relu, cd.gate_mode);
+    if ((cd.out_relu && !h->ymask) || h->buf_bytes < handoff_bytes(g)) return false;
+    const int tr = cd.training ? 1 : 0, ppg = conv2d_parts_per_group(g.N, g.groups, g.HW);
+    long blocks = 0;
+    if (conv1x1_bwd_data_ws(N, Cin, Cout, H * W, &blocks)) return false;
+    const int rows = ppg;
+    if (!inline_fin_ok(tr, g.groups, rows)) return false;
+    const bool tables = g.pos && inline_fin_ok(tr, g.groups, w.plan.nparts) && axial_out_bwd_stats_tables_ok(cd, sim_tables_blocks(g), g.L);
+    if (tables && (!h->relative || sim_tables_blocks(g) > blocks || g.L > 128)) return false;
+    const LayerStats st(const_cast<float*>(h->stats), g);
+    e->stk = (const float*)h->stacked;
+    e->mean = st.out.mean;
+    e->rstd = st.out.rstd;
+    e->ymask = cd.out_relu ? h->ymask : nullptr;
+    e->partials = (float*)h->buf;
+    e->OC = g.OC;
+    e->bf16 = g.bf16;
+    e->tj = tables ? TablesJob{h->relative, handoff_tables(g, h->buf), g.hq, g.L, sim_tables_blocks(g)} : TablesJob{nullptr, nullptr, 0, 0, 0};
+    h->rows = rows;
+    h->tables = tables ? 1 : 0;
+    return true;
+}
+
 }
 
 using namespace medt;
@@ -330,9 +379,16 @@
     return axial_out_fwd(*d, stacked, st.out, y, s, out_inl ? &out_src : nullptr);
 }
 
-int medt_axial_layer_bwd(const medt_axial_desc* d, const medt_axial_params* p, const float* x, const float* y,
-                         const float* dy, const medt_axial_saved* sv, float* dx, const medt_axial_grads* gr, void* ws,
-                         size_t ws_bytes, void* stream) {
+size_t medt_bwd_handoff_bytes(const medt_axial_desc* consumer) {
+    AxialGeom g;
+    if (!consumer || axial_geom(*consumer, &g)) return 0;
+    return handoff_consumer_ok(*consumer, g) ? handoff_bytes(g) : 0;
+}
+
+static int axial_layer_bwd_impl(const medt_axial_desc* d, const medt_axial_params* p, const float* x, const float* y,
+                                const float* dy, const medt_axial_saved* sv, float* dx, const medt_axial_grads* gr, void* ws,
+                                size_t ws_bytes, void* stream, const medt_bwd_handoff* take, medt_bwd_handoff* give) {
+    if (give) { give->rows = 0; give->tables = 0; }
     AxialGeom g;
     int rc = check_common(d, p, sv, &g);
     if (rc) return rc;
@@ -352,6 +408,16 @@
     GatePtrs gates;
     if ((rc = effective_gates(d, p, w.gate_eff, s, &gates))) return rc;
     const int tr = d->training ? 1 : 0, ppg = conv2d_parts_per_group(g.N, g.groups, g.HW), TL = 2 * g.L - 1;
+    const bool taken = take && take->rows > 0;
+    if (taken) {
+        if (!handoff_consumer_ok(*d, g) || !take->buf || take->buf_bytes < handoff_bytes(g) || take->rows != ppg) {
+            set_error("axial bwd: this layer cannot take handed-over statistics (%d rows)", take->rows);
+            return MEDT_EINVAL;
+        }
+        w.part_ob = (float*)take->buf;
+        if (take->tables) w.tables = handoff_tables(g, take->buf);
+    }
+    const int ob_rows = taken ? take->rows : ppg;
     if (wopos_small_bwd_ok(g, *d)) {
         if ((rc = wopos_small_bwd(g, *d, *p, y, dy, qkv_raw, stacked, sv->lse, st.qkv, st.sim, st.out, w.dqkv,
                                   w.part_ob, w.part_sb, w.part_qb, w.coef_qkv, s))) return rc;
@@ -373,16 +439,17 @@
         }
     }
     const float out_dscale = 1.f / (float)(d->stride * d->stride);
-    const bool sim_inl = w.sweep && g.pos && inline_fin_ok(tr, g.groups, w.plan.nparts) &&
-                         axial_out_bwd_stats_tables_ok(*d, sim_tables_blocks(g), g.L);
+    const bool sim_inl = taken ? take->tables != 0
+                               : w.sweep && g.pos && inline_fin_ok(tr, g.groups, w.plan.nparts) &&
+                                     axial_out_bwd_stats_tables_ok(*d, sim_tables_blocks(g), g.L);
     const TablesJob btj{p->relative, w.tables, g.hq, g.L, sim_tables_blocks(g)};
-    if ((rc = axial_out_bwd_stats(*d, stacked, dy, st.out, w.part_ob, s, sim_inl ? &btj : nullptr, ymask))) return rc;
+    if (!taken && (rc = axial_out_bwd_stats(*d, stacked, dy, st.out, w.part_ob, s, sim_inl ? &btj : nullptr, ymask))) return rc;
     BfinSrc ob = no_bfin_src();
-    if (w.sweep && inline_fin_ok(tr, g.groups, ppg)) {
-        ob.j = BfinJob{w.part_ob, ppg, g.groups, g.OC, tr, g.row_count, out_dscale, st.out, p->bn_output.weight, w.coef_out,
+    if (w.sweep && inline_fin_ok(tr, g.groups, ob_rows)) {
+        ob.j = BfinJob{w.part_ob, ob_rows, g.groups, g.OC, tr, g.row_count, out_dscale, st.out, p->bn_output.weight, w.coef_out,
                        gr->bn_out_weight, gr->bn_out_bias};
         ob.on = 1;
-    } else if ((rc = bn_bwd_finalize(w.part_ob, ppg, g.groups, g.OC, g.row_count, out_dscale, st.out, p->bn_output.weight, tr,
+    } else if ((rc = bn_bwd_finalize(w.part_ob, ob_rows, g.groups, g.OC, g.row_count, out_dscale, st.out, p->bn_output.weight, tr,
                                      w.coef_out, gr->bn_out_weight, gr->bn_out_bias, s))) return rc;
     BfinSrc qb = no_bfin_src();
     if (w.sweep && (!g.bf16 || w.raw32) && inline_fin_ok(tr, g.groups, w.qb_rpg)) {
@@ -412,7 +479,9 @@
             bq_coef = nullptr;
         }
     }
-    if ((rc = conv1x1_bwd_data(w.dqkv, bq_raw, bq_coef, p->w_qkv, dx, g.N, g.C, 2 * g.C, g.HW, g.groups, s)))
+    StatsEpi epi;
+    const bool gave = give && handoff_fill(give, g.N, g.C, g.H, g.W, 2 * g.C, &epi);
+    if ((rc = conv1x1_bwd_data(w.dqkv, bq_raw, bq_coef, p->w_qkv, dx, g.N, g.C, 2 * g.C, g.HW, g.groups, s, gave ? &epi : nullptr)))
         return rc;
     Queue* q = queue_for(s);
     if ((rc = conv2d_bwd_weight(w.dqkv, bq_raw, bq_coef, x, gr->w_qkv, w.dw_scratch, g.N, g.C, g.H, g.W, 2 * g.C, 1,
@@ -437,6 +506,18 @@
     return MEDT_OK;
 }
 
+int medt_axial_layer_bwd(const medt_axial_desc* d, const medt_axial_params* p, const float* x, const float* y,
+                         const float* dy, const medt_axial_saved* sv, float* dx, const medt_axial_grads* gr, void* ws,
+                         size_t ws_bytes, void* stream) {
+    return axial_layer_bwd_impl(d, p, x, y, dy, sv, dx, gr, ws, ws_bytes, stream, nullptr, nullptr);
+}
+
+int medt_axial_layer_bwd_handoff(const medt_axial_desc* d, const medt_axial_params* p, const float* x, const float* y,
+                                 const float* dy, const medt_axial_saved* sv, float* dx, const medt_axial_grads* gr,
+                                 const medt_bwd_handoff* take, medt_bwd_handoff* give, void* ws, size_t ws_bytes, void* stream) {
+    return axial_layer_bwd_impl(d, p, x, y, dy, sv, dx, gr, ws, ws_bytes, stream, take, give);
+}
+
 
 }
 
@@ -567,10 +648,11 @@
     return bn_finalize(cw.partials, g.ppg, d->bn_groups, d->Cout, count, *bn, d->momentum, d->eps, 2, st, s);
 }
 
-int medt_conv_block_bwd(const medt_conv_desc* d, const float* x, const float* w, const medt_bn_ptrs* bn, const float* z,
-                        const float* y, const float* stats, const float* dy, float* dx, float* dw, float* dbias,
-                        float* dbn_weight, float* dbn_bias, float* dres, const float* dx_add, void* ws, size_t ws_bytes,
-                        void* stream) {
+static int conv_block_bwd_impl(const medt_conv_desc* d, const float* x, const float* w, const medt_bn_ptrs* bn, const float* z,
+                               const float* y, const float* stats, const float* dy, float* dx, float* dw, float* dbias,
+                               float* dbn_weight, float* dbn_bias, float* dres, const float* dx_add, void* ws, size_t ws_bytes,
+                               void* stream, medt_bwd_handoff* give) {
+    if (give) { give->rows = 0; give->tables = 0; }
     ConvGeom g;
     int rc = conv_geom(d, &g);
     if (rc) return rc;
@@ -620,6 +702,14 @@
         grad_out = dy;
     }
     const bool preflipped = stats && conv_preflip(d);
+    StatsEpi epi;
+    if (give && dx && !dx_done && !dx_add && d->K == 1 && d->stride == 1 && d->pad == 0 &&
+        !conv_use_mfma(d->Cout, d->Cin, 1, 1, (long)d->N * d->H * d->W) &&
+        conv2d_bwd_data_1x1_ws(d->N, d->H, d->W, d->Cout) == conv1x1_bwd_data_ws(d->N, d->Cin, d->Cout, d->H * d->W) &&
+        handoff_fill(give, d->N, d->Cin, d->H, d->W, d->Cout, &epi)) {
+        if ((rc = conv1x1_bwd_data(grad_out, nullptr, nullptr, w, dx, d->N, d->Cin, d->Cout, d->H * d->W, 1, s, &epi))) return rc;
+        dx_done = true;
+    }
     if (dx && !dx_done && (rc = conv2d_bwd_data(grad_out, w, dx, preflipped ? conv_preflip_ptr(d, const_cast<float*>(stats)) : cw.wt, cw.ksplit_bwd,
                                                 d->N, d->Cin, d->H, d->W, d->Cout, d->K, d->stride, d->pad, s, dx_add, preflipped))) return rc;
     Queue* q = queue_for(s);
@@ -632,6 +722,22 @@
     }
     return conv2d_bwd_weight(grad_out, nullptr, nullptr, x, dw, cw.dw_scratch, d->N, d->Cin, d->H, d->W, d->Cout, d->K, d->stride,
                              d->pad, 1, s, q);
+}
+
+int medt_conv_block_bwd(const medt_conv_desc* d, const float* x, const float* w, const medt_bn_ptrs* bn, const float* z,
+                        const float* y, const float* stats, const float* dy, float* dx, float* dw, float* dbias,
+                        float* dbn_weight, float* dbn_bias, float* dres, const float* dx_add, void* ws, size_t ws_bytes,
+                        void* stream) {
+    return conv_block_bwd_impl(d, x, w, bn, z, y, stats, dy, dx, dw, dbias, dbn_weight, dbn_bias, dres, dx_add, ws, ws_bytes, stream,
+                               nullptr);
+}
+
+int medt_conv_block_bwd_handoff(const medt_conv_desc* d, const float* x, const float* w, const medt_bn_ptrs* bn, const float* z,
+                                const float* y, const float* stats, const float* dy, float* dx, float* dw, float* dbias,
+                                float* dbn_weight, float* dbn_bias, float* dres, const float* dx_add, medt_bwd_handoff* give, void* ws,
+                                size_t ws_bytes, void* stream) {
+    return conv_block_bwd_impl(d, x, w, bn, z, y, stats, dy, dx, dw, dbias, dbn_weight, dbn_bias, dres, dx_add, ws, ws_bytes, stream,
+                               give);
 }
 
 size_t medt_wopos_block_workspace_bytes(const medt_block_desc* d) {
diff --git a/medical-transformer_amd/csrc/medt_kernels.h b/medical-transformer_amd/csrc/medt_kernels.h
--- a/medical-transformer_amd/csrc/medt_kernels.h
+++ b/medical-transformer_amd/csrc/medt_kernels.h
@@ -8,8 +8,10 @@
 int conv1x1_ptiles(int HW);
 int conv1x1_fwd(const float* x, const float* w, float* y, float* partials,
                 int N, int Cin, int Cout, int HW, hipStream_t s);
+struct StatsEpi;
 int conv1x1_bwd_data(const float* dy, const float* raw, const float* coef, const float* w, float* dx,
-                     int N, int Cin, int Cout, int HW, int groups, hipStream_t s);
+                     int N, int Cin, int Cout, int HW, int groups, hipStream_t s, const StatsEpi* epi = nullptr);
+bool conv1x1_bwd_data_ws(int N, int Cin, int Cout, int HW, long* blocks = nullptr);
 struct TablesJob { const float* relative; float* tables; int HQ, L, blocks; };
 int bn_finalize(const float* partials, int parts_per_group, int groups, int CH, double count,
                 const medt_bn_ptrs& bn, float momentum, float eps, int training, BnStats out, hipStream_t s,
@@ -32,6 +34,14 @@
 bool axial_out_bwd_stats_tables_ok(const medt_axial_desc& d, int blocks, int L);
 int axial_out_bwd_stats(const medt_axial_desc& d, const float* stacked, const float* dy, BnStats st,
                         float* partials, hipStream_t s, const TablesJob* tj = nullptr, const float* ymask = nullptr);
+struct StatsEpi {
+    const float* stk;
+    const float *mean, *rstd;
+    const float* ymask;
+    float* partials;
+    int OC, bf16;
+    TablesJob tj;
+};
 
 int reduce_rows(const float* in, int P, int K, float* out, hipStream_t s);
 
@@ -51,6 +61,7 @@
 size_t conv2d_fwd_scratch_floats(int N, int groups, int Cin, int H, int W, int Cout, int K, int stride, int pad);
 int conv2d_bwd_data(const float* dy, const float* w, float* dx, float* wt_scratch, float* ksplit_scratch, int N, int Cin,
                     int H, int W, int Cout, int K, int stride, int pad, hipStream_t s, const float* add = nullptr, bool wt_ready = false);
+bool conv2d_bwd_data_1x1_ws(int N, int H, int W, int Cout);
 bool conv2d_bwd_data_flips(int N, int Cin, int H, int W, int Cout, int K, int stride, int pad);
 int conv_flip_weights(const float* w, float* wt, int Cout, int Cin, int K, hipStream_t s);
 size_t conv2d_bwd_data_scratch_floats(int N, int Cin, int H, int W, int Cout, int K, int stride, int pad);
diff --git a/medical-transformer_amd/csrc/pointwise.hip b/medical-transformer_amd/csrc/pointwise.hip
--- a/medical-transformer_amd/csrc/pointwise.hip
+++ b/medical-transformer_amd/csrc/pointwise.hip
@@ -71,10 +71,48 @@
     return launch_status("conv1x1_fwd");
 }
 
-template <int CT>
+template <int CT, int PER, bool BF>
+__device__ __forceinline__ void stats_epilogue_load(const StatsEpi& e, bool ok, int n, int p, int c0, int Cin, int HW,
+                                                    float (&sx)[CT * PER], float (&ym)[CT]) {
+    constexpr int bf16 = BF ? 1 : 0;
+#pragma unroll
+    for (int c = 0; c < CT; ++c) {
+        ym[c] = (ok && e.ymask) ? e.ymask[((size_t)n * Cin + c0 + c) * HW + p] : 1.f;
+#pragma unroll
+        for (int t = 0; t < PER; ++t)
+            sx[c * PER + t] = ok ? ld_act(e.stk, ((size_t)n * e.OC + (c0 + c) * PER + t) * HW + p, bf16) : 0.f;
+    }
+}
+template <int CT, int PER>
+__device__ __forceinline__ void stats_epilogue(const StatsEpi& e, const float (&dxv)[CT], const float (&sx)[CT * PER],
+                                               const float (&ym)[CT], bool ok, int c0, float* red) {
+    float v[CT * PER * 2];
+#pragma unroll
+    for (int c = 0; c < CT; ++c) {
+        float d = dxv[c];
+        if (e.ymask) d = ym[c] > 0.f ? d : 0.f;
+#pragma unroll
+        for (int t = 0; t < PER; ++t) {
+            const int ch = (c0 + c) * PER + t;
+            const float xh = (sx[c * PER + t] - e.mean[ch]) * e.rstd[ch];
+            v[(c * PER + t) * 2] = ok ? d : 0.f;
+            v[(c * PER + t) * 2 + 1] = ok ? d * xh : 0.f;
+        }
+    }
+    block_sum<CT * PER * 2>(v, red, e.partials + ((size_t)blockIdx.x * e.OC + c0 * PER) * 2);
+}
+
+template <int CT, int PER = 0>
 __global__ __launch_bounds__(MEDT_THREADS) void conv1x1_bwd_data_kernel(
     const float* __restrict__ dy, const float* __restrict__ raw, const float* __restrict__ coef,
-    const float* __restrict__ w, float* __restrict__ dx, int N, int Cin, int Cout, int HW, int npg) {
+    const float* __restrict__ w, float* __restrict__ dx, int N, int Cin, int Cout, int HW, int npg, StatsEpi epi) {
+    if constexpr (PER > 0) {
+        const int lin = blockIdx.y * gridDim.x + blockIdx.x;
+        if (lin < epi.tj.blocks) {
+            MEDT_STATIC_SHARED float tl[512];
+            sim_tables_block(lin, epi.tj.relative, epi.tj.tables, epi.tj.HQ, epi.tj.L, tl);
+        }
+    }
     const long q = (long)blockIdx.x * MEDT_THREADS + threadIdx.x;
     const int  c0 = blockIdx.y * CT;
     const bool ok = q < (long)N * HW;
@@ -84,6 +122,12 @@
     float acc[CT];
 #pragma unroll
     for (int c = 0; c < CT; ++c) acc[c] = 0.f;
+    float esx[PER > 0 ? CT * PER : 1], eym[CT];
+    if constexpr (PER > 0) {
+        if (epi.bf16) stats_epilogue_load<CT, PER, true>(epi, ok, n, p, c0, Cin, HW, esx, eym);
+        else stats_epilogue_load<CT, PER, false>(epi, ok, n, p, c0, Cin, HW, esx, eym);
+        MEDT_SCHED_FENCE();
+    }
     auto batch = [&](auto u_tag, auto cf_tag, int o) {
         constexpr int UU = decltype(u_tag)::value;
         constexpr bool CF = decltype(cf_tag)::value;
@@ -122,6 +166,10 @@
         float* dp = dx + ((size_t)n * Cin + c0) * HW + p;
 #pragma unroll
         for (int c = 0; c < CT; ++c) dp[(size_t)c * HW] = acc[c];
+    }
+    if constexpr (PER > 0) {
+        MEDT_STATIC_SHARED float red[MEDT_WAVES * CT * PER * 2];
+        stats_epilogue<CT, PER>(epi, acc, esx, eym, ok, c0, red);
     }
 }
 
@@ -201,41 +249,73 @@
     }
 }
 
+struct Dgrad1x1Plan { bool ws; int CT; unsigned gx; };
+static Dgrad1x1Plan dgrad1x1_plan(int N, int Cin, int Cout, int HW) {
+    Dgrad1x1Plan pl;
+    if ((long)N * HW <= 4096 && Cout >= 64 && Cout <= 768 && Cin % 8 == 0) {
+        pl.ws = true;
+        pl.gx = (unsigned)(((long)N * HW + 63) / 64);
+        pl.CT = (Cin % 16 == 0 && pl.gx * (Cin / 16) >= 64) ? 16 : 8;
+        return pl;
+    }
+    pl.ws = false;
+    pl.gx = (unsigned)(((long)N * HW + MEDT_THREADS - 1) / MEDT_THREADS);
+    int CT = 16;
+    while (CT > 1 && (Cin % CT != 0 || (long)pl.gx * (Cin / CT) < 512)) CT >>= 1;
+    while (Cin % CT != 0) CT >>= 1;
+    pl.CT = CT;
+    return pl;
+}
+
+bool conv1x1_bwd_data_ws(int N, int Cin, int Cout, int HW, long* blocks) {
+    const Dgrad1x1Plan pl = dgrad1x1_plan(N, Cin, Cout, HW);
+    if (blocks) *blocks = (long)pl.gx * (Cin / pl.CT);
+    return pl.ws;
+}
+
 int conv1x1_bwd_data_impl(const float* dy, const float* raw, const float* coef, const float* w, float* dx, int N, int Cin,
-                          int Cout, int HW, int groups, hipStream_t s);
+                          int Cout, int HW, int groups, hipStream_t s, const StatsEpi* epi);
 int conv1x1_bwd_data(const float* dy, const float* raw, const float* coef, const float* w, float* dx, int N, int Cin,
-                     int Cout, int HW, int groups, hipStream_t s) {
+                     int Cout, int HW, int groups, hipStream_t s, const StatsEpi* epi) {
     if (abl_skip(groups > 1 ? "qkv_dgrad_l" : "qkv_dgrad_g")) return MEDT_OK;
-    return conv1x1_bwd_data_impl(dy, raw, coef, w, dx, N, Cin, Cout, HW, groups, s);
+    return conv1x1_bwd_data_impl(dy, raw, coef, w, dx, N, Cin, Cout, HW, groups, s, epi);
 }
 int conv1x1_bwd_data_impl(const float* dy, const float* raw, const float* coef, const float* w, float* dx, int N, int Cin,
-                     int Cout, int HW, int groups, hipStream_t s) {
+                     int Cout, int HW, int groups, hipStream_t s, const StatsEpi* epi) {
     const int npg = N / groups;
-    const unsigned gx = (unsigned)(((long)N * HW + MEDT_THREADS - 1) / MEDT_THREADS);
-    if ((long)N * HW <= 4096 && Cout >= 64 && Cout <= 768 && Cin % 8 == 0) {
-        const unsigned g64 = (unsigned)(((long)N * HW + 63) / 64);
-        if (Cin % 16 == 0 && g64 * (Cin / 16) >= 64)
-            hipLaunchKernelGGL(conv1x1_bwd_data_ws_kernel<16>, dim3(g64, Cin / 16), dim3(MEDT_THREADS),
-                               (size_t)Cout * 16 * sizeof(float), s, dy, raw, coef, w, dx, N, Cin, Cout, HW, npg);
-        else
-            hipLaunchKernelGGL(conv1x1_bwd_data_ws_kernel<8>, dim3(g64, Cin / 8), dim3(MEDT_THREADS),
-                               (size_t)Cout * 8 * sizeof(float), s, dy, raw, coef, w, dx, N, Cin, Cout, HW, npg);
+    const Dgrad1x1Plan pl = dgrad1x1_plan(N, Cin, Cout, HW);
+    const int per = epi ? epi->OC / Cin : 0;
+    if (epi && (pl.ws || per < 1 || per > 2 || epi->OC != per * Cin || ((long)N * HW) % MEDT_THREADS != 0 ||
+                epi->tj.blocks > (long)pl.gx * (Cin / pl.CT) || (epi->tj.blocks && epi->tj.L > 128))) {
+        set_error("conv1x1_bwd_data: the statistics epilogue does not fit this problem (plain kernel, whole workgroups, room for the tables)");
+        return MEDT_EINVAL;
+    }
+    const StatsEpi e = epi ? *epi : StatsEpi{nullptr, nullptr, nullptr, nullptr, nullptr, 0, 0, TablesJob{nullptr, nullptr, 0, 0, 0}};
+#define MEDT_LAUNCH_1X1_WS(T)                                                                                      \
+    hipLaunchKernelGGL(conv1x1_bwd_data_ws_kernel<T>, dim3(pl.gx, Cin / T), dim3(MEDT_THREADS),                    \
+                       (size_t)Cout * T * sizeof(float), s, dy, raw, coef, w, dx, N, Cin, Cout, HW, npg)
+#define MEDT_LAUNCH_1X1(T, P)                                                                                      \
+    hipLaunchKernelGGL((conv1x1_bwd_data_kernel<T, P>), dim3(pl.gx, Cin / T), dim3(MEDT_THREADS), 0, s, dy, raw, coef, w, dx, N, \
+                       Cin, Cout, HW, npg, e)
+#define MEDT_PER_1X1(L, T)                                                                                          \
+    do {                                                                                                           \
+        if (per == 2) L(T, 2); else if (per == 1) L(T, 1); else L(T, 0);                                           \
+    } while (0)
+    if (pl.ws) {
+        if (pl.CT == 16) MEDT_LAUNCH_1X1_WS(16);
+        else MEDT_LAUNCH_1X1_WS(8);
         return launch_status("conv1x1_bwd_data_ws");
     }
-    int CT = 16;
-    while (CT > 1 && (Cin % CT != 0 || (long)gx * (Cin / CT) < 512)) CT >>= 1;
-    while (Cin % CT != 0) CT >>= 1;
-#define MEDT_LAUNCH_1X1(T)                                                                                       \
-    hipLaunchKernelGGL(conv1x1_bwd_data_kernel<T>, dim3(gx, Cin / T), dim3(MEDT_THREADS), 0, s, dy, raw, coef, w, dx, N, \
-                       Cin, Cout, HW, npg)
-    switch (CT) {
-        case 16: MEDT_LAUNCH_1X1(16); break;
-        case 8: MEDT_LAUNCH_1X1(8); break;
-        case 4: MEDT_LAUNCH_1X1(4); break;
-        case 2: MEDT_LAUNCH_1X1(2); break;
-        default: MEDT_LAUNCH_1X1(1); break;
-    }
+    switch (pl.CT) {
+        case 16: MEDT_PER_1X1(MEDT_LAUNCH_1X1, 16); break;
+        case 8: MEDT_PER_1X1(MEDT_LAUNCH_1X1, 8); break;
+        case 4: MEDT_PER_1X1(MEDT_LAUNCH_1X1, 4); break;
+        case 2: MEDT_PER_1X1(MEDT_LAUNCH_1X1, 2); break;
+        default: MEDT_PER_1X1(MEDT_LAUNCH_1X1, 1); break;
+    }
+#undef MEDT_PER_1X1
 #undef MEDT_LAUNCH_1X1
+#undef MEDT_LAUNCH_1X1_WS
     return launch_status("conv1x1_bwd_data");
 }
 
diff --git a/medical-transformer_amd/lib/models/axialnet.py b/medical-transformer_amd/lib/models/axialnet.py
--- a/medical-transformer_amd/lib/models/axialnet.py
+++ b/medical-transformer_amd/lib/models/axialnet.py
@@ -64,7 +64,7 @@
     def forward(self, x):
         return self.run(x, self.bn_groups, False)
 
-    def run(self, x, bn_groups=1, out_relu=False, pre=None):
+    def run(self, x, bn_groups=1, out_relu=False, pre=None, take=None, give=None):
         L = x.shape[3] if self.width else x.shape[2]
         if self._has_pos and L != self.kernel_size:
             raise RuntimeError(f"axial attention built for sequence length {self.kernel_size}, got {L}")
@@ -72,7 +72,7 @@
         return medt_amd.axial_attention(
             x, self.qkv_transform.weight, self.bn_qkv, self.bn_similarity, self.bn_output,
             self.relative if self._has_pos else None, gates, self.groups, self.width, self.stride,
-            self.training, bn_groups, out_relu, self._gate_mode, pre)
+            self.training, bn_groups, out_relu, self._gate_mode, pre, take, give)
 
 
 class AxialAttention(_AxialAttentionBase):
diff --git a/medical-transformer_amd/medt_amd/_lib.py b/medical-transformer_amd/medt_amd/_lib.py
--- a/medical-transformer_amd/medt_amd/_lib.py
+++ b/medical-transformer_amd/medt_amd/_lib.py
@@ -50,6 +50,12 @@
                 ("bn_out_bias", C.c_void_p), ("relative", C.c_void_p), ("gates", C.c_void_p)]
 
 
+class BwdHandoff(C.Structure):
+    _fields_ = [("consumer", AxialDesc), ("stacked", C.c_void_p), ("stats", C.c_void_p), ("relative", C.c_void_p),
+                ("ymask", C.c_void_p), ("buf", C.c_void_p), ("buf_bytes", C.c_size_t), ("rows", C.c_int32),
+                ("tables", C.c_int32)]
+
+
 class BlockDesc(C.Structure):
     _fields_ = [("N", C.c_int32), ("C", C.c_int32), ("width", C.c_int32), ("H", C.c_int32), ("W", C.c_int32),
                 ("G", C.c_int32), ("training", C.c_int32), ("bn_groups", C.c_int32), ("eps", C.c_float),
@@ -97,6 +103,10 @@
     "medt_axial_layer_bwd": (C.c_int, [C.POINTER(AxialDesc), C.POINTER(AxialParams), C.c_void_p, C.c_void_p, C.c_void_p,
                                        C.POINTER(AxialSaved), C.c_void_p, C.POINTER(AxialGrads), C.c_void_p,
                                        C.c_size_t, C.c_void_p]),
+    "medt_bwd_handoff_bytes": (C.c_size_t, [C.POINTER(AxialDesc)]),
+    "medt_axial_layer_bwd_handoff": (C.c_int, [C.POINTER(AxialDesc), C.POINTER(AxialParams), C.c_void_p, C.c_void_p, C.c_void_p,
+                                               C.POINTER(AxialSaved), C.c_void_p, C.POINTER(AxialGrads),
+                                               C.POINTER(BwdHandoff), C.POINTER(BwdHandoff), C.c_void_p, C.c_size_t, C.c_void_p]),
     "medt_axial_core_stats": (C.c_int, [C.POINTER(AxialDesc), C.POINTER(AxialParams), C.POINTER(AxialSaved),
                                         C.c_void_p, C.c_size_t, C.c_void_p]),
     "medt_axial_core_fwd": (C.c_int, [C.POINTER(AxialDesc), C.POINTER(AxialParams), C.POINTER(AxialSaved),
@@ -120,6 +130,10 @@
     "medt_conv_block_bwd": (C.c_int, [C.POINTER(ConvDesc), C.c_void_p, C.c_void_p, C.POINTER(BnPtrs), C.c_void_p,
                                       C.c_void_p, C.c_void_p, C.c_void_p, C.c_void_p, C.c_void_p, C.c_void_p, C.c_void_p,
                                       C.c_void_p, C.c_void_p, C.c_void_p, C.c_void_p, C.c_size_t, C.c_void_p]),
+    "medt_conv_block_bwd_handoff": (C.c_int, [C.POINTER(ConvDesc), C.c_void_p, C.c_void_p, C.POINTER(BnPtrs), C.c_void_p,
+                                              C.c_void_p, C.c_void_p, C.c_void_p, C.c_void_p, C.c_void_p, C.c_void_p, C.c_void_p,
+                                              C.c_void_p, C.c_void_p, C.c_void_p, C.POINTER(BwdHandoff), C.c_void_p, C.c_size_t,
+                                              C.c_void_p]),
     "medt_gate_mlp_fwd": (C.c_int, [C.c_void_p] * 9 + [C.c_int] * 5 + [C.c_void_p]),
     "medt_gate_mlp_bwd": (C.c_int, [C.c_void_p] * 13 + [C.c_int] * 5 + [C.c_void_p]),
     "medt_up2x_relu_add_fwd": (C.c_int, [C.c_void_p, C.c_void_p, C.c_void_p, C.c_int, C.c_int, C.c_int, C.c_void_p]),
diff --git a/medical-transformer_amd/medt_amd/axial.py b/medical-transformer_amd/medt_amd/axial.py
--- a/medical-transformer_amd/medt_amd/axial.py
+++ b/medical-transformer_amd/medt_amd/axial.py
@@ -1,6 +1,7 @@
 from __future__ import annotations
 
 import ctypes as C
+import os
 from typing import Optional
 
 import torch
@@ -23,9 +24,57 @@
         raise L.MedtError(f"activation storage dtype {dtype!r} unsupported (float32 or bfloat16)")
 
 
+HANDOFF = os.environ.get("MEDT_BWD_HANDOFF", "1") != "0"
+HANDOFF_COUNT = {"given": 0, "taken": 0, "ignored": 0}
+
+
+class BwdHandoff:
+    __slots__ = ("consumer", "dx", "version", "buf", "rows", "tables")
+
+    def __init__(self):
+        self.consumer = None
+        self.clear()
+
+    def clear(self):
+        self.dx, self.version, self.buf, self.rows, self.tables = None, 0, None, 0, 0
+
+    def register(self, desc, stacked, stats, relative, y):
+        self.consumer = (desc, stacked, stats, relative, y)
+        self.clear()
+
+    def give(self):
+        if not HANDOFF or self.consumer is None:
+            return None
+        desc, stacked, stats, relative, y = self.consumer
+        nbytes = L.lib().medt_bwd_handoff_bytes(C.byref(desc))
+        if nbytes == 0:
+            return None
+        buf = torch.empty((nbytes,), device=stacked.device, dtype=torch.uint8)
+        return L.BwdHandoff(desc, stacked.data_ptr(), stats.data_ptr(), L.ptr(relative), L.ptr(y), buf.data_ptr(), nbytes, 0, 0), buf
+
+    def given(self, st, buf, dx):
+        self.clear()
+        if st.rows > 0:
+            self.dx, self.version, self.buf, self.rows, self.tables = dx, dx._version, buf, st.rows, st.tables
+            HANDOFF_COUNT["given"] += 1
+
+    def take(self, dy):
+        if self.dx is None:
+            return None
+        ok = dy.data_ptr() == self.dx.data_ptr() and dy.shape == self.dx.shape and dy._version == self.version
+        out = None
+        if ok and self.consumer is not None:
+            desc, stacked, stats, relative, y = self.consumer
+            out = (L.BwdHandoff(desc, stacked.data_ptr(), stats.data_ptr(), L.ptr(relative), L.ptr(y), self.buf.data_ptr(),
+                                self.buf.numel(), self.rows, self.tables), self.buf)
+        HANDOFF_COUNT["taken" if out is not None else "ignored"] += 1
+        self.clear()
+        return out
+
+
 class AxialConfig:
     __slots__ = ("groups", "axis", "has_pos", "stride", "bn_groups", "eps", "momentum",
-                 "bn_qkv", "bn_similarity", "bn_output", "out_relu", "gate_mode", "act_dtype", "pre")
+                 "bn_qkv", "bn_similarity", "bn_output", "out_relu", "gate_mode", "act_dtype", "pre", "take", "give")
 
     def __init__(self, groups, axis, has_pos, stride, bn_qkv, bn_similarity, bn_output, bn_groups=1,
                  eps=1e-5, momentum=0.1, out_relu=False, gate_mode=0):
@@ -35,6 +84,8 @@
         self.bn_groups, self.eps, self.momentum, self.out_relu = bn_groups, eps, momentum, out_relu
         self.bn_qkv, self.bn_similarity, self.bn_output = bn_qkv, bn_similarity, bn_output
         self.pre = None
+        self.take = None
+        self.give = None
 
 
 def _require_device(x: torch.Tensor):
@@ -107,6 +158,8 @@
                                              ws.data_ptr(), ws_bytes, stream), "medt_axial_layer_fwd")
             if q is not None:
                 q.hold(ws, stats)
+        if cfg.take is not None and HANDOFF:
+            cfg.take.register(desc, stacked, stats, relative, y.detach() if cfg.out_relu else None)
         ctx.cfg, ctx.training, ctx.has_gates = cfg, training, gates is not None
         ctx.slots = tuple(OPT.grad_slot(t) if t is not None else None
                           for t in (w_qkv, bnq_w, bnq_b, bns_w, bns_b, bno_w, bno_b, relative))
@@ -170,9 +223,22 @@
         ws = torch.empty((ws_bytes,), device=dev, dtype=torch.uint8)
         stream = torch.cuda.current_stream().cuda_stream
         q = DEFER.recording(allow=not pend and all(r is None for r in ret) and (not want_gates or gate_direct))
-        L.check(lib.medt_axial_layer_bwd(C.byref(desc), C.byref(params), x.data_ptr(), L.ptr(y), dy.data_ptr(), C.byref(saved),
-                                         dx.data_ptr(), C.byref(grads), ws.data_ptr(), ws_bytes, stream),
-                "medt_axial_layer_bwd")
+        take = cfg.take.take(dy) if cfg.take is not None else None
+        give = cfg.give.give() if cfg.give is not None else None
+        if take is None and give is None:
+            L.check(lib.medt_axial_layer_bwd(C.byref(desc), C.byref(params), x.data_ptr(), L.ptr(y), dy.data_ptr(), C.byref(saved),
+                                             dx.data_ptr(), C.byref(grads), ws.data_ptr(), ws_bytes, stream),
+                    "medt_axial_layer_bwd")
+        else:
+            L.check(lib.medt_axial_layer_bwd_handoff(C.byref(desc), C.byref(params), x.data_ptr(), L.ptr(y), dy.data_ptr(),
+                                                     C.byref(saved), dx.data_ptr(), C.byref(grads),
+                                                     C.byref(take[0]) if take is not None else None,
+                                                     C.byref(give[0]) if give is not None else None,
+                                                     ws.data_ptr(), ws_bytes, stream), "medt_axial_layer_bwd_handoff")
+            if give is not None:
+                cfg.give.given(give[0], give[1], dx)
+            if q is not None:
+                q.hold(*[t[1] for t in (take, give) if t is not None])
         if q is not None:
             q.hold(ws, x, qkv_raw, stats, *dst)
             if tmp_sizes:
@@ -192,10 +258,11 @@
 
 def axial_attention(x, qkv_weight, bn_qkv, bn_similarity, bn_output, relative: Optional[torch.Tensor],
                     gates, groups: int, width: bool, stride: int, training: bool, bn_groups: int = 1,
-                    out_relu: bool = False, gate_mode: int = 0, pre=None):
+                    out_relu: bool = False, gate_mode: int = 0, pre=None, take=None, give=None):
     cfg = AxialConfig(groups, 1 if width else 0, relative is not None, stride, bn_qkv, bn_similarity, bn_output,
                       bn_groups, bn_qkv.eps, _momentum(bn_qkv), out_relu, gate_mode)
     cfg.pre = pre
+    cfg.take, cfg.give = take, give
     g = gates if gates is not None else (None, None, None, None)
     return AxialAttentionFn.apply(x, qkv_weight, bn_qkv.weight, bn_qkv.bias, bn_similarity.weight,
                                   bn_similarity.bias, bn_output.weight, bn_output.bias, relative,
diff --git a/medical-transformer_amd/medt_amd/net.py b/medical-transformer_amd/medt_amd/net.py
--- a/medical-transformer_amd/medt_amd/net.py
+++ b/medical-transformer_amd/medt_amd/net.py
@@ -6,6 +6,7 @@
 from . import ops
 from . import defer as DEFER
 from . import block as BLOCK
+from . import axial as AXIAL
 
 import os
 
@@ -15,6 +16,8 @@
 SINKS = os.environ.get("MEDT_GRAD_SINKS", "1") != "0"
 EARLY_FIN = os.environ.get("MEDT_EARLY_FIN", "1") != "0"
 _side = {}
+import threading
+_hint = threading.local()
 
 
 def _side_stream(device):
@@ -49,16 +52,17 @@
     pre.setdefault("ds", None)
     out = ops.conv_block(x, blk.conv_down, blk.bn1, relu=True, training=blk.bn1.training, bn_groups=bn_groups,
                          x_sink=sink, x_role="final", pre=pre["down"])
-    out = blk.hight_block.run(out, bn_groups, False, pre["h"])
-    out = blk.width_block.run(out, bn_groups, True, pre["w"])
+    hh, hw = (AXIAL.BwdHandoff(), AXIAL.BwdHandoff()) if getattr(_hint, "handoff", True) else (None, None)
+    out = blk.hight_block.run(out, bn_groups, False, pre["h"], take=hh)
+    out = blk.width_block.run(out, bn_groups, True, pre["w"], take=hw, give=hh)
     if blk.downsample is not None:
         identity = ops.conv_block(x, blk.downsample[0], blk.downsample[1], relu=False,
                                   training=blk.downsample[1].training, bn_groups=bn_groups, x_sink=sink, x_role="deposit",
                                   pre=pre["ds"])
         return ops.conv_block(out, blk.conv_up, blk.bn2, res=identity, relu=True, training=blk.bn2.training,
-                              bn_groups=bn_groups, pre=pre["up"])
+                              bn_groups=bn_groups, pre=pre["up"], give=hw)
     return ops.conv_block(out, blk.conv_up, blk.bn2, res=x, relu=True, training=blk.bn2.training,
-                          bn_groups=bn_groups, res_sink=sink, pre=pre["up"])
+                          bn_groups=bn_groups, res_sink=sink, pre=pre["up"], give=hw)
 
 
 def _layer(seq, x, bn_groups=1):
@@ -107,9 +111,14 @@
     if side is not None:
         side.wait_stream(main)
     DEFER.set_aux_stream(side)
-    g = _stem(net, xin, first_of_branch=side is not None)
-    x1 = _layer(net.layer1, g)
-    x2 = _layer(net.layer2, x1)
+    prev_handoff = getattr(_hint, "handoff", True)
+    _hint.handoff = False
+    try:
+        g = _stem(net, xin, first_of_branch=side is not None)
+        x1 = _layer(net.layer1, g)
+        x2 = _layer(net.layer2, x1)
+    finally:
+        _hint.handoff = prev_handoff
     y = ops.up2x_relu_add(ops.conv_block(x2, net.decoder4), x1, ops.sink_of(x1) if SINKS else None)
     y = ops.up2x_relu_add(ops.conv_block(y, net.decoder5), None)
     if side is not None and EARLY_FIN:
diff --git a/medical-transformer_amd/medt_amd/ops.py b/medical-transformer_amd/medt_amd/ops.py
--- a/medical-transformer_amd/medt_amd/ops.py
+++ b/medical-transformer_amd/medt_amd/ops.py
@@ -53,10 +53,12 @@
 
 
 class ConvBlockCfg:
-    __slots__ = ("stride", "pad", "bn", "relu", "bn_groups", "x_sink", "x_role", "res_sink", "last_of_branch", "pre", "lean")
+    __slots__ = ("stride", "pad", "bn", "relu", "bn_groups", "x_sink", "x_role", "res_sink", "last_of_branch", "pre", "lean",
+                 "give")
 
     def __init__(self, stride, pad, bn, relu, bn_groups=1, x_sink=None, x_role=None, res_sink=None, last_of_branch=False,
-                 pre=None):
+                 pre=None, give=None):
+        self.give = give
         self.stride, self.pad, self.bn, self.relu, self.bn_groups = stride, pad, bn, relu, bn_groups
         self.x_sink, self.x_role, self.res_sink = x_sink, x_role, res_sink
         self.last_of_branch = last_of_branch
@@ -145,10 +147,21 @@
         ws = torch.empty((ws_bytes,), device=dev, dtype=torch.uint8)
         bnp = _bn_ptrs(cfg.bn, False) if has_bn else None
         q = DEFER.recording(allow=not pend and all(r is None for r in ret))
-        L.check(lib.medt_conv_block_bwd(C.byref(desc), x.data_ptr(), w.data_ptr(), C.byref(bnp) if has_bn else None,
-                                        L.ptr(z), L.ptr(y), L.ptr(stats), dy.data_ptr(), L.ptr(dx), dst[0].data_ptr(),
-                                        L.ptr(dst[1]), L.ptr(dst[2]), L.ptr(dst[3]), L.ptr(dres), L.ptr(dx_add), ws.data_ptr(),
-                                        ws_bytes, _stream()), "medt_conv_block_bwd")
+        give = cfg.give.give() if (cfg.give is not None and dx is not None and dep is None) else None
+        if give is None:
+            L.check(lib.medt_conv_block_bwd(C.byref(desc), x.data_ptr(), w.data_ptr(), C.byref(bnp) if has_bn else None,
+                                            L.ptr(z), L.ptr(y), L.ptr(stats), dy.data_ptr(), L.ptr(dx), dst[0].data_ptr(),
+                                            L.ptr(dst[1]), L.ptr(dst[2]), L.ptr(dst[3]), L.ptr(dres), L.ptr(dx_add), ws.data_ptr(),
+                                            ws_bytes, _stream()), "medt_conv_block_bwd")
+        else:
+            L.check(lib.medt_conv_block_bwd_handoff(C.byref(desc), x.data_ptr(), w.data_ptr(), C.byref(bnp) if has_bn else None,
+                                                    L.ptr(z), L.ptr(y), L.ptr(stats), dy.data_ptr(), L.ptr(dx), dst[0].data_ptr(),
+                                                    L.ptr(dst[1]), L.ptr(dst[2]), L.ptr(dst[3]), L.ptr(dres), L.ptr(dx_add),
+                                                    C.byref(give[0]), ws.data_ptr(), ws_bytes, _stream()),
+                    "medt_conv_block_bwd_handoff")
+            cfg.give.given(give[0], give[1], dx)
+            if q is not None:
+                q.hold(give[1])
         if q is not None:
             q.hold(ws, x, dy, stats, dres, *dst)
         for slot, tmp in pend:
@@ -169,9 +182,9 @@
 
 
 def conv_block(x, conv, bn=None, res=None, relu=False, training=False, bn_groups=1, x_sink=None, x_role=None,
-               res_sink=None, last_of_branch=False, pre=None):
+               res_sink=None, last_of_branch=False, pre=None, give=None):
     cfg = ConvBlockCfg(conv.stride[0], conv.padding[0], bn, relu, bn_groups if bn is not None else 1, x_sink, x_role,
-                       res_sink, last_of_branch, pre)
+                       res_sink, last_of_branch, pre, give)
     if bn is None:
         training = torch.is_grad_enabled() and (x.requires_grad or conv.weight.requires_grad)
     return ConvBlockFn.apply(x, conv.weight, conv.bias, bn.weight if bn is not None else None,
```

Measured after the change: 2129 images/s. Within noise of the previous version (-0.9%).
